# wusize/CLIPSelf

Hardware: AMD Instinct MI355X
Metric: images/sec (student+teacher distill step), ViT-B/16 32 crops/img (higher is better)
Workload: dtype bf16; 1 GPU; EVA02-CLIP-B-16 CLIPSelf image-patches step, 64 images x 32 crops per GPU, 224^2 (BASELINE configs[1]); global_batch=64, crops_per_image=32, image_size=224, parallelism=dp1, teacher_chunk=2048, teacher_last_block=cls_query_only, teacher_schedule=one_batch_ahead_on_side_stream

## Files before the change

clipself_amd/csrc/elementwise.hip:

```cpp
#include "cs_common.h"

namespace {

__device__ __forceinline__ float silu_f(float x) { return x / (1.f + __expf(-x)); }

__global__ __launch_bounds__(256) void swiglu_fwd_kernel(const __bf16* __restrict__ x12, long ldx, __bf16* __restrict__ h, long ldh,
                                                         int M, int Hd) {
    const int vec_per_row = Hd >> 3;
    const long total = (long)M * vec_per_row;
    for (long i = (long)blockIdx.x * blockDim.x + threadIdx.x; i < total; i += (long)gridDim.x * blockDim.x) {
        const int m = (int)(i / vec_per_row), j = (int)(i - (long)m * vec_per_row) * 8;
        U128 a, b, o;
        a.u = *(const uint4*)(x12 + (size_t)m * ldx + j);
        b.u = *(const uint4*)(x12 + (size_t)m * ldx + Hd + j);
#pragma unroll
        for (int e = 0; e < 8; ++e) o.e[e] = f2bf(silu_f(bf2f(a.e[e])) * bf2f(b.e[e]));
        *(uint4*)(h + (size_t)m * ldh + j) = o.u;
    }
}

__global__ __launch_bounds__(256) void swiglu_bwd_kernel(const __bf16* __restrict__ dh, long lddh, const __bf16* __restrict__ x12, long ldx,
                                                         __bf16* __restrict__ dx12, long lddx, int M, int Hd) {
    const int vec_per_row = Hd >> 3;
    const long total = (long)M * vec_per_row;
    for (long i = (long)blockIdx.x * blockDim.x + threadIdx.x; i < total; i += (long)gridDim.x * blockDim.x) {
        const int m = (int)(i / vec_per_row), j = (int)(i - (long)m * vec_per_row) * 8;
        U128 a, b, g, o1, o2;
        a.u = *(const uint4*)(x12 + (size_t)m * ldx + j);
        b.u = *(const uint4*)(x12 + (size_t)m * ldx + Hd + j);
        g.u = *(const uint4*)(dh + (size_t)m * lddh + j);
#pragma unroll
        for (int e = 0; e < 8; ++e) {
            const float x1 = bf2f(a.e[e]), x2 = bf2f(b.e[e]), d = bf2f(g.e[e]);
            const float sig = 1.f / (1.f + __expf(-x1));
            o1.e[e] = f2bf(d * x2 * (sig + x1 * sig * (1.f - sig)));
            o2.e[e] = f2bf(d * x1 * sig);
        }
        *(uint4*)(dx12 + (size_t)m * lddx + j) = o1.u;
        *(uint4*)(dx12 + (size_t)m * lddx + Hd + j) = o2.u;
    }
}

__global__ __launch_bounds__(256) void swiglu_bwd_colsum_kernel(const __bf16* __restrict__ dh, long lddh, const __bf16* __restrict__ x12, long ldx,
                                                                __bf16* __restrict__ dx12, long lddx, float* __restrict__ part, int M, int Hd,
                                                                int rows_per_block) {
    __shared__ float red[2][4][512];
    const int tx = threadIdx.x & 63, ty = threadIdx.x >> 6;
    const int j = (blockIdx.x * 64 + tx) * 8;
    const int m_begin = blockIdx.y * rows_per_block, m_end = min(M, m_begin + rows_per_block);
    float s1[8] = {0, 0, 0, 0, 0, 0, 0, 0}, s2[8] = {0, 0, 0, 0, 0, 0, 0, 0};
    if (j < Hd) {
        auto one = [&](const U128& a, const U128& b, const U128& g, int m) {
            U128 o1, o2;
#pragma unroll
            for (int e = 0; e < 8; ++e) {
                const float x1 = bf2f(a.e[e]), x2 = bf2f(b.e[e]), d = bf2f(g.e[e]);
                const float sig = 1.f / (1.f + __expf(-x1));
                o1.e[e] = f2bf(d * x2 * (sig + x1 * sig * (1.f - sig)));
                o2.e[e] = f2bf(d * x1 * sig);
                s1[e] += bf2f(o1.e[e]);
                s2[e] += bf2f(o2.e[e]);
            }
            *(uint4*)(dx12 + (size_t)m * lddx + j) = o1.u;
            *(uint4*)(dx12 + (size_t)m * lddx + Hd + j) = o2.u;
        };
        int m = m_begin + ty;
        for (; m + 4 < m_end; m += 8) {
            U128 a[2], b[2], g[2];
#pragma unroll
            for (int u = 0; u < 2; ++u) {
                a[u].u = *(const uint4*)(x12 + (size_t)(m + 4 * u) * ldx + j);
                b[u].u = *(const uint4*)(x12 + (size_t)(m + 4 * u) * ldx + Hd + j);
                g[u].u = *(const uint4*)(dh + (size_t)(m + 4 * u) * lddh + j);
            }
            one(a[0], b[0], g[0], m);
            one(a[1], b[1], g[1], m + 4);
        }
        for (; m < m_end; m += 4) {
            U128 a, b, g;
            a.u = *(const uint4*)(x12 + (size_t)m * ldx + j);
            b.u = *(const uint4*)(x12 + (size_t)m * ldx + Hd + j);
            g.u = *(const uint4*)(dh + (size_t)m * lddh + j);
            one(a, b, g, m);
        }
    }
#pragma unroll
    for (int e = 0; e < 8; ++e) { red[0][ty][tx * 8 + e] = s1[e]; red[1][ty][tx * 8 + e] = s2[e]; }
    __syncthreads();
    for (int c = threadIdx.x; c < 512; c += 256) {
        const int col = blockIdx.x * 512 + c;
        if (col < Hd) {
            part[(size_t)blockIdx.y * 2 * Hd + col] = (red[0][0][c] + red[0][1][c]) + (red[0][2][c] + red[0][3][c]);
            part[(size_t)blockIdx.y * 2 * Hd + Hd + col] = (red[1][0][c] + red[1][1][c]) + (red[1][2][c] + red[1][3][c]);
        }
    }
}

template <int IT>
__global__ __launch_bounds__(256) void swiglu_bwd_q8_kernel(const __bf16* __restrict__ dh, long lddh, const __bf16* __restrict__ x12, long ldx,
// ... 127 lines not shown
            U128 o;
#pragma unroll
            for (int e = 0; e < 8; ++e) ((uint16_t*)&o)[e] = tile[rv + e][c];
            *(uint4*)(dst + (size_t)(c0 + c) * ld_out + r0 + rv) = o.u;
        }
        return;
    }
    const int tx = threadIdx.x & 63, ty = threadIdx.x >> 6;
#pragma unroll
    for (int i = 0; i < 16; ++i) {
        const int r = r0 + ty * 16 + i, c = c0 + tx;
        tile[ty * 16 + i][tx] = (r < R && c < Cc) ? src[(size_t)r * ld_in + c] : (uint16_t)0;
    }
    __syncthreads();
#pragma unroll
    for (int i = 0; i < 16; ++i) {
        const int c = c0 + ty * 16 + i, r = r0 + tx;
        if (c < Cc && r < ld_out) dst[(size_t)c * ld_out + r] = tile[tx][ty * 16 + i];
    }
}

__global__ __launch_bounds__(256) void transpose_bf16_kernel(const __bf16* __restrict__ in, long ld_in, __bf16* __restrict__ out,
                                                             long ld_out, int R, int Cc) {
    __shared__ uint16_t tile[64][66];
    transpose_tile(in, ld_in, out, ld_out, R, Cc, blockIdx.y * 64, blockIdx.x * 64, tile);
}

struct TransposeDesc {
    const __bf16* in;
    __bf16* out;
    long ld_in, ld_out;
    int R, Cc, tile0, tiles_x;
};
__global__ __launch_bounds__(256) void transpose_bf16_batched_kernel(const TransposeDesc* __restrict__ desc, int count) {
    __shared__ uint16_t tile[64][66];
    const int t = blockIdx.x;
    int i = 0;
    while (i + 1 < count && desc[i + 1].tile0 <= t) ++i;
    const TransposeDesc d = desc[i];
    const int local = t - d.tile0;
    transpose_tile(d.in, d.ld_in, d.out, d.ld_out, d.R, d.Cc, (local / d.tiles_x) * 64, (local % d.tiles_x) * 64, tile);
}

__global__ __launch_bounds__(256) void colsum_bf16_kernel(const __bf16* __restrict__ x, long ldx, float* __restrict__ out, int M, int N,
                                                          int rows_per_block) {
    __shared__ float red[4][512];
    const int tx = threadIdx.x & 63, ty = threadIdx.x >> 6;
    const int n = (blockIdx.x * 64 + tx) * 8;
    const int m_begin = blockIdx.y * rows_per_block, m_end = min(M, m_begin + rows_per_block);
    float s[8] = {0, 0, 0, 0, 0, 0, 0, 0};
    const bool vec = (ldx & 7) == 0 && ((uintptr_t)x & 15) == 0;
    if (n + 8 <= N && vec) {
        int m = m_begin + ty;
        for (; m + 12 < m_end; m += 16) {
            U128 v[4];
#pragma unroll
            for (int u = 0; u < 4; ++u) v[u].u = *(const uint4*)(x + (size_t)(m + 4 * u) * ldx + n);
#pragma unroll
            for (int u = 0; u < 4; ++u)
#pragma unroll
                for (int e = 0; e < 8; ++e) s[e] += bf2f(v[u].e[e]);
        }
        for (; m < m_end; m += 4) {
            U128 v;
            v.u = *(const uint4*)(x + (size_t)m * ldx + n);
#pragma unroll
            for (int e = 0; e < 8; ++e) s[e] += bf2f(v.e[e]);
        }
    } else {
        for (int m = m_begin + ty; m < m_end; m += 4)
            for (int e = 0; e < 8; ++e)
                if (n + e < N) s[e] += bf2f(x[(size_t)m * ldx + n + e]);
    }
#pragma unroll
    for (int e = 0; e < 8; ++e) red[ty][tx * 8 + e] = s[e];
    __syncthreads();
    for (int c = threadIdx.x; c < 512; c += 256) {
        const int col = blockIdx.x * 512 + c;
        if (col < N) out[(size_t)blockIdx.y * N + col] = (red[0][c] + red[1][c]) + (red[2][c] + red[3][c]);
    }
}

__global__ __launch_bounds__(256) void colsum_reduce_kernel(const float* __restrict__ part, int nblocks, int N, float* __restrict__ out) {
    __shared__ float red[4][64];
    const int tx = threadIdx.x & 63, r = threadIdx.x >> 6;
    const int n = blockIdx.x * 64 + tx;
    float s = 0.f;
    if (n < N) {
        int b = r;
        for (; b + 28 < nblocks; b += 32) {
            float v[8];
#pragma unroll
            for (int u = 0; u < 8; ++u) v[u] = part[(size_t)(b + 4 * u) * N + n];
#pragma unroll
            for (int u = 0; u < 8; ++u) s += v[u];
        }
        for (; b < nblocks; b += 4) s += part[(size_t)b * N + n];
    }
    red[r][tx] = s;
    __syncthreads();
    if (r == 0 && n < N) out[n] += (red[0][tx] + red[1][tx]) + (red[2][tx] + red[3][tx]);
}

template <typename TI>
__global__ __launch_bounds__(256) void im2row_kernel(const TI* __restrict__ img, __bf16* __restrict__ out, int B, int S, int p, int g, int ldo) {
    const int segs = p / 8;
    const long total = (long)B * g * g * 3 * p * segs;
    for (long i = (long)blockIdx.x * blockDim.x + threadIdx.x; i < total; i += (long)gridDim.x * blockDim.x) {
        long t = i;
        const int sg = (int)(t % segs); t /= segs;
        const int iy = (int)(t % p); t /= p;
        const int c = (int)(t % 3); t /= 3;
        const int px = (int)(t % g); t /= g;
        const int py = (int)(t % g); t /= g;
        const int b = (int)t;
        const TI* s = img + (((size_t)b * 3 + c) * S + (py * p + iy)) * S + px * p + sg * 8;
        U128 o;
#pragma unroll
        for (int e = 0; e < 8; ++e) o.e[e] = f2bf((float)s[e]);
        const size_t row = ((size_t)b * g + py) * g + px;
        *(uint4*)(out + row * ldo + (c * p + iy) * p + sg * 8) = o.u;
    }
}

template <typename TI>
__global__ __launch_bounds__(256) void im2row_generic_kernel(const TI* __restrict__ img, __bf16* __restrict__ out, int B, int S, int p, int g, int ldo) {
    const long total = (long)B * g * g * ldo;
    const int kk = 3 * p * p;
    for (long i = (long)blockIdx.x * blockDim.x + threadIdx.x; i < total; i += (long)gridDim.x * blockDim.x) {
        const int col = (int)(i % ldo);
        const long row = i / ldo;
        float v = 0.f;
        if (col < kk) {
            const int ix = col % p, iy = (col / p) % p, c = col / (p * p);
            const int px = (int)(row % g), py = (int)((row / g) % g), b = (int)(row / ((long)g * g));
            v = (float)img[(((size_t)b * 3 + c) * S + (py * p + iy)) * S + px * p + ix];
        }
        out[i] = f2bf(v);
    }
}

__global__ void cls_row_kernel(float* __restrict__ x, const float* __restrict__ cls, const float* __restrict__ pos, int B, int Ntok, int C) {
    const long i = (long)blockIdx.x * blockDim.x + threadIdx.x;
    if (i >= (long)B * C) return;
    const int b = (int)(i / C), c = (int)(i - (long)b * C);
    x[(size_t)b * Ntok * C + c] = cls[c] + pos[c];
}

inline int grid_for(long total, int block = 256, int cap = 256 * 16) {
    long g = (total + block - 1) / block;
    return (int)(g < 1 ? 1 : (g > cap ? cap : g));
}

}

extern "C" int cs_swiglu_fwd(const void* x12, long ldx, void* h, long ldh, int M, int Hd, hipStream_t stream) {
    CS_CHECK_ARG(Hd % 8 == 0 && ldx % 8 == 0 && ldh % 8 == 0 && M > 0, "cs_swiglu_fwd: Hd/ld must be multiples of 8");
    hipLaunchKernelGGL(swiglu_fwd_kernel, dim3(grid_for((long)M * (Hd / 8))), dim3(256), 0, stream, (const __bf16*)x12, ldx, (__bf16*)h, ldh, M, Hd);
    CS_LAUNCH_CHECK();
    return 0;
}
extern "C" int cs_swiglu_bwd(const void* dh, long lddh, const void* x12, long ldx, void* dx12, long lddx, int M, int Hd, hipStream_t stream) {
    CS_CHECK_ARG(Hd % 8 == 0 && ldx % 8 == 0 && lddh % 8 == 0 && lddx % 8 == 0 && M > 0, "cs_swiglu_bwd: Hd/ld must be multiples of 8");
    hipLaunchKernelGGL(swiglu_bwd_kernel, dim3(grid_for((long)M * (Hd / 8))), dim3(256), 0, stream, (const __bf16*)dh, lddh, (const __bf16*)x12, ldx,
                       (__bf16*)dx12, lddx, M, Hd);
    CS_LAUNCH_CHECK();
    return 0;
}
constexpr int COLSUM_ROWS = 64;
extern "C" int cs_swiglu_bwd_colsum(const void* dh, long lddh, const void* x12, long ldx, void* dx12, long lddx, float* colsum, void* workspace,
                                    int M, int Hd, hipStream_t stream) {
    CS_CHECK_ARG(Hd % 8 == 0 && ldx % 8 == 0 && lddh % 8 == 0 && lddx % 8 == 0 && M > 0, "cs_swiglu_bwd_colsum: Hd/ld must be multiples of 8");
    CS_CHECK_ARG(colsum != nullptr && workspace != nullptr, "cs_swiglu_bwd_colsum: colsum and workspace (cs_colsum_workspace(M, 2*Hd) bytes) are required");
    const int nblocks = (M + COLSUM_ROWS - 1) / COLSUM_ROWS;
    hipLaunchKernelGGL(swiglu_bwd_colsum_kernel, dim3((Hd + 511) / 512, nblocks), dim3(256), 0, stream, (const __bf16*)dh, lddh, (const __bf16*)x12, ldx,
                       (__bf16*)dx12, lddx, (float*)workspace, M, Hd, COLSUM_ROWS);
    CS_LAUNCH_CHECK();
    hipLaunchKernelGGL(colsum_reduce_kernel, dim3((2 * Hd + 63) / 64), dim3(256), 0, stream, (const float*)workspace, nblocks, 2 * Hd, colsum);
    CS_LAUNCH_CHECK();
    return 0;
}
extern "C" int cs_swiglu_bwd_q8(const void* dh, long lddh, const void* x12, long ldx, void* dx12, long lddx, void* q8, long ldq, float* q_scale,
                                int M, int Hd, hipStream_t stream) {
    const int Kp = (2 * Hd + 127) / 128 * 128;
    CS_CHECK_ARG(Hd % 8 == 0 && Hd >= 8 && Hd <= 4096 && ldx % 8 == 0 && lddh % 8 == 0 && lddx % 8 == 0 && M > 0, "cs_swiglu_bwd_q8: Hd=%d (%% 8, <= 4096), ld %% 8", Hd);
    CS_CHECK_ARG(q8 && q_scale && ldq >= Kp && ldq % 8 == 0 && ((uintptr_t)q8 % 8) == 0, "cs_swiglu_bwd_q8: q8 rows of >= %d bytes, 8-byte aligned", Kp);
    const dim3 grid((M + 3) / 4), block(256);
#define SWQ(IT) hipLaunchKernelGGL(swiglu_bwd_q8_kernel<IT>, grid, block, 0, stream, (const __bf16*)dh, lddh, (const __bf16*)x12, ldx, (__bf16*)dx12, lddx, \
                                   (unsigned char*)q8, ldq, q_scale, M, Hd, Kp)
    if (Hd <= 2048) SWQ(4); else if (Hd <= 3072) SWQ(6); else SWQ(8);
#undef SWQ
    CS_LAUNCH_CHECK();
    return 0;
}
extern "C" int cs_gelu_fwd(const void* x, long ldx, void* y, long ldy, int M, int N, int quick, hipStream_t stream) {
    CS_CHECK_ARG(x && y && N % 8 == 0 && ldx % 8 == 0 && ldy % 8 == 0 && M > 0 && N > 0, "cs_gelu_fwd: N/ld must be multiples of 8");
    const dim3 grid(grid_for((long)M * (N / 8))), block(256);
    if (quick) hipLaunchKernelGGL(gelu_fwd_kernel<true>, grid, block, 0, stream, (const __bf16*)x, ldx, (__bf16*)y, ldy, M, N);
    else hipLaunchKernelGGL(gelu_fwd_kernel<false>, grid, block, 0, stream, (const __bf16*)x, ldx, (__bf16*)y, ldy, M, N);
    CS_LAUNCH_CHECK();
    return 0;
}
extern "C" int cs_gelu_bwd(const void* dy, long lddy, const void* x, long ldx, void* dx, long lddx, int M, int N, int quick, hipStream_t stream) {
    CS_CHECK_ARG(dy && x && dx && N % 8 == 0 && ldx % 8 == 0 && lddy % 8 == 0 && lddx % 8 == 0 && M > 0 && N > 0,
                 "cs_gelu_bwd: N/ld must be multiples of 8");
    const dim3 grid(grid_for((long)M * (N / 8))), block(256);
    if (quick) hipLaunchKernelGGL(gelu_bwd_kernel<true>, grid, block, 0, stream, (const __bf16*)dy, lddy, (const __bf16*)x, ldx, (__bf16*)dx, lddx, M, N);
    else hipLaunchKernelGGL(gelu_bwd_kernel<false>, grid, block, 0, stream, (const __bf16*)dy, lddy, (const __bf16*)x, ldx, (__bf16*)dx, lddx, M, N);
    CS_LAUNCH_CHECK();
    return 0;
}
extern "C" int cs_cast_f32_bf16(const float* x, void* y, long n, hipStream_t stream) {
    CS_CHECK_ARG(n > 0 && n % 8 == 0, "cs_cast_f32_bf16: n must be a positive multiple of 8");
    hipLaunchKernelGGL(cast_f32_bf16_kernel, dim3(grid_for(n / 8)), dim3(256), 0, stream, x, (__bf16*)y, n / 8);
    CS_LAUNCH_CHECK();
    return 0;
}
extern "C" int cs_transpose_bf16(const void* in, long ld_in, void* out, long ld_out, int R, int Cc, hipStream_t stream) {
    CS_CHECK_ARG(R > 0 && Cc > 0 && ld_out >= R, "cs_transpose_bf16: bad shape R=%d C=%d ld_out=%ld", R, Cc, ld_out);
    dim3 grid((Cc + 63) / 64, (int)((ld_out + 63) / 64));
    hipLaunchKernelGGL(transpose_bf16_kernel, grid, dim3(256), 0, stream, (const __bf16*)in, ld_in, (__bf16*)out, ld_out, R, Cc);
    CS_LAUNCH_CHECK();
    return 0;
}
extern "C" int cs_transpose_bf16_batched(const void* desc, int count, int total_tiles, hipStream_t stream) {
    CS_CHECK_ARG(desc != nullptr && count > 0 && total_tiles > 0, "cs_transpose_bf16_batched: empty batch");
    static_assert(sizeof(TransposeDesc) == 48, "descriptor layout is part of the C ABI");
    hipLaunchKernelGGL(transpose_bf16_batched_kernel, dim3(total_tiles), dim3(256), 0, stream, (const TransposeDesc*)desc, count);
    CS_LAUNCH_CHECK();
    return 0;
}
extern "C" size_t cs_colsum_workspace(int M, int N) {
    return (size_t)((M + COLSUM_ROWS - 1) / COLSUM_ROWS) * (size_t)(N > 0 ? N : 0) * sizeof(float);
}
extern "C" int cs_colsum_bf16(const void* x, long ldx, float* out, void* workspace, int M, int N, hipStream_t stream) {
    CS_CHECK_ARG(M > 0 && N > 0 && workspace != nullptr, "cs_colsum_bf16: empty input or no workspace (cs_colsum_workspace bytes)");
    const int nblocks = (M + COLSUM_ROWS - 1) / COLSUM_ROWS;
    dim3 grid((N + 511) / 512, nblocks);
    hipLaunchKernelGGL(colsum_bf16_kernel, grid, dim3(256), 0, stream, (const __bf16*)x, ldx, (float*)workspace, M, N, COLSUM_ROWS);
    CS_LAUNCH_CHECK();
    hipLaunchKernelGGL(colsum_reduce_kernel, dim3((N + 63) / 64), dim3(256), 0, stream, (const float*)workspace, nblocks, N, out);
    CS_LAUNCH_CHECK();
    return 0;
}
extern "C" int cs_im2row(const void* img, int img_dtype, void* out, int B, int S, int p, int ldo, hipStream_t stream) {
    CS_CHECK_ARG(S % p == 0 && B > 0 && ldo >= 3 * p * p, "cs_im2row: patch size must divide S and ldo >= 3*p*p (p=%d S=%d ldo=%d)", p, S, ldo);
    const int g = S / p;
    if (p % 8 == 0 && ldo == 3 * p * p) {
        const long total = (long)B * g * g * 3 * p * (p / 8);
        if (img_dtype == 0)
            hipLaunchKernelGGL((im2row_kernel<float>), dim3(grid_for(total)), dim3(256), 0, stream, (const float*)img, (__bf16*)out, B, S, p, g, ldo);
        else
            hipLaunchKernelGGL((im2row_kernel<__bf16>), dim3(grid_for(total)), dim3(256), 0, stream, (const __bf16*)img, (__bf16*)out, B, S, p, g, ldo);
    } else {
        const long total = (long)B * g * g * ldo;
        if (img_dtype == 0)
            hipLaunchKernelGGL((im2row_generic_kernel<float>), dim3(grid_for(total)), dim3(256), 0, stream, (const float*)img, (__bf16*)out, B, S, p, g, ldo);
        else
            hipLaunchKernelGGL((im2row_generic_kernel<__bf16>), dim3(grid_for(total)), dim3(256), 0, stream, (const __bf16*)img, (__bf16*)out, B, S, p, g, ldo);
    }
    CS_LAUNCH_CHECK();
    return 0;
}
extern "C" int cs_cls_row(float* x, const float* cls, const float* pos, int B, int Ntok, int C, hipStream_t stream) {
    CS_CHECK_ARG(B > 0, "cs_cls_row: empty batch");
    hipLaunchKernelGGL(cls_row_kernel, dim3((int)(((long)B * C + 255) / 256)), dim3(256), 0, stream, x, cls, pos, B, Ntok, C);
    CS_LAUNCH_CHECK();
    return 0;
}

namespace {

template <int IT>
__global__ __launch_bounds__(256) void quant_rows_fp8_kernel(const __bf16* __restrict__ x, long ldx, unsigned char* __restrict__ q, long ldq,
                                                             float* __restrict__ scale, int M, int K, int Kp) {
    const int lane = threadIdx.x & 63;
    const long row = (long)blockIdx.x * 4 + (threadIdx.x >> 6);
    if (row >= M) return;
    U128 v[IT];
    float amax = 0.f;
#pragma unroll
    for (int it = 0; it < IT; ++it) {
        const int k = (it * 64 + lane) * 8;
        if (k < K) {
            v[it].u = *(const uint4*)(x + row * ldx + k);
#pragma unroll
            for (int e = 0; e < 8; ++e) amax = fmaxf(amax, fabsf(bf2f(v[it].e[e])));
        } else {
            v[it].u = make_uint4(0, 0, 0, 0);
        }
    }
    amax = wave_max(amax);
    const float inv = amax > 0.f ? 448.f / amax : 0.f;
    if (lane == 0) scale[row] = amax > 0.f ? amax / 448.f : 1.f;
#pragma unroll
    for (int it = 0; it < IT; ++it) {
        const int k = (it * 64 + lane) * 8;
        if (k < Kp) {
            unsigned lo = 0, hi = 0;
            lo = __builtin_amdgcn_cvt_pk_fp8_f32(bf2f(v[it].e[0]) * inv, bf2f(v[it].e[1]) * inv, lo, false);
            lo = __builtin_amdgcn_cvt_pk_fp8_f32(bf2f(v[it].e[2]) * inv, bf2f(v[it].e[3]) * inv, lo, true);
            hi = __builtin_amdgcn_cvt_pk_fp8_f32(bf2f(v[it].e[4]) * inv, bf2f(v[it].e[5]) * inv, hi, false);
            hi = __builtin_amdgcn_cvt_pk_fp8_f32(bf2f(v[it].e[6]) * inv, bf2f(v[it].e[7]) * inv, hi, true);
            *(uint2*)(q + row * ldq + k) = make_uint2(lo, hi);
        }
    }
}

}

extern "C" int cs_quant_rows_fp8(const void* x, long ldx, void* q, long ldq, float* scale, int M, int K, hipStream_t stream) {
    const int Kp = (K + 127) / 128 * 128;
    CS_CHECK_ARG(M > 0 && K > 0 && K % 8 == 0 && K <= 8192, "cs_quant_rows_fp8: K=%d must be a multiple of 8, at most 8192", K);
    CS_CHECK_ARG(ldx % 8 == 0 && ldq >= Kp && ldq % 8 == 0 && ((uintptr_t)x % 16) == 0 && ((uintptr_t)q % 8) == 0,
                 "cs_quant_rows_fp8: rows must be 16-byte (input) / 8-byte (output) aligned and ldq >= %d", Kp);
    if (K <= 4096) hipLaunchKernelGGL(quant_rows_fp8_kernel<8>, dim3((M + 3) / 4), dim3(256), 0, stream, (const __bf16*)x, ldx, (unsigned char*)q, ldq, scale, M, K, Kp);
    else hipLaunchKernelGGL(quant_rows_fp8_kernel<16>, dim3((M + 3) / 4), dim3(256), 0, stream, (const __bf16*)x, ldx, (unsigned char*)q, ldq, scale, M, K, Kp);
    CS_LAUNCH_CHECK();
    return 0;
}
```

clipself_amd/csrc/gemm.hip:

```cpp
#include "gemm_common.h"
#include <hip/amd_detail/amd_hip_unsafe_atomics.h>

namespace {

constexpr int EP_LD = 68;
constexpr int EP_BYTES = 32 * EP_LD * 4;

template <int FM, int BN>
__device__ __forceinline__ void epilogue_swiglu(const GemmArgs& p, const f32x16 (&acc)[FM][2], char* slab_bytes, char* rowst_bytes, int lane,
                                                int row0, int tn, int wn) {
    const int l31 = lane & 31, hf = lane >> 5;
    uint32_t* slab = (uint32_t*)slab_bytes;
    const int hbase = tn * (BN / 2) + wn * 32;
    const int hl = hbase + l31;
    float b1 = 0.f, b2 = 0.f;
    if (p.bias && hl < p.group) { b1 = p.bias[hl]; b2 = p.bias[p.group + hl]; }
    const bool ln = p.ln_mean != nullptr;
    float c1 = 0.f, c2 = 0.f;
    float2* rowst = (float2*)rowst_bytes;
    if (ln) {
        if (hl < p.group) { c1 = p.ln_colsum[hl]; c2 = p.ln_colsum[p.group + hl]; }
        for (int r = lane; r < FM * 32; r += 64) {
            const int row = min(row0 + r, p.M - 1);
            const float rs = p.ln_rstd[row];
            rowst[r] = make_float2(-rs * p.ln_mean[row], rs);
        }
        asm volatile("s_waitcnt lgkmcnt(0)" ::: "memory");
    }
    const int c4 = lane & 7, hcol = hbase + c4 * 4;
    const bool colok = hcol < p.group;
#pragma unroll
    for (int i = 0; i < FM; ++i) {
#pragma unroll
        for (int e = 0; e < 16; e += 2) {
            float h[2];
            float4 st4 = make_float4(0.f, 1.f, 0.f, 1.f);
            if (ln) st4 = *(const float4*)(rowst + i * 32 + mfma32_row(e, lane));
#pragma unroll
            for (int t = 0; t < 2; ++t) {
                float u = acc[i][0][e + t], v = acc[i][1][e + t];
                if (ln) {
                    const float2 st = t ? make_float2(st4.z, st4.w) : make_float2(st4.x, st4.y);
                    u = fmaf(st.y, u, fmaf(st.x, c1, b1));
                    v = fmaf(st.y, v, fmaf(st.x, c2, b2));
                } else {
                    u += b1;
                    v += b2;
                }
                h[t] = u * __builtin_amdgcn_rcpf(1.f + __builtin_amdgcn_exp2f(-1.4426950408889634f * u)) * v;
            }
            union { bf16x2 v; uint32_t u; } pk;
            pk.v[0] = f2bf(h[0]);
            pk.v[1] = f2bf(h[1]);
            const int rp = ((e & 3) >> 1) + 4 * (e >> 2) + 2 * hf;
            slab[rp * 32 + l31] = pk.u;
        }
        asm volatile("s_waitcnt lgkmcnt(0)" ::: "memory");
        const int row_base = row0 + i * 32;
        float ps[4] = {0, 0, 0, 0}, pq[4] = {0, 0, 0, 0};
#pragma unroll
        for (int k = 0; k < 2; ++k) {
            const int rp = (lane >> 3) + 8 * k;
            const uint4 w = *(const uint4*)(slab + rp * 32 + c4 * 4);
            const uint2 lo = make_uint2((w.x & 0xffffu) | (w.y << 16), (w.z & 0xffffu) | (w.w << 16));
            const uint2 hi = make_uint2((w.x >> 16) | (w.y & 0xffff0000u), (w.z >> 16) | (w.w & 0xffff0000u));
            const int ra = row_base + 2 * rp;
            if (colok && ra < p.M) *(uint2*)((__bf16*)p.C + (size_t)ra * p.ldc + hcol) = lo;
            if (colok && ra + 1 < p.M) *(uint2*)((__bf16*)p.C + (size_t)(ra + 1) * p.ldc + hcol) = hi;
            if (p.stats_part && colok) {
                const uint32_t ws[4] = {w.x, w.y, w.z, w.w};
#pragma unroll
                for (int t = 0; t < 4; ++t) {
                    const float a = __uint_as_float(ws[t] << 16), b = __uint_as_float(ws[t] & 0xffff0000u);
                    ps[2 * k] += a; pq[2 * k] += a * a;
                    ps[2 * k + 1] += b; pq[2 * k + 1] += b * b;
                }
            }
        }
        if (p.stats_part) {
            const int sel = lane & 7;
            float sv = 0.f, qv = 0.f;
#pragma unroll
            for (int j = 0; j < 4; ++j) {
// ... 538 lines not shown
                 "cs_gemm_nt: N, ldc must be multiples of 4 and C 16-byte aligned (vector epilogue)");
    CS_CHECK_ARG(bias == nullptr || ((uintptr_t)bias % 16) == 0, "cs_gemm_nt: bias must be 16-byte aligned");
    GemmArgs a;
    a.A = (const __bf16*)A; a.B = (const __bf16*)B; a.C = C; a.bias = bias; a.extra = extra;
    a.M = M; a.N = N; a.K = K; a.lda = lda; a.ldb = ldb; a.ldc = ldc; a.group = group;
    a.split_stride = 0;
    a.ln_mean = ln_mean; a.ln_rstd = ln_rstd; a.ln_colsum = ln_colsum; a.stats_part = stats_part;
    a.xb_out = (__bf16*)xb_out; a.ldxb = ldxb;
    a.tiles_m = a.tiles_n = 0;
    a.gm = ((flags >> 8) & 15) ? ((flags >> 8) & 15) : 8;
    a.rm = (flags >> 16) & 3;
    a.nsplit = 1;
    if (a.rm == 1 || a.rm == 2) {
        const int f = (flags >> 8) & 15;
        CS_CHECK_ARG(f == 0 || f == 1 || f == 2 || f == 4 || f == 8, "cs_gemm_nt: B-stationary raster needs 1, 2, 4 or 8 N parts (got %d)", f);
        int parts = f;
        if (parts == 0) for (parts = 1; parts < 8 && (double)N * K * 2 / parts > 3.3e6; parts *= 2) {}
        a.nsplit = parts;
        a.gm = 8;
    }
    if (epi == EPI_SWIGLU_BF16) CS_CHECK_ARG(group > 0 && N == 2 * group, "cs_gemm_nt: swiglu epilogue needs N == 2*group");
    if (epi == EPI_RESID_LN_F32) CS_CHECK_ARG(ln_mean && ln_rstd && ln_colsum && ((uintptr_t)ln_colsum % 16) == 0, "cs_gemm_nt_ln: epilogue 6 needs mean, rstd and a 16-byte aligned column-sum vector");
    CS_CHECK_ARG(stats_part == nullptr || epi == EPI_SWIGLU_BF16 || epi == EPI_RESID_F32 || epi == EPI_RESID_LN_F32,
                 "cs_gemm_nt_ln: statistics output exists for the SwiGLU and residual epilogues");
    CS_CHECK_ARG(xb_out == nullptr || ((epi == EPI_RESID_F32 || epi == EPI_RESID_LN_F32) && ldxb % 4 == 0 && ((uintptr_t)xb_out % 8) == 0),
                 "cs_gemm_nt_ln: the bf16 copy exists for the residual epilogues (8-byte aligned, ldxb %% 4 == 0)");
    CS_CHECK_ARG((ln_mean == nullptr) == (ln_rstd == nullptr) && (ln_mean == nullptr || ln_colsum != nullptr),
                 "cs_gemm_nt_ln: mean, rstd and the column-sum vector come together");
    CS_CHECK_ARG(ln_mean == nullptr || epi_is_bf16(epi) || epi == EPI_SWIGLU_BF16 || epi == EPI_RESID_LN_F32,
                 "cs_gemm_nt_ln: a folded LayerNorm exists for epilogues 0, 3, 6, 7 and 8");
    if (epi == EPI_PATCH_F32 || epi == EPI_RESID_F32 || epi == EPI_RESID_LN_F32) CS_CHECK_ARG(extra != nullptr && ((uintptr_t)extra % 16) == 0, "cs_gemm_nt: epilogue %d needs 16-byte aligned extra", epi);
    if (epi == EPI_PATCH_F32) CS_CHECK_ARG(group > 0, "cs_gemm_nt: patch epilogue needs group");
    a.ktiles_per_split = K / BK;
    const int glds = (flags & 1) ? 0 : 1;
    const int force = (flags >> 4) & 15;
    a.dbg = (flags >> 12) & 15;
    a.reserve = (flags >> 20) & 255;
    switch (epi) {
        case EPI_BF16: return launch<EPI_BF16>(a, splits, glds, force, stream);
        case EPI_F32: return launch<EPI_F32>(a, splits, glds, force, stream);
        case EPI_RESID_F32: return launch<EPI_RESID_F32>(a, splits, glds, force, stream);
        case EPI_SWIGLU_BF16: return launch<EPI_SWIGLU_BF16>(a, splits, glds, force, stream);
        case EPI_ATOMIC_F32: return launch<EPI_ATOMIC_F32>(a, splits, glds, force, stream);
        case EPI_PATCH_F32: return launch<EPI_PATCH_F32>(a, splits, glds, force, stream);
        case EPI_RESID_LN_F32: return launch<EPI_RESID_LN_F32>(a, splits, glds, force, stream);
        case EPI_GELU_BF16: return launch<EPI_GELU_BF16>(a, splits, glds, force, stream);
        case EPI_QGELU_BF16: return launch<EPI_QGELU_BF16>(a, splits, glds, force, stream);
    }
    cs_set_error("cs_gemm_nt: unknown epilogue %d", epi);
    return -1;
}

static int gemm_nt_split_f32(const void* A, const void* B, float* C, int M, int N, int K, int lda, int ldb, int cfg, int splits, hipStream_t stream) {
    CS_CHECK_ARG(M > 0 && N > 0 && K > 0 && K % BK == 0 && N % 4 == 0, "cs_gemm_wgrad: bad problem M=%d N=%d K=%d", M, N, K);
    CS_CHECK_ARG((lda % 8) == 0 && (ldb % 8) == 0 && ((uintptr_t)A % 16) == 0 && ((uintptr_t)B % 16) == 0, "cs_gemm_wgrad: operands must be 16-byte aligned rows");
    GemmArgs a;
    a.A = (const __bf16*)A; a.B = (const __bf16*)B; a.C = C; a.bias = nullptr; a.extra = nullptr;
    a.M = M; a.N = N; a.K = K; a.lda = lda; a.ldb = ldb; a.ldc = N; a.group = 0;
    a.split_stride = (long)M * N;
    a.ln_mean = a.ln_rstd = a.ln_colsum = nullptr; a.stats_part = nullptr; a.xb_out = nullptr; a.ldxb = 0;
    a.tiles_m = a.tiles_n = 0; a.gm = 8; a.dbg = 0; a.rm = 0; a.nsplit = 1; a.reserve = 0;
    a.ktiles_per_split = K / BK;
    return launch<EPI_F32>(a, splits, 1, cfg, stream);
}

extern "C" int cs_gemm_nt(const void* A, const void* B, void* C, const float* bias, const float* extra, int M, int N, int K,
                          int lda, int ldb, int ldc, int epi, int splits, int group, int flags, hipStream_t stream) {
    CS_CHECK_ARG(epi != EPI_RESID_LN_F32, "cs_gemm_nt: epilogue 6 (folded LayerNorm) is reached through cs_gemm_nt_ln");
    return gemm_nt_impl(A, B, C, bias, extra, nullptr, nullptr, nullptr, nullptr, nullptr, 0, M, N, K, lda, ldb, ldc, epi, splits, group, flags, stream);
}

extern "C" int cs_gemm_nt_ln(const void* A, const void* B, void* C, const float* bias, const float* extra, const float* ln_mean,
                             const float* ln_rstd, const float* ln_colsum, float* stats_part, void* xb_out, int ldxb, int M, int N, int K,
                             int lda, int ldb, int ldc, int epi, int splits, int group, int flags, hipStream_t stream) {
    return gemm_nt_impl(A, B, C, bias, extra, ln_mean, ln_rstd, ln_colsum, stats_part, xb_out, ldxb, M, N, K, lda, ldb, ldc, epi, splits, group,
                        flags, stream);
}


namespace {

__global__ __launch_bounds__(256) void splitk_reduce_kernel(const float* __restrict__ ws, int splits, long stride, float* __restrict__ dst,
                                                            int M, int N, int ldc) {
    const long i = (long)blockIdx.x * 256 + threadIdx.x;
    const int n4 = N >> 2;
    if (i >= (long)M * n4) return;
    const int row = (int)(i / n4), c = (int)(i - (long)row * n4) * 4;
    float4 acc = *(const float4*)(ws + (size_t)row * N + c);
    for (int s = 1; s < splits; ++s) {
        const float4 t = *(const float4*)(ws + (size_t)s * stride + (size_t)row * N + c);
        acc.x += t.x; acc.y += t.y; acc.z += t.z; acc.w += t.w;
    }
    float4* d = (float4*)(dst + (size_t)row * ldc + c);
    const float4 o = *d;
    *d = make_float4(o.x + acc.x, o.y + acc.y, o.z + acc.z, o.w + acc.w);
}

typedef __attribute__((ext_vector_type(4))) short s16x4;

__device__ __forceinline__ int tn_swz(int tok) { return (tok & 3) << 1; }
typedef short s16x8 __attribute__((ext_vector_type(8)));
struct TrFrag { s16x4 lo, hi; };
__device__ __forceinline__ void tr_read(TrFrag& f, const char* tile, int tok, int colbyte) {
    const int a0 = tok * 512 + (colbyte ^ (tn_swz(tok) << 5)), a1 = (tok + 4) * 512 + (colbyte ^ (tn_swz(tok + 4) << 5));
    const unsigned base = (unsigned)(uintptr_t)(__attribute__((address_space(3))) const char*)tile;
    asm volatile("ds_read_b64_tr_b16 %0, %1" : "=v"(f.lo) : "v"(base + (unsigned)a0));
    asm volatile("ds_read_b64_tr_b16 %0, %1" : "=v"(f.hi) : "v"(base + (unsigned)a1));
}
__device__ __forceinline__ bf16x8 tr_join(const TrFrag& f) {
    const s16x8 v = __builtin_shufflevector(f.lo, f.hi, 0, 1, 2, 3, 4, 5, 6, 7);
    return __builtin_bit_cast(bf16x8, v);
}

template <bool RAGGED>
__global__ __launch_bounds__(512) void gemm_tn_kernel(GemmArgs p) {
    constexpr int BM = 256, BN = 256, WN = 4, TM = 128, TN = 64, FM = 4, FN = 2;
    constexpr int T_BYTES = 64 * 512;
    extern __shared__ __attribute__((aligned(16))) char smem[];
    const int tid = threadIdx.x, lane = tid & 63;
    const int wave = __builtin_amdgcn_readfirstlane(tid >> 6);
    const int wm = wave / WN, wn = wave - wm * WN;
    const int li = lane & 15, grp = lane >> 4, hf = grp >> 1, g1 = grp & 1;
    int tm, tn;
    tile_of_block(p, tm, tn);
    const int n0 = tm * BM, k0 = tn * BN;
    char* const b_ring = smem + 3 * T_BYTES;
    const int drow = lane >> 5, pc = lane & 31;
    const bool role_a = wave >= 4;
    const int piece0 = (wave & 3) * 8;
    unsigned ocol[8], ooff[8];
#pragma unroll
    for (int x = 0; x < 8; ++x) {
        const int row = 2 * (piece0 + x) + drow;
        const int lc = ((((pc >> 1) ^ tn_swz(row)) << 1) | (pc & 1));
        const unsigned ca = (unsigned)(RAGGED ? min(n0 + lc * 8, p.M - 8) : n0 + lc * 8) * 2u;
        const unsigned cb = (unsigned)(RAGGED ? min(k0 + lc * 8, p.N - 8) : k0 + lc * 8) * 2u;
        ocol[x] = role_a ? ca : cb;
        ooff[x] = (unsigned)row * (unsigned)(role_a ? p.lda : p.ldb) * 2u + ocol[x];
    }
    const int ktiles_all = (p.K + 63) >> 6;
    const int kt_begin = blockIdx.y * p.ktiles_per_split, kt_end = min(kt_begin + p.ktiles_per_split, ktiles_all);
    auto issue = [&](int kt, char* dst) {
        const int ld = role_a ? p.lda : p.ldb;
        const char* src = (const char*)(role_a ? p.A : p.B) + (size_t)kt * 64 * ld * 2;
        const int rmax = p.K - 1 - kt * 64;
        if (!RAGGED || rmax >= 63) {
#pragma unroll
            for (int x = 0; x < 8; ++x)
                __builtin_amdgcn_global_load_lds((const __attribute__((address_space(1))) void*)(src + ooff[x]),
                                                 (__attribute__((address_space(3))) void*)(dst + (piece0 + x) * 1024), 16, 0, 0);
        } else {
#pragma unroll
            for (int x = 0; x < 8; ++x) {
                const int row = min(2 * (piece0 + x) + drow, rmax);
                __builtin_amdgcn_global_load_lds((const __attribute__((address_space(1))) void*)(src + (size_t)row * ld * 2 + ocol[x]),
                                                 (__attribute__((address_space(3))) void*)(dst + (piece0 + x) * 1024), 16, 0, 0);
            }
        }
    };
    f32x16 acc[FM][FN];
#pragma unroll
    for (int i = 0; i < FM; ++i)
#pragma unroll
        for (int j = 0; j < FN; ++j)
#pragma unroll
            for (int e = 0; e < 16; ++e) acc[i][j][e] = 0.f;
    if (role_a) {
        if (kt_begin < kt_end) issue(kt_begin, smem);
        if (kt_begin + 1 < kt_end) issue(kt_begin + 1, smem + T_BYTES);
    } else if (kt_begin < kt_end) {
        issue(kt_begin, b_ring);
    }
    const int segbyte = (16 * g1 + 4 * (li & 3)) * 2, trow = 8 * hf + (li >> 2);
    int cur = 0;
    for (int kt = kt_begin; kt < kt_end; ++kt) {
        if (role_a && kt + 1 < kt_end) asm volatile("s_waitcnt vmcnt(8)" ::: "memory");
        else asm volatile("s_waitcnt vmcnt(0)" ::: "memory");
        asm volatile("s_waitcnt lgkmcnt(0)" ::: "memory");
        __builtin_amdgcn_s_barrier();
        const int i0 = kt - kt_begin;
        if (!role_a && kt + 1 < kt_end) issue(kt + 1, b_ring + ((i0 + 1) & 1) * T_BYTES);
        const char* ta = smem + cur * T_BYTES;
        const char* tb = b_ring + (i0 & 1) * T_BYTES;
        const int tvalid = p.K - kt * 64;
        if (RAGGED && tvalid < 64) {
            for (int idx = tid; idx < (64 - tvalid) * 32; idx += 512)
                *(uint4*)(smem + cur * T_BYTES + (tvalid + (idx >> 5)) * 512 + (idx & 31) * 16) = make_uint4(0, 0, 0, 0);
            __syncthreads();
        }
        TrFrag a[2][FM], b[2][FN];
        auto load_frags = [&](int set, int ts) {
#pragma unroll
            for (int i = 0; i < FM; ++i) tr_read(a[set][i], ta, 16 * ts + trow, (wm * TM + i * 32) * 2 + segbyte);
#pragma unroll
            for (int j = 0; j < FN; ++j) tr_read(b[set][j], tb, 16 * ts + trow, (wn * TN + j * 32) * 2 + segbyte);
        };
        static_assert(FM == 4 && FN == 2, "tr_wait names exactly FM = 4 and FN = 2 fragment pairs: extend its operand list with the tile");
        auto tr_wait = [&](int set) {
            asm volatile("s_waitcnt lgkmcnt(0)"
                         : "+v"(a[set][0].lo), "+v"(a[set][0].hi), "+v"(a[set][1].lo), "+v"(a[set][1].hi), "+v"(a[set][2].lo), "+v"(a[set][2].hi),
                           "+v"(a[set][3].lo), "+v"(a[set][3].hi), "+v"(b[set][0].lo), "+v"(b[set][0].hi), "+v"(b[set][1].lo), "+v"(b[set][1].hi));
        };
        load_frags(0, 0);
        tr_wait(0);
#pragma unroll
        for (int ts = 0; ts < 4; ++ts) {
            if (ts < 3) load_frags((ts + 1) & 1, ts + 1);
            if (ts == 3 && role_a && kt + 2 < kt_end) issue(kt + 2, smem + ((i0 + 2) % 3) * T_BYTES);
#pragma unroll
            for (int i = 0; i < FM; ++i)
#pragma unroll
                for (int j = 0; j < FN; ++j)
                    acc[i][j] = __builtin_amdgcn_mfma_f32_32x32x16_bf16(tr_join(a[ts & 1][i]), tr_join(b[ts & 1][j]), acc[i][j], 0, 0, 0);
            if (ts < 3) tr_wait((ts + 1) & 1);
        }
        cur = cur == 2 ? 0 : cur + 1;
    }
    __syncthreads();
    epilogue<EPI_F32, FM, FN, BN>(p, acc, smem, wave, lane, n0 + wm * TM, k0, tn, wn);
}

void choose_wgrad(int M, int N, int K, int& cfg, int& splits) {
    const int ktiles = K / BK;
    const double out_mb = 4.0 * M * N / 1e6;
    const struct { int cfg, bm, bn, per_cu; double us; } cand[3] = {{1, 128, 128, 2, 1.9}, {2, 256, 128, 1, 1.4}, {7, 256, 256, 1, 2.2}};
    double best = 1e30;
    cfg = 7; splits = 1;
    for (const auto& c : cand) {
        if (M < c.bm || N < c.bn) continue;
        const long tiles = (long)((M + c.bm - 1) / c.bm) * ((N + c.bn - 1) / c.bn);
        for (int s = 1; s <= 64 && s <= ktiles; ++s) {
            const long rounds = (tiles * s + (long)cs_num_cus() * c.per_cu - 1) / ((long)cs_num_cus() * c.per_cu);
            const int kper = (ktiles + s - 1) / s;
            const double t = rounds * (kper * c.us + 6.0) + (s + 2) * out_mb / 5.0 + 6.0;
            if (t < best) { best = t; cfg = c.cfg; splits = s; }
        }
    }
}

}

namespace {
int choose_tn_splits(int N, int K, int tokens) {
    const long tiles = (long)((N + 255) / 256) * ((K + 255) / 256);
    const int ktiles = (tokens + 63) / 64;
    double best = 1e30;
    int splits = 1;
    for (int sp = 1; sp <= 64 && sp <= ktiles; ++sp) {
        const long rounds = (tiles * sp + 255) / 256;
        const double t = rounds * (((ktiles + sp - 1) / sp) * 2.2 + 6.0) + (sp + 2) * (4.0 * N * K / 1e6) / 5.0;
        if (t < best) { best = t; splits = sp; }
    }
    return splits;
}
}

extern "C" size_t cs_gemm_wgrad_tn_workspace(int N, int K, int tokens) {
    if (tokens <= 0 || N < 8 || K < 8 || N % 8 != 0 || K % 8 != 0) return 0;
    return (size_t)choose_tn_splits(N, K, tokens) * N * K * sizeof(float);
}

extern "C" int cs_gemm_wgrad_tn(const void* dY, const void* X, float* dW, void* workspace, int N, int K, int tokens, int ldy, int ldx, int ldc,
                                hipStream_t stream) {
    if (tokens <= 0 || N < 8 || K < 8 || N % 8 != 0 || K % 8 != 0) return 1;
    CS_CHECK_ARG(workspace != nullptr && ((uintptr_t)workspace % 16) == 0 && dW != nullptr && ((uintptr_t)dW % 16) == 0 && ldc % 4 == 0,
                 "cs_gemm_wgrad_tn: workspace / dW must be 16-byte aligned buffers");
    CS_CHECK_ARG(ldy % 8 == 0 && ldx % 8 == 0 && ((uintptr_t)dY % 16) == 0 && ((uintptr_t)X % 16) == 0 && ldy >= N && ldx >= K,
                 "cs_gemm_wgrad_tn: operand rows must be 16-byte aligned");
    CS_CHECK_ARG((long)64 * ldy * 2 < 0x7fffffffL && (long)64 * ldx * 2 < 0x7fffffffL, "cs_gemm_wgrad_tn: row stride too large");
    int splits = choose_tn_splits(N, K, tokens);
    GemmArgs a;
    a.A = (const __bf16*)dY; a.B = (const __bf16*)X; a.C = workspace; a.bias = nullptr; a.extra = nullptr;
    a.M = N; a.N = K; a.K = tokens; a.lda = ldy; a.ldb = ldx; a.ldc = K; a.group = 0;
    a.split_stride = (long)N * K;
    a.ln_mean = a.ln_rstd = a.ln_colsum = nullptr; a.stats_part = nullptr; a.xb_out = nullptr; a.ldxb = 0;
    a.tiles_m = (N + 255) / 256; a.tiles_n = (K + 255) / 256; a.gm = 8; a.dbg = 0; a.rm = 0; a.nsplit = 1; a.reserve = 0;
    const int ktiles = (tokens + 63) / 64;
    a.ktiles_per_split = (ktiles + splits - 1) / splits;
    constexpr size_t lds = 160 * 1024;
    static bool once = ((void)hipFuncSetAttribute((const void*)gemm_tn_kernel<false>, hipFuncAttributeMaxDynamicSharedMemorySize, (int)lds),
                        (void)hipFuncSetAttribute((const void*)gemm_tn_kernel<true>, hipFuncAttributeMaxDynamicSharedMemorySize, (int)lds), true);
    (void)once;
    if (tokens % 64 == 0 && N % 256 == 0 && K % 256 == 0) hipLaunchKernelGGL(gemm_tn_kernel<false>, dim3(a.tiles_m * a.tiles_n, splits), dim3(512), lds, stream, a);
    else hipLaunchKernelGGL(gemm_tn_kernel<true>, dim3(a.tiles_m * a.tiles_n, splits), dim3(512), lds, stream, a);
    CS_LAUNCH_CHECK();
    const long n = (long)N * (K >> 2);
    hipLaunchKernelGGL(splitk_reduce_kernel, dim3((unsigned)((n + 255) / 256)), dim3(256), 0, stream, (const float*)workspace, splits,
                       (long)N * K, dW, N, K, ldc);
    CS_LAUNCH_CHECK();
    return 0;
}

extern "C" size_t cs_gemm_wgrad_workspace(int M, int N, int K) {
    int cfg, splits;
    choose_wgrad(M, N, K, cfg, splits);
    return (size_t)splits * M * N * sizeof(float);
}

extern "C" int cs_gemm_wgrad(const void* A, const void* B, float* dW, void* workspace, int M, int N, int K, int lda, int ldb, int ldc,
                             hipStream_t stream) {
    CS_CHECK_ARG(workspace != nullptr && ((uintptr_t)workspace % 16) == 0 && dW != nullptr && ((uintptr_t)dW % 16) == 0 && ldc % 4 == 0,
                 "cs_gemm_wgrad: workspace / dW must be 16-byte aligned buffers");
    int cfg, splits;
    choose_wgrad(M, N, K, cfg, splits);
    const int rc = gemm_nt_split_f32(A, B, (float*)workspace, M, N, K, lda, ldb, cfg, splits, stream);
    if (rc) return rc;
    const long n = (long)M * (N >> 2);
    hipLaunchKernelGGL(splitk_reduce_kernel, dim3((unsigned)((n + 255) / 256)), dim3(256), 0, stream, (const float*)workspace, splits,
                       (long)M * N, dW, M, N, ldc);
    CS_LAUNCH_CHECK();
    return 0;
}
```

clipself_amd/csrc/norm.hip:

```cpp
#include "cs_common.h"

namespace {

constexpr int MAXC = 3072;
constexpr int ROWS_PER_WG = 4;

template <typename T> struct Vec4;
template <> struct Vec4<float> {
    typedef float4 raw;
    static __device__ __forceinline__ raw load_raw(const float* p) { return *(const float4*)p; }
    static __device__ __forceinline__ void cvt(const raw& t, float (&v)[4]) { v[0] = t.x; v[1] = t.y; v[2] = t.z; v[3] = t.w; }
    static __device__ __forceinline__ void load(const float* p, float (&v)[4]) { cvt(load_raw(p), v); }
};
template <> struct Vec4<__bf16> {
    typedef uint2 raw;
    static __device__ __forceinline__ raw load_raw(const __bf16* p) { return *(const uint2*)p; }
    static __device__ __forceinline__ void cvt(const raw& r, float (&v)[4]) {
        U64 t; t.u = r;
#pragma unroll
        for (int i = 0; i < 4; ++i) v[i] = bf2f(t.e[i]);
    }
    static __device__ __forceinline__ void load(const __bf16* p, float (&v)[4]) { cvt(load_raw(p), v); }
};
__device__ __forceinline__ void store_bf16x4(__bf16* p, const float (&v)[4]) {
    U64 t;
#pragma unroll
    for (int i = 0; i < 4; ++i) t.e[i] = f2bf(v[i]);
    *(uint2*)p = t.u;
}
__device__ __forceinline__ void store_x4(__bf16* p, const float (&v)[4]) { store_bf16x4(p, v); }
__device__ __forceinline__ void store_x4(float* p, const float (&v)[4]) { *(float4*)p = make_float4(v[0], v[1], v[2], v[3]); }

template <typename TX, int MAXG, typename TY = __bf16, bool Q8 = false, bool RAG = false>
__global__ __launch_bounds__(256) void ln_fwd_kernel(const TX* __restrict__ x, long ldx, const float* __restrict__ gamma,
                                                     const float* __restrict__ beta, TY* __restrict__ y, long ldy,
                                                     float* __restrict__ mean_out, float* __restrict__ rstd_out,
                                                     int M, int C, float eps, unsigned char* __restrict__ q8 = nullptr, long ldq = 0,
                                                     float* __restrict__ q_scale = nullptr, int Kp = 0) {
    const int lane = threadIdx.x & 63;
    const int row = blockIdx.x * ROWS_PER_WG + (threadIdx.x >> 6);
    if (row >= M) return;
    const TX* xr = x + (size_t)row * ldx;
    const int ng = (C + 255) >> 8;
    const int clast = (C - 1) & ~3;
    float v[MAXG][4];
    typename Vec4<TX>::raw xr_raw[MAXG];
#pragma unroll
    for (int g = 0; g < MAXG; ++g) {
        const int c = (g * 64 + lane) * 4;
        xr_raw[g] = Vec4<TX>::load_raw(xr + (g < ng ? min(c, clast) : 0));
    }
    float s = 0.f;
#pragma unroll
    for (int g = 0; g < MAXG; ++g) {
        const int c = (g * 64 + lane) * 4;
        Vec4<TX>::cvt(xr_raw[g], v[g]);
#pragma unroll
        for (int i = 0; i < 4; ++i) v[g][i] = (g < ng && (RAG ? c + i < C : c < C)) ? v[g][i] : 0.f;
        s += (v[g][0] + v[g][1]) + (v[g][2] + v[g][3]);
    }
    const float mean = wave_sum(s) / (float)C;
    float q = 0.f;
#pragma unroll
    for (int g = 0; g < MAXG; ++g) {
        const int c = (g * 64 + lane) * 4;
#pragma unroll
        for (int i = 0; i < 4; ++i) { const float d = v[g][i] - mean; q += (g < ng && c + i < C) ? d * d : 0.f; }
    }
    const float rstd = rsqrtf(wave_sum(q) / (float)C + eps);
    if (y != nullptr) {
        TY* yr = y + (size_t)row * ldy;
        float4 ga[MAXG], be[MAXG];
#pragma unroll
        for (int g = 0; g < MAXG; ++g) {
            const int c = g < ng ? min((g * 64 + lane) * 4, clast) : 0;
            ga[g] = *(const float4*)(gamma + c);
            be[g] = *(const float4*)(beta + c);
        }
        float amax = 0.f;
#pragma unroll
        for (int g = 0; g < MAXG; ++g) {
            const int c = (g * 64 + lane) * 4;
            if (g < ng && c < C) {
                float o[4] = {(v[g][0] - mean) * rstd * ga[g].x + be[g].x, (v[g][1] - mean) * rstd * ga[g].y + be[g].y,
                              (v[g][2] - mean) * rstd * ga[g].z + be[g].z, (v[g][3] - mean) * rstd * ga[g].w + be[g].w};
                if (RAG) {
#pragma unroll
                    for (int i = 0; i < 4; ++i) o[i] = (c + i < C) ? o[i] : 0.f;
                }
                store_x4(yr + c, o);
                if (Q8) {
#pragma unroll
                    for (int i = 0; i < 4; ++i) {
                        v[g][i] = (c + i < C) ? bf2f(f2bf(o[i])) : 0.f;
                        amax = fmaxf(amax, fabsf(v[g][i]));
                    }
                }
            } else if (Q8) {
#pragma unroll
                for (int i = 0; i < 4; ++i) v[g][i] = 0.f;
            }
        }
        if (Q8) {
            amax = wave_max(amax);
            const float inv = amax > 0.f ? 448.f / amax : 0.f;
            if (lane == 0) q_scale[row] = amax > 0.f ? amax / 448.f : 1.f;
#pragma unroll
            for (int g = 0; g < MAXG; ++g) {
                const int c = (g * 64 + lane) * 4;
                if (c < Kp) {
                    unsigned w = 0;
                    w = __builtin_amdgcn_cvt_pk_fp8_f32(v[g][0] * inv, v[g][1] * inv, w, false);
                    w = __builtin_amdgcn_cvt_pk_fp8_f32(v[g][2] * inv, v[g][3] * inv, w, true);
                    *(unsigned*)(q8 + (size_t)row * ldq + c) = w;
                }
            }
        }
    }
    if (lane == 0 && mean_out) { mean_out[row] = mean; rstd_out[row] = rstd; }
}

__global__ __launch_bounds__(256) void ln_stats_finalize_kernel(const float* __restrict__ part, int P, int npp, int C, int M, float eps,
                                                                float* __restrict__ mean_out, float* __restrict__ rstd_out) {
    const int row = blockIdx.x * 256 + threadIdx.x;
    if (row >= M) return;
    const float2* src = (const float2*)part + row;
    float s = 0.f, q = 0.f, b = 0.f;
    int p = 0;
    for (; p + 8 <= P; p += 8) {
        float2 v[8];
#pragma unroll
        for (int j = 0; j < 8; ++j) v[j] = src[(size_t)(p + j) * M];
#pragma unroll
        for (int j = 0; j < 8; ++j) {
            const int n = min(npp, C - (p + j) * npp);
            if (n > 0) {
                const float t = v[j].x * v[j].x / (float)n;
                s += v[j].x;
                q += fmaxf(v[j].y - t, 0.f);
                b += t;
            }
        }
    }
    for (; p < P; ++p) {
        const int n = min(npp, C - p * npp);
        if (n <= 0) break;
        const float2 sq = src[(size_t)p * M];
        const float t = sq.x * sq.x / (float)n;
        s += sq.x;
        q += fmaxf(sq.y - t, 0.f);
        b += t;
    }
    const float mean = s / (float)C;
    const float m2 = q + fmaxf(b - s * mean, 0.f);
    mean_out[row] = mean;
    rstd_out[row] = rsqrtf(m2 / (float)C + eps);
}

__global__ __launch_bounds__(256) void ln_stats_finalize2_kernel(const float* __restrict__ part, int P, int npp, int C, int M, float eps,
                                                                 float* __restrict__ mean_out, float* __restrict__ rstd_out) {
    const int row = (blockIdx.x * 256 + threadIdx.x) * 2;
    if (row >= M) return;
    const float4* src = (const float4*)(part + (size_t)row * 2);
    const size_t stride = (size_t)M / 2;
    float s[2] = {0.f, 0.f}, q[2] = {0.f, 0.f}, b[2] = {0.f, 0.f};
    auto add = [&](const float4& v, int n) {
        const float t0 = v.x * v.x / (float)n, t1 = v.z * v.z / (float)n;
        s[0] += v.x; q[0] += fmaxf(v.y - t0, 0.f); b[0] += t0;
        s[1] += v.z; q[1] += fmaxf(v.w - t1, 0.f); b[1] += t1;
    };
    for (int p = 0; p < P; p += 16) {
        float4 v[16];
#pragma unroll
        for (int j = 0; j < 16; ++j) v[j] = src[(size_t)min(p + j, P - 1) * stride];
#pragma unroll
        for (int j = 0; j < 16; ++j) {
            const int n = min(npp, C - (p + j) * npp);
            if (p + j < P && n > 0) add(v[j], n);
        }
    }
#pragma unroll
    for (int r = 0; r < 2; ++r) {
        const float mean = s[r] / (float)C;
        const float m2 = q[r] + fmaxf(b[r] - s[r] * mean, 0.f);
        mean_out[row + r] = mean;
        rstd_out[row + r] = rsqrtf(m2 / (float)C + eps);
    }
}

enum { DX_BF16 = 0, DX_F32_ASSIGN = 1, DX_F32_ACCUM = 2 };

template <typename TX, int DXMODE, int MAXG, bool COPY, bool RAG = false>
__global__ __launch_bounds__(256) void ln_bwd_kernel(const __bf16* __restrict__ dy, long lddy, const TX* __restrict__ x, long ldx,
                                                     const float* __restrict__ gamma, const float* __restrict__ mean_in,
                                                     const float* __restrict__ rstd_in, void* __restrict__ dx, long lddx,
                                                     __bf16* __restrict__ dxb, long lddxb, float* __restrict__ part, int M, int C,
                                                     unsigned char* __restrict__ q8 = nullptr, long ldq = 0, float* __restrict__ q_scale = nullptr,
                                                     int Kp = 0) {
    static_assert(!COPY || DXMODE != DX_BF16, "the bf16 copy exists for the fp32 stream modes");
// ... 66 lines not shown
                } else {
                    float* p = (float*)dx + (size_t)row * lddx + c;
                    if (DXMODE == DX_F32_ACCUM) {
                        const float4 t = *(const float4*)p;
                        const float tv[4] = {t.x, t.y, t.z, t.w};
#pragma unroll
                        for (int i = 0; i < 4; ++i) o[i] += (!RAG || c + i < C) ? tv[i] : 0.f;
                    }
                    *(float4*)p = make_float4(o[0], o[1], o[2], o[3]);
                    if (COPY) {
                        U64 t;
#pragma unroll
                        for (int i = 0; i < 4; ++i) {
                            t.e[i] = f2bf(o[i]);
                            rq[g][i] = (c + i < C) ? bf2f(t.e[i]) : 0.f;
                            dc[g][i] += rq[g][i];
                            amax = fmaxf(amax, fabsf(rq[g][i]));
                        }
                        *(uint2*)(dxb + (size_t)row * lddxb + c) = t.u;
                    }
                }
            }
        }
        if (COPY && q8 != nullptr) {
            amax = wave_max(amax);
            const float inv = amax > 0.f ? 448.f / amax : 0.f;
            if (lane == 0) q_scale[row] = amax > 0.f ? amax / 448.f : 1.f;
#pragma unroll
            for (int g = 0; g < MAXG; ++g) {
                const int c = (g * 64 + lane) * 4;
                if (c < Kp) {
                    unsigned w = 0;
                    w = __builtin_amdgcn_cvt_pk_fp8_f32(rq[g][0] * inv, rq[g][1] * inv, w, false);
                    w = __builtin_amdgcn_cvt_pk_fp8_f32(rq[g][2] * inv, rq[g][3] * inv, w, true);
                    *(unsigned*)(q8 + (size_t)row * ldq + c) = w;
                }
            }
        }
    }
    if (part == nullptr) return;
    if (wave > 0) {
        float* mine = red + (size_t)(wave - 1) * NR * Cp;
#pragma unroll
        for (int g = 0; g < MAXG; ++g) {
            const int c = (g * 64 + lane) * 4;
            if (g < ng && c < C) {
                *(float4*)(mine + c) = make_float4(dg[g][0], dg[g][1], dg[g][2], dg[g][3]);
                *(float4*)(mine + Cp + c) = make_float4(db[g][0], db[g][1], db[g][2], db[g][3]);
                if (COPY) *(float4*)(mine + 2 * Cp + c) = make_float4(dc[g][0], dc[g][1], dc[g][2], dc[g][3]);
            }
        }
    }
    __syncthreads();
    if (wave == 0) {
        float* outp = part + (size_t)blockIdx.x * NR * Cp;
#pragma unroll
        for (int g = 0; g < MAXG; ++g) {
            const int c = (g * 64 + lane) * 4;
            if (g < ng && c < C) {
                float a[4] = {dg[g][0], dg[g][1], dg[g][2], dg[g][3]};
                float b[4] = {db[g][0], db[g][1], db[g][2], db[g][3]};
                float cc[4] = {0.f, 0.f, 0.f, 0.f};
                if (COPY) { cc[0] = dc[g][0]; cc[1] = dc[g][1]; cc[2] = dc[g][2]; cc[3] = dc[g][3]; }
                for (int w = 0; w < 3; ++w) {
                    const float4 t = *(const float4*)(red + (size_t)w * NR * Cp + c);
                    const float4 u = *(const float4*)(red + (size_t)w * NR * Cp + Cp + c);
                    a[0] += t.x; a[1] += t.y; a[2] += t.z; a[3] += t.w;
                    b[0] += u.x; b[1] += u.y; b[2] += u.z; b[3] += u.w;
                    if (COPY) {
                        const float4 v = *(const float4*)(red + (size_t)w * NR * Cp + 2 * Cp + c);
                        cc[0] += v.x; cc[1] += v.y; cc[2] += v.z; cc[3] += v.w;
                    }
                }
                *(float4*)(outp + c) = make_float4(a[0], a[1], a[2], a[3]);
                *(float4*)(outp + Cp + c) = make_float4(b[0], b[1], b[2], b[3]);
                if (COPY) *(float4*)(outp + 2 * Cp + c) = make_float4(cc[0], cc[1], cc[2], cc[3]);
            }
        }
    }
}

__global__ __launch_bounds__(256) void ln_param_reduce_kernel(const float* __restrict__ part, int nparts, int C, int NR, float* __restrict__ out0,
                                                              float* __restrict__ out1, float* __restrict__ out2, int accumulate) {
    __shared__ float red[16][16];
    const int cl = threadIdx.x & 15, grp = threadIdx.x >> 4;
    const int Cp = (C + 3) & ~3;
    const int c = blockIdx.x * 16 + cl;
    const int r = c / Cp, cc = c - r * Cp;
    float* const outs[3] = {out0, out1, out2};
    const bool live = r < NR && cc < C && outs[r < 3 ? r : 0] != nullptr;
    float s0 = 0.f, s1 = 0.f, s2 = 0.f, s3 = 0.f;
    const size_t stride = (size_t)NR * Cp;
    if (live) {
        int p = grp;
        for (; p + 48 < nparts; p += 64) {
            s0 += part[(size_t)p * stride + c];
            s1 += part[(size_t)(p + 16) * stride + c];
            s2 += part[(size_t)(p + 32) * stride + c];
            s3 += part[(size_t)(p + 48) * stride + c];
        }
        for (; p < nparts; p += 16) s0 += part[(size_t)p * stride + c];
    }
    red[grp][cl] = (s0 + s1) + (s2 + s3);
    __syncthreads();
    if (grp == 0 && live) {
        float s = 0.f;
#pragma unroll
        for (int g = 0; g < 16; ++g) s += red[g][cl];
        float* dst = outs[r] + cc;
        *dst = accumulate ? *dst + s : s;
    }
}

__global__ __launch_bounds__(256) void l2norm_fwd_kernel(const float* __restrict__ x, float* __restrict__ y,
                                                         float* __restrict__ inv_out, int M, int C, float eps) {
    const int lane = threadIdx.x & 63;
    const int row = blockIdx.x * ROWS_PER_WG + (threadIdx.x >> 6);
    if (row >= M) return;
    const float* xr = x + (size_t)row * C;
    float s = 0.f;
    for (int c = lane * 4; c < C; c += 256) { const float4 t = *(const float4*)(xr + c); s += t.x * t.x + t.y * t.y + t.z * t.z + t.w * t.w; }
    const float inv = 1.f / fmaxf(sqrtf(wave_sum(s)), eps);
    for (int c = lane * 4; c < C; c += 256) {
        const float4 t = *(const float4*)(xr + c);
        *(float4*)(y + (size_t)row * C + c) = make_float4(t.x * inv, t.y * inv, t.z * inv, t.w * inv);
    }
    if (lane == 0 && inv_out) inv_out[row] = inv;
}

__global__ __launch_bounds__(256) void l2norm_bwd_kernel(const float* __restrict__ dy, const float* __restrict__ y,
                                                         const float* __restrict__ inv, __bf16* __restrict__ dx, int M, int C) {
    const int lane = threadIdx.x & 63;
    const int row = blockIdx.x * ROWS_PER_WG + (threadIdx.x >> 6);
    if (row >= M) return;
    const float* yr = y + (size_t)row * C;
    const float* gr = dy + (size_t)row * C;
    float s = 0.f;
    for (int c = lane * 4; c < C; c += 256) {
        const float4 a = *(const float4*)(yr + c), b = *(const float4*)(gr + c);
        s += a.x * b.x + a.y * b.y + a.z * b.z + a.w * b.w;
    }
    const float dot = wave_sum(s), iv = inv[row];
    for (int c = lane * 4; c < C; c += 256) {
        const float4 a = *(const float4*)(yr + c), b = *(const float4*)(gr + c);
        float o[4] = {(b.x - a.x * dot) * iv, (b.y - a.y * dot) * iv, (b.z - a.z * dot) * iv, (b.w - a.w * dot) * iv};
        store_bf16x4(dx + (size_t)row * C + c, o);
    }
}

}

static int layernorm_fwd_impl(const void* x, int x_dtype, long ldx, const float* gamma, const float* beta, void* y, long ldy, float* mean,
                              float* rstd, int M, int C, float eps, void* q8, long ldq, float* q_scale, hipStream_t stream) {
    CS_CHECK_ARG(C <= MAXC && (C % 4 == 0 || (ldx >= ((C + 3) & ~3) && (y == nullptr || ldy >= ((C + 3) & ~3)))), "cs_layernorm_fwd: C=%d unsupported (ld too small for a padded row, or > %d)", C, MAXC);
    CS_CHECK_ARG(M > 0, "cs_layernorm_fwd: empty input");
    dim3 grid((M + ROWS_PER_WG - 1) / ROWS_PER_WG), block(256);
    if (q8 != nullptr) {
        const int Kp = (C + 127) / 128 * 128;
        CS_CHECK_ARG(y != nullptr && q_scale != nullptr && ldq >= Kp && ldq % 4 == 0 && ((uintptr_t)q8 % 4) == 0 && Kp <= 256 * 12,
                     "cs_layernorm_fwd_q8: needs y, the scale vector and 4-byte aligned e4m3 rows of >= %d bytes", Kp);
#define LNQ2(TX, NG, RG) hipLaunchKernelGGL((ln_fwd_kernel<TX, NG, __bf16, true, RG>), grid, block, 0, stream, (const TX*)x, ldx, gamma, beta, (__bf16*)y, ldy, mean, rstd, M, C, eps, (unsigned char*)q8, ldq, q_scale, Kp)
#define LNQ(TX, NG) do { if (C % 4 == 0) LNQ2(TX, NG, false); else LNQ2(TX, NG, true); } while (0)
        if (x_dtype == 0) { if (Kp <= 1024) LNQ(float, 4); else if (Kp <= 2048) LNQ(float, 8); else LNQ(float, 12); }
        else { if (Kp <= 1024) LNQ(__bf16, 4); else if (Kp <= 2048) LNQ(__bf16, 8); else LNQ(__bf16, 12); }
#undef LNQ
#undef LNQ2
        CS_LAUNCH_CHECK();
        return 0;
    }
#define LNF2(TX, NG, RG) hipLaunchKernelGGL((ln_fwd_kernel<TX, NG, __bf16, false, RG>), grid, block, 0, stream, (const TX*)x, ldx, gamma, beta, (__bf16*)y, ldy, mean, rstd, M, C, eps)
#define LNF(TX, NG) do { if (C % 4 == 0) LNF2(TX, NG, false); else LNF2(TX, NG, true); } while (0)
    if (x_dtype == 0) { if (C <= 1024) LNF(float, 4); else if (C <= 2048) LNF(float, 8); else LNF(float, 12); }
    else { if (C <= 1024) LNF(__bf16, 4); else if (C <= 2048) LNF(__bf16, 8); else LNF(__bf16, 12); }
#undef LNF
#undef LNF2
    CS_LAUNCH_CHECK();
    return 0;
}
extern "C" int cs_layernorm_fwd(const void* x, int x_dtype, long ldx, const float* gamma, const float* beta, void* y, long ldy,
                                float* mean, float* rstd, int M, int C, float eps, hipStream_t stream) {
    return layernorm_fwd_impl(x, x_dtype, ldx, gamma, beta, y, ldy, mean, rstd, M, C, eps, nullptr, 0, nullptr, stream);
}
extern "C" int cs_layernorm_fwd_q8(const void* x, int x_dtype, long ldx, const float* gamma, const float* beta, void* y, long ldy,
                                   float* mean, float* rstd, void* q8, long ldq, float* q_scale, int M, int C, float eps, hipStream_t stream) {
    CS_CHECK_ARG(q8 != nullptr, "cs_layernorm_fwd_q8: q8 is required (use cs_layernorm_fwd otherwise)");
    return layernorm_fwd_impl(x, x_dtype, ldx, gamma, beta, y, ldy, mean, rstd, M, C, eps, q8, ldq, q_scale, stream);
}

extern "C" int cs_layernorm_fwd_f32(const float* x, long ldx, const float* gamma, const float* beta, float* y, long ldy, float* mean,
                                    float* rstd, int M, int C, float eps, hipStream_t stream) {
    CS_CHECK_ARG(x && y && gamma && beta && C <= MAXC && C % 4 == 0 && ldx % 4 == 0 && ldy % 4 == 0 && M > 0,
                 "cs_layernorm_fwd_f32: C=%d unsupported (multiple of 4, <= %d)", C, MAXC);
    CS_CHECK_ARG((mean == nullptr) == (rstd == nullptr), "cs_layernorm_fwd_f32: mean/rstd must both be given or both null");
    dim3 grid((M + ROWS_PER_WG - 1) / ROWS_PER_WG), block(256);
#define LNF32(NG) hipLaunchKernelGGL((ln_fwd_kernel<float, NG, float>), grid, block, 0, stream, x, ldx, gamma, beta, y, ldy, mean, rstd, M, C, eps)
    if (C <= 1024) LNF32(4); else if (C <= 2048) LNF32(8); else LNF32(12);
#undef LNF32
    CS_LAUNCH_CHECK();
    return 0;
}

extern "C" int cs_ln_stats_finalize(const float* part, int P, int npp, int C, int M, float eps, float* mean, float* rstd, hipStream_t stream) {
    CS_CHECK_ARG(part && mean && rstd && P > 0 && npp > 0 && C > 0 && M > 0 && (long)P * npp >= C,
                 "cs_ln_stats_finalize: bad arguments P=%d npp=%d C=%d M=%d", P, npp, C, M);
    if (M % 2 == 0 && ((uintptr_t)part % 16) == 0)
        hipLaunchKernelGGL(ln_stats_finalize2_kernel, dim3((M / 2 + 255) / 256), dim3(256), 0, stream, part, P, npp, C, M, eps, mean, rstd);
    else
        hipLaunchKernelGGL(ln_stats_finalize_kernel, dim3((M + 255) / 256), dim3(256), 0, stream, part, P, npp, C, M, eps, mean, rstd);
    CS_LAUNCH_CHECK();
    return 0;
}

extern "C" size_t cs_layernorm_bwd_workspace(int M, int C) {
    const int nwg = min(512, (M + 3) / 4);
    return (size_t)nwg * 3 * ((C + 3) & ~3) * sizeof(float);
}
static int layernorm_bwd_impl(const void* dy, long lddy, const void* x, int x_dtype, long ldx, const float* gamma, const float* mean,
                              const float* rstd, void* dx, int dx_mode, long lddx, float* dgamma, float* dbeta,
                              int accumulate_params, void* workspace, void* dx_copy, long ldcopy, float* copy_colsum, void* q8, long ldq,
                              float* q_scale, int M, int C, hipStream_t stream) {
    const int Kp = (C + 127) / 128 * 128;
    CS_CHECK_ARG(q8 == nullptr || (dx_copy != nullptr && q_scale != nullptr && ldq >= Kp && ldq % 4 == 0 && ((uintptr_t)q8 % 4) == 0 && Kp <= 256 * 12),
                 "cs_layernorm_bwd_q8: needs dx_copy, the scale vector and 4-byte aligned e4m3 rows of >= %d bytes", Kp);
    CS_CHECK_ARG(C <= MAXC && (C % 4 == 0 || (ldx >= ((C + 3) & ~3) && lddy >= ((C + 3) & ~3) && lddx >= ((C + 3) & ~3))), "cs_layernorm_bwd: C=%d unsupported", C);
    CS_CHECK_ARG(M > 0, "cs_layernorm_bwd: empty input");
    CS_CHECK_ARG(dx_mode >= 0 && dx_mode <= 2, "cs_layernorm_bwd: bad dx_mode");
    CS_CHECK_ARG((dgamma == nullptr) == (dbeta == nullptr), "cs_layernorm_bwd: dgamma/dbeta must both be given or both null");
    CS_CHECK_ARG(dx_copy == nullptr || (dx_mode != 0 && ldcopy >= ((C + 3) & ~3) && ldcopy % 4 == 0 && ((uintptr_t)dx_copy % 8) == 0),
                 "cs_layernorm_bwd: the bf16 copy exists for the fp32 dx modes (8-byte aligned rows, ldcopy >= C rounded up to 4)");
    CS_CHECK_ARG(copy_colsum == nullptr || dx_copy != nullptr, "cs_layernorm_bwd: copy_colsum are the column sums of dx_copy");
    const bool need_part = dgamma != nullptr || copy_colsum != nullptr;
    CS_CHECK_ARG(!need_part || workspace != nullptr, "cs_layernorm_bwd: workspace required for dgamma/dbeta / copy_colsum");
    const int nwg = min(512, (M + 3) / 4);
    float* part = need_part ? (float*)workspace : nullptr;
    const bool copy = dx_copy != nullptr;
    const int NR = copy ? 3 : 2;
    const size_t lds = (size_t)3 * NR * ((C + 3) & ~3) * sizeof(float);
    dim3 grid(nwg), block(256);
#define LNB5(TX, MODE, NG, CP, RG)                                                                                          \
    do {                                                                                                                    \
        static bool once = (hipFuncSetAttribute((const void*)ln_bwd_kernel<TX, MODE, NG, CP, RG>, hipFuncAttributeMaxDynamicSharedMemorySize, 3 * 3 * MAXC * 4), true); \
        (void)once;                                                                                                         \
        hipLaunchKernelGGL((ln_bwd_kernel<TX, MODE, NG, CP, RG>), grid, block, lds, stream, (const __bf16*)dy, lddy, (const TX*)x, ldx, gamma, mean, rstd, dx, lddx, \
                           (__bf16*)dx_copy, ldcopy, part, M, C, (unsigned char*)q8, ldq, q_scale, Kp);                     \
    } while (0)
#define LNB4(TX, MODE, NG, CP) do { if (C % 4 == 0) LNB5(TX, MODE, NG, CP, false); else LNB5(TX, MODE, NG, CP, true); } while (0)
#define LNB3(TX, MODE, NG) do { if (copy) { if constexpr (MODE != DX_BF16) LNB4(TX, MODE, NG, true); } else LNB4(TX, MODE, NG, false); } while (0)
#define LNB(TX, MODE) do { if (C <= 1024) LNB3(TX, MODE, 4); else if (C <= 2048) LNB3(TX, MODE, 8); else LNB3(TX, MODE, 12); } while (0)
    if (x_dtype == 0) {
        if (dx_mode == 0) LNB(float, DX_BF16); else if (dx_mode == 1) LNB(float, DX_F32_ASSIGN); else LNB(float, DX_F32_ACCUM);
    } else {
        if (dx_mode == 0) LNB(__bf16, DX_BF16); else if (dx_mode == 1) LNB(__bf16, DX_F32_ASSIGN); else LNB(__bf16, DX_F32_ACCUM);
    }
#undef LNB
#undef LNB3
#undef LNB4
#undef LNB5
    CS_LAUNCH_CHECK();
    if (need_part) {
        hipLaunchKernelGGL(ln_param_reduce_kernel, dim3((NR * ((C + 3) & ~3) + 15) / 16), dim3(256), 0, stream, part, nwg, C, NR, dgamma, dbeta,
                           copy_colsum, accumulate_params);
        CS_LAUNCH_CHECK();
    }
    return 0;
}
extern "C" int cs_layernorm_bwd(const void* dy, long lddy, const void* x, int x_dtype, long ldx, const float* gamma, const float* mean,
                                const float* rstd, void* dx, int dx_mode, long lddx, float* dgamma, float* dbeta,
                                int accumulate_params, void* workspace, void* dx_copy, long ldcopy, float* copy_colsum, int M, int C,
                                hipStream_t stream) {
    return layernorm_bwd_impl(dy, lddy, x, x_dtype, ldx, gamma, mean, rstd, dx, dx_mode, lddx, dgamma, dbeta, accumulate_params, workspace,
                              dx_copy, ldcopy, copy_colsum, nullptr, 0, nullptr, M, C, stream);
}
extern "C" int cs_layernorm_bwd_q8(const void* dy, long lddy, const void* x, int x_dtype, long ldx, const float* gamma, const float* mean,
                                   const float* rstd, void* dx, int dx_mode, long lddx, float* dgamma, float* dbeta,
                                   int accumulate_params, void* workspace, void* dx_copy, long ldcopy, float* copy_colsum, void* q8, long ldq,
                                   float* q_scale, int M, int C, hipStream_t stream) {
    CS_CHECK_ARG(q8 != nullptr, "cs_layernorm_bwd_q8: q8 is required (cs_layernorm_bwd is the form without it)");
    return layernorm_bwd_impl(dy, lddy, x, x_dtype, ldx, gamma, mean, rstd, dx, dx_mode, lddx, dgamma, dbeta, accumulate_params, workspace,
                              dx_copy, ldcopy, copy_colsum, q8, ldq, q_scale, M, C, stream);
}

extern "C" int cs_l2norm_fwd(const float* x, float* y, float* inv_norm, int M, int C, float eps, hipStream_t stream) {
    CS_CHECK_ARG(C % 4 == 0 && M > 0, "cs_l2norm_fwd: C must be a multiple of 4");
    hipLaunchKernelGGL(l2norm_fwd_kernel, dim3((M + ROWS_PER_WG - 1) / ROWS_PER_WG), dim3(256), 0, stream, x, y, inv_norm, M, C, eps);
    CS_LAUNCH_CHECK();
    return 0;
}
extern "C" int cs_l2norm_bwd(const float* dy, const float* y, const float* inv_norm, void* dx_bf16, int M, int C, hipStream_t stream) {
    CS_CHECK_ARG(C % 4 == 0 && M > 0, "cs_l2norm_bwd: C must be a multiple of 4");
    hipLaunchKernelGGL(l2norm_bwd_kernel, dim3((M + ROWS_PER_WG - 1) / ROWS_PER_WG), dim3(256), 0, stream, dy, y, inv_norm, (__bf16*)dx_bf16, M, C);
    CS_LAUNCH_CHECK();
    return 0;
}
```

clipself_amd/engine.py:

```python
from __future__ import annotations

import os

import torch

from .config import TowerCfg
from .engine_base import (ALIGN, BF16, DX_BF16, DX_F32_ACCUM, DX_F32_ASSIGN, EPI_ATOMIC_F32, EPI_BF16, EPI_F32, EPI_GELU_BF16,
                          EPI_PATCH_F32, EPI_QGELU_BF16, EPI_RESID_F32, EPI_RESID_LN_F32, EPI_SWIGLU_BF16, F32, TowerEngine, _round_up,
                          is_no_decay, padded_hidden)


def param_groups_layout(cfg: TowerCfg, prefix: str = "visual."):
    C, Hd, E, p = cfg.width, cfg.hidden, cfg.embed_dim, cfg.patch_size
    Hp, Kpe, Kp = padded_hidden(cfg), 3 * p * p, _round_up(3 * p * p, 64)
    t = lambda name, shape, storage=None: (name, shape, storage if storage is not None else shape)
    groups = [[t(prefix + "cls_token", (1, 1, C))], [t(prefix + "pos_embed", (1, cfg.tokens, C))],
              [t(prefix + "patch_embed.proj.weight", (C, 3, p, p), (C, Kp))], [t(prefix + "patch_embed.proj.bias", (C,))]]
    for i in range(cfg.layers):
        b = f"{prefix}blocks.{i}."
        groups += [
            [t(b + "norm1.weight", (C,))], [t(b + "norm1.bias", (C,))],
            [t(b + "attn.q_proj.weight", (C, C)), t(b + "attn.k_proj.weight", (C, C)), t(b + "attn.v_proj.weight", (C, C))],
            [t(b + "attn.q_bias", (C,)), t(b + "attn._k_bias_zero", (C,)), t(b + "attn.v_bias", (C,))],
            [t(b + "attn.inner_attn_ln.weight", (C,))], [t(b + "attn.inner_attn_ln.bias", (C,))],
            [t(b + "attn.proj.weight", (C, C))], [t(b + "attn.proj.bias", (C,))],
            [t(b + "norm2.weight", (C,))], [t(b + "norm2.bias", (C,))],
            [t(b + "mlp.w1.weight", (Hd, C), (Hp, C)), t(b + "mlp.w2.weight", (Hd, C), (Hp, C))],
            [t(b + "mlp.w1.bias", (Hd,), (Hp,)), t(b + "mlp.w2.bias", (Hd,), (Hp,))],
            [t(b + "mlp.ffn_ln.weight", (Hd,), (Hp,))], [t(b + "mlp.ffn_ln.bias", (Hd,), (Hp,))],
            [t(b + "mlp.w3.weight", (C, Hd), (C, Hp))], [t(b + "mlp.w3.bias", (C,))],
        ]
    groups += [[t(prefix + "norm.weight", (C,))], [t(prefix + "norm.bias", (C,))],
               [t(prefix + "head.weight", (E, C))], [t(prefix + "head.bias", (E,))]]
    return groups


class EvaEngine(TowerEngine):
    BLOCK_TAG, FINAL_NORM, RESID_BIAS = "blocks.", "norm", "mlp.w3.bias"
    FP8_MAX_ROW = 8192

    def _layout(self):
        return param_groups_layout(self.cfg, self.prefix)

    def _pos_table(self, views):
        return views[self.prefix + "pos_embed"][0]

    def _never_reached(self, i: int, name: str) -> bool:
        return i == self.cfg.layers - 1 and (name.rsplit(".", 2)[-2:] in (["q_proj", "weight"], ["k_proj", "weight"])
                                             or name.endswith("attn.q_bias"))

    def __init__(self, cfg: TowerCfg, ops, trainable: bool = False, prefix: str = "visual."):
        super().__init__(cfg, ops, trainable=trainable, prefix=prefix)
        self.fold_sub_ln = not trainable
        self.fp8_forward = False
        self.w8 = {}
        self.fp8_dgrad = False
        self.wt8 = {}
        self.fused_swiglu_colsum = os.environ.get("CLIPSELF_NO_FUSED_SWIGLU_COLSUM") != "1"

    def _wants_folds(self):
        return self.fold_sub_ln

    def _fold_pass(self, images):
        return self.fold_sub_ln and self.block_folds_active(images)

    def _lo_plane(self, last, cls_folded):
        return last > 0

    def _bwd_widths(self):
        return max(self.cfg.width, self.Hp), max(2 * self.Hp, 3 * self.cfg.width)

    def _bwd_gq(self, M):
        C = self.cfg.width
        return (self.ops.empty((M, _round_up(C, 128)), torch.uint8), self.ops.empty((M,), F32)) if self.fp8_dgrad and C <= 3072 else None

    def _head(self, rows, out):
        self.ops.gemm_nt(rows, self.w[self.prefix + "head.weight"], out, bias=self.p[self.prefix + "head.bias"], epi=EPI_F32)

    def _head_dgrad(self, d_feats, d_lnf):
        self.ops.gemm_nt(d_feats, self.wt["head"][:, :self.cfg.embed_dim], d_lnf, epi=EPI_BF16)

    def _head_wgrad(self, d_feats, lnf, ws):
        self.ops.colsum_bf16(d_feats, self.g[self.prefix + "head.bias"], ws[1])
        self._wgrad(d_feats, lnf, self.g[self.prefix + "head.weight"])

    def sync_shadow(self):
        super().sync_shadow()
        if self.fp8_forward:
            self.sync_fp8()

    def _build_folds(self):
        cfg, C, Hl = self.cfg, self.cfg.width, self.cfg.hidden
        self.fold = {}
        with torch.no_grad():
            for i in range(cfg.layers):
                b = f"{self.prefix}blocks.{i}."
                out = {}
                for key, wname, ln, bname, K in (("proj", "attn.proj.weight", "attn.inner_attn_ln", "attn.proj.bias", C),
                                                 ("w3", "mlp.w3.weight", "mlp.ffn_ln", "mlp.w3.bias", Hl)):
                    W = self.storage_of(self.master, b + wname)
                    g, beta = self.p[b + ln + ".weight"][:K], self.p[b + ln + ".bias"][:K]
                    Wf = torch.zeros_like(W, dtype=BF16)
                    Wf[:, :K] = (W[:, :K] * g[None, :]).to(BF16)
                    out[key] = (Wf, Wf.float().sum(dim=1).contiguous(), (W[:, :K] @ beta + self.p[b + bname]).contiguous())
                if self.fold_block_ln:
                    Hd = self.Hp
                    for key, wname, bias_name, ln, rows in (("qkv", "attn.q_proj.weight", "attn.q_bias", "norm1", 3 * C),
                                                           ("w12", "mlp.w1.weight", "mlp.w1.bias", "norm2", 2 * Hd)):
                        o, ob = self.offsets[b + wname][0], self.offsets[b + bias_name][0]
                        W, bias = self.master[o:o + rows * C].view(rows, C), self.master[ob:ob + rows]
                        g, beta = self.p[b + ln + ".weight"], self.p[b + ln + ".bias"]
                        Wf = (W * g[None, :]).to(BF16).contiguous()
                        out[key] = (Wf, Wf.float().sum(dim=1).contiguous(), (W @ beta + bias).contiguous())
                self.fold[i] = out

    def sync_transposed(self, blocks=None):
        cfg, C, Hd = self.cfg, self.cfg.width, self.Hp
        pairs = []
        for i in (range(self.first_trainable, cfg.layers) if blocks is None else blocks):
            b = f"{self.prefix}blocks.{i}."
            o = self.offsets[b + "attn.q_proj.weight"][0]
            pairs.append((self.shadow[o:o + 3 * C * C].view(3 * C, C), self._wt_alloc((i, "qkv"), 3 * C, C)))
            pairs.append((self.w[b + "attn.proj.weight"], self._wt_alloc((i, "proj"), C, C)))
            o = self.offsets[b + "mlp.w1.weight"][0]
            pairs.append((self.shadow[o:o + 2 * Hd * C].view(2 * Hd, C), self._wt_alloc((i, "w12"), 2 * Hd, C)))
            pairs.append((self.storage_of(self.shadow, b + "mlp.w3.weight"), self._wt_alloc((i, "w3"), C, Hd)))
        pairs.append((self.w[self.prefix + "head.weight"], self._wt_alloc("head", self.cfg.embed_dim, C)))
        self.ops.transpose_bf16_batched(pairs)

    def _fp8_rows(self, X):
        M, K = X.shape
        q = self.ops.empty((M, _round_up(K, 128)), torch.uint8)
        sc = self.ops.empty((M,), F32)
        self.ops.quant_rows_fp8(X, q, sc)
        return q, sc

    def sync_fp8(self, blocks=None):
        cfg, C, Hd = self.cfg, self.cfg.width, self.Hp
        for i in (range(cfg.layers) if blocks is None else blocks):
            b = f"{self.prefix}blocks.{i}."
            o = self.offsets[b + "attn.q_proj.weight"][0]
# ... 79 lines not shown
        ops, cfg, P = self.ops, self.cfg, self.prefix
        B, _, S, _ = images.shape
        p, C = cfg.patch_size, cfg.width
        g = S // p
        N, Kpe = g * g + 1, self.Kpe
        A = ops.empty((B * g * g, Kpe), BF16)
        ops.im2row(images.contiguous(), A, p)
        x = ops.empty((B, N, C), F32)
        pos = self.pos_for(g)
        ops.gemm_nt(A, self.storage_of(self.shadow, P + "patch_embed.proj.weight"), x.view(B * N, C),
                    bias=self.p[P + "patch_embed.proj.bias"], extra=pos, epi=EPI_PATCH_F32, group=g * g)
        ops.cls_row(x, self.p[P + "cls_token"].view(C), pos)
        if keep is not None:
            keep["patches"] = A
        return x, g

    def _qkv_w(self, b):
        C = self.cfg.width
        o = self.offsets[b + "attn.q_proj.weight"][0]
        ob = self.offsets[b + "attn.q_bias"][0]
        return self.shadow[o:o + 3 * C * C].view(3 * C, C), self.master[ob:ob + 3 * C]

    def _w12(self, b):
        C, Hd = self.cfg.width, self.Hp
        o = self.offsets[b + "mlp.w1.weight"][0]
        ob = self.offsets[b + "mlp.w1.bias"][0]
        return self.shadow[o:o + 2 * Hd * C].view(2 * Hd, C), self.master[ob:ob + 2 * Hd]

    def _block_fwd(self, i, x, B, N, cos, sin, with_attn=True, save=None, inplace=True):
        ops, cfg = self.ops, self.cfg
        C, Hd, Hl, H, eps = cfg.width, self.Hp, cfg.hidden, cfg.heads, cfg.ln_eps
        padded = Hd != Hl
        b = f"{self.prefix}blocks.{i}."
        M = B * N
        keep = save is not None
        st = (lambda: (ops.empty((M,), F32), ops.empty((M,), F32))) if keep else (lambda: (None, None))

        ln1 = ops.empty((M, C), BF16)
        m1, r1 = st()
        q1 = self._ln(x, self.p[b + "norm1.weight"], self.p[b + "norm1.bias"], ln1, m1, r1, eps)
        wqkv, bqkv = self._qkv_w(b)
        qkv = lse = None
        if with_attn and not keep and inplace and self.fold_sub_ln:
            qkv = ops.empty((M, 3 * C), BF16)
            ops.gemm_nt(ln1, wqkv, qkv, bias=bqkv, epi=EPI_BF16)
            att = ops.empty((M, C), BF16)
            part = ops.empty((H, M, 2), F32)
            ops.attn_fwd_stats(qkv, cos, sin, att, None, part, B, N, H, cfg.head_width ** -0.5)
            return self._block_post_folded(i, b, x, att, part, M)
        if with_attn:
            qkv = ops.empty((M, 3 * C), BF16)
            self._linear(i, "qkv", ln1, wqkv, qkv, bqkv, xq=q1)
            att = ops.empty((M, C), BF16)
            lse = ops.empty((B * H, N), F32) if keep else None
            ops.attn_fwd(qkv, cos, sin, att, lse, B, N, H, cfg.head_width ** -0.5)
        else:
            att = ops.empty((M, C), BF16)
            self._linear(i, "qkv", ln1, wqkv[2 * C:], att, bqkv[2 * C:], rows=(2 * C, 3 * C), xq=q1)
        x2 = self._block_post(i, b, x, att, M, st, save, inplace)
        if keep:
            save.update(x0=x, ln1=ln1, st1=(m1, r1), qkv=qkv, lse=lse, att=att, with_attn=with_attn)
        return x2

    def _block_post(self, i, b, x, att, M, st, save, inplace):
        ops, cfg = self.ops, self.cfg
        C, Hd, Hl, eps = cfg.width, self.Hp, cfg.hidden, cfg.ln_eps
        padded = Hd != Hl
        keep = save is not None
        iln = ops.empty((M, C), BF16)
        m2, r2 = st()
        q2 = self._ln(att, self.p[b + "attn.inner_attn_ln.weight"], self.p[b + "attn.inner_attn_ln.bias"], iln, m2, r2, eps)
        x1 = x if inplace else ops.empty((M, C), F32)
        self._linear(i, "proj", iln, self.w[b + "attn.proj.weight"], x1, self.p[b + "attn.proj.bias"], extra=x, epi=EPI_RESID_F32, xq=q2)

        ln2 = ops.empty((M, C), BF16)
        m3, r3 = st()
        q3 = self._ln(x1, self.p[b + "norm2.weight"], self.p[b + "norm2.bias"], ln2, m3, r3, eps)
        w12, b12 = self._w12(b)
        hid = ops.empty((M, Hd), BF16)
        x12 = None
        if keep or self.fp8_forward:
            x12 = ops.empty((M, 2 * Hd), BF16)
            self._linear(i, "w12", ln2, w12, x12, b12, xq=q3)
            ops.swiglu_fwd(x12, hid)
        else:
            ops.gemm_nt(ln2, w12, hid, bias=b12, epi=EPI_SWIGLU_BF16, group=Hd)
        fln = (ops.zeros if padded else ops.empty)((M, Hd), BF16)
        m4, r4 = st()
        q4 = self._ln(hid[:, :Hl], self.p[b + "mlp.ffn_ln.weight"], self.p[b + "mlp.ffn_ln.bias"], fln[:, :Hl], m4, r4, eps)
        x2 = x1 if inplace else ops.empty((M, C), F32)
        self._linear(i, "w3", fln, self.storage_of(self.shadow, b + "mlp.w3.weight"), x2, self.p[b + "mlp.w3.bias"], extra=x1,
                     epi=EPI_RESID_F32, xq=q4)
        if keep:
            save.update(iln=iln, st2=(m2, r2), x1=x1, ln2=ln2, st3=(m3, r3), x12=x12, hid=hid, fln=fln, st4=(m4, r4))
        return x2

    def _block_post_folded(self, i, b, x, att, att_part, M):
        ops, cfg = self.ops, self.cfg
        C, Hd, Hl, eps = cfg.width, self.Hp, cfg.hidden, cfg.ln_eps
        f = self.fold[i]
        mean, rstd = ops.empty((M,), F32), ops.empty((M,), F32)
        ops.ln_stats_finalize(att_part, 64, C, mean, rstd, eps)
        Wp, cp, dp = f["proj"]
        ops.gemm_nt_ln(att, Wp, x, bias=dp, extra=x, ln_mean=mean, ln_rstd=rstd, ln_colsum=cp, epi=EPI_RESID_LN_F32)

        ln2 = ops.empty((M, C), BF16)
        ops.layernorm_fwd(x, self.p[b + "norm2.weight"], self.p[b + "norm2.bias"], ln2, None, None, eps)
        w12, b12 = self._w12(b)
        hid = ops.empty((M, Hd), BF16)
        part = ops.empty((4 * ((Hd + 127) // 128), M, 2), F32)
        ops.gemm_nt_ln(ln2, w12, hid, bias=b12, stats_part=part, epi=EPI_SWIGLU_BF16, group=Hd)
        ops.ln_stats_finalize(part, 32, Hl, mean, rstd, eps)
        W3, c3, d3 = f["w3"]
        ops.gemm_nt_ln(hid, W3, x, bias=d3, extra=x, ln_mean=mean, ln_rstd=rstd, ln_colsum=c3, epi=EPI_RESID_LN_F32)
        return x

    def _teacher_block_folded(self, i, x, xb, st, B, N, cos, sin, emit_next, lo=None):
        ops, cfg = self.ops, self.cfg
        C, Hd, Hl, H, eps = cfg.width, self.Hp, cfg.hidden, cfg.heads, cfg.ln_eps
        b = f"{self.prefix}blocks.{i}."
        M = B * N
        f = self.fold[i]
        qkv = ops.empty((M, 3 * C), BF16)
        first = xb is None
        if first:
            ln1 = ops.empty((M, C), BF16)
            ops.layernorm_fwd(x, self.p[b + "norm1.weight"], self.p[b + "norm1.bias"], ln1, None, None, eps)
            wqkv, bqkv = self._qkv_w(b)
            ops.gemm_nt(ln1, wqkv, qkv, bias=bqkv, epi=EPI_BF16)
        else:
            Wq, cq, dq = f["qkv"]
            ops.gemm_nt_ln(xb, Wq, qkv, bias=dq, ln_mean=st[0], ln_rstd=st[1], ln_colsum=cq, epi=EPI_BF16)
        att = ops.empty((M, C), BF16)
        part_a = ops.empty((H, M, 2), F32)
        ops.attn_fwd_stats(qkv, cos, sin, att, None, part_a, B, N, H, cfg.head_width ** -0.5)
        mean, rstd = ops.empty((M,), F32), ops.empty((M,), F32)
        ops.ln_stats_finalize(part_a, 64, C, mean, rstd, eps)
        Wp, cp, dp = f["proj"]
        part_x = ops.empty(((C + 63) // 64, M, 2), F32)
        xb2 = xb if (lo is not None and not first) else ops.empty((M, C), BF16)
        if lo is not None:
            ops.gemm_nt_ln_split(att, Wp, xb2, lo, dp, mean, rstd, cp, x_in=x if first else None, stats_part=part_x)
        else:
            ops.gemm_nt_ln(att, Wp, x, bias=dp, extra=x, ln_mean=mean, ln_rstd=rstd, ln_colsum=cp, stats_part=part_x, xb_out=xb2,
                           epi=EPI_RESID_LN_F32)
        mean2, rstd2 = ops.empty((M,), F32), ops.empty((M,), F32)
        ops.ln_stats_finalize(part_x, 64, C, mean2, rstd2, eps)
        W12, c12, d12 = f["w12"]
        hid = ops.empty((M, Hd), BF16)
        part_h = ops.empty((4 * ((Hd + 127) // 128), M, 2), F32)
        ops.gemm_nt_ln(xb2, W12, hid, bias=d12, ln_mean=mean2, ln_rstd=rstd2, ln_colsum=c12, stats_part=part_h, epi=EPI_SWIGLU_BF16,
                       group=Hd)
        ops.ln_stats_finalize(part_h, 32, Hl, mean, rstd, eps)
        W3, c3, d3 = f["w3"]
        if lo is not None:
            if not emit_next:
                ops.gemm_nt_ln_split(hid, W3, xb2, lo, d3, mean, rstd, c3, x_out=x)
                return None, None
            ops.gemm_nt_ln_split(hid, W3, xb2, lo, d3, mean, rstd, c3, stats_part=part_x)
        else:
            if not emit_next:
                ops.gemm_nt_ln(hid, W3, x, bias=d3, extra=x, ln_mean=mean, ln_rstd=rstd, ln_colsum=c3, epi=EPI_RESID_LN_F32)
                return None, None
            ops.gemm_nt_ln(hid, W3, x, bias=d3, extra=x, ln_mean=mean, ln_rstd=rstd, ln_colsum=c3, stats_part=part_x, xb_out=xb2,
                           epi=EPI_RESID_LN_F32)
        ops.ln_stats_finalize(part_x, 64, C, mean2, rstd2, eps)
        return xb2, (mean2, rstd2)

    def _block_fwd_cls(self, i, x, B, N, cos, sin, xb=None, st=None, lo=None):
        ops, cfg = self.ops, self.cfg
        C, H, eps = cfg.width, cfg.heads, cfg.ln_eps
        b = f"{self.prefix}blocks.{i}."
        M = B * N
        wqkv, bqkv = self._qkv_w(b)
        kv = ops.empty((M, 2 * C), BF16)
        q = ops.empty((B, C), BF16)
        if xb is not None:
            Wq, cq, dq = self.fold[i]["qkv"]
            ops.gemm_nt_ln(xb, Wq[C:], kv, bias=dq[C:], ln_mean=st[0], ln_rstd=st[1], ln_colsum=cq[C:], epi=EPI_BF16)
            xc = (self._join_planes(xb.view(B, N, C)[:, 0, :], lo.view(B, N, C)[:, 0, :]) if lo is not None
                  else x.view(B, N, C)[:, 0, :].contiguous())
            ln1c = ops.empty((B, C), BF16)
            ops.layernorm_fwd(xc, self.p[b + "norm1.weight"], self.p[b + "norm1.bias"], ln1c, None, None, eps)
            ops.gemm_nt(ln1c, wqkv[:C], q, bias=bqkv[:C], epi=EPI_BF16)
        else:
            ln1 = ops.empty((M, C), BF16)
            ops.layernorm_fwd(x, self.p[b + "norm1.weight"], self.p[b + "norm1.bias"], ln1, None, None, eps)
            ops.gemm_nt(ln1, wqkv[C:], kv, bias=bqkv[C:], epi=EPI_BF16)
            ops.gemm_nt(ln1.view(B, N, C)[:, 0, :], wqkv[:C], q, bias=bqkv[:C], epi=EPI_BF16)
            xc = x.view(B, N, C)[:, 0, :].contiguous()
        att = ops.empty((B, C), BF16)
        ops.attn_cls_fwd(q, kv, cos, sin, att, B, N, H, cfg.head_width ** -0.5)
        return self._block_post(i, b, xc, att, B, lambda: (None, None), None, True)

    def _block_bwd(self, i, s, g, gb, B, N, cos, sin, ws, next_bias=None, gq=None):
        q8a = dict(q8=gq[0], q_scale=gq[1]) if gq is not None else {}
        ops, cfg = self.ops, self.cfg
        C, Hd, Hl, H = cfg.width, self.Hp, cfg.hidden, cfg.heads
        padded = Hd != Hl
        b = f"{self.prefix}blocks.{i}."
        M = B * N
        G = self.g
        self._wgrad(gb, s["fln"], self.storage_of(self.grad, b + "mlp.w3.weight"))
        d_fln = ops.empty((M, Hd), BF16)
        self._dgrad(i, "w3", gb, d_fln, q=gq)
        d_hid = (ops.zeros if padded else ops.empty)((M, Hd), BF16)
        ops.layernorm_bwd(d_fln[:, :Hl], s["hid"][:, :Hl], self.p[b + "mlp.ffn_ln.weight"], *s["st4"], d_hid[:, :Hl], DX_BF16,
                          G[b + "mlp.ffn_ln.weight"], G[b + "mlp.ffn_ln.bias"], True, ws[0])
        d_x12 = ops.empty((M, 2 * Hd), BF16)
        ob = self.offsets[b + "mlp.w1.bias"][0]
        q12 = None
        if self.fp8_dgrad and Hd <= 4096:
            q12 = (ops.empty((M, _round_up(2 * Hd, 128)), torch.uint8), ops.empty((M,), F32))
            ops.swiglu_bwd(d_hid, s["x12"], d_x12, q8=q12[0], q_scale=q12[1])
            ops.colsum_bf16(d_x12, self.grad[ob:ob + 2 * Hd], ws[1])
        elif self.fused_swiglu_colsum:
            ops.swiglu_bwd_colsum(d_hid, s["x12"], d_x12, self.grad[ob:ob + 2 * Hd], ws[1])
        else:
            ops.swiglu_bwd(d_hid, s["x12"], d_x12)
            ops.colsum_bf16(d_x12, self.grad[ob:ob + 2 * Hd], ws[1])
        ow = self.offsets[b + "mlp.w1.weight"][0]
        self._wgrad(d_x12, s["ln2"], self.grad[ow:ow + 2 * Hd * C].view(2 * Hd, C))
        d_ln2 = ops.empty((M, C), BF16)
        self._dgrad(i, "w12", d_x12, d_ln2, q=q12)
        ops.layernorm_bwd(d_ln2, s["x1"], self.p[b + "norm2.weight"], *s["st3"], g, DX_F32_ACCUM,
                          G[b + "norm2.weight"], G[b + "norm2.bias"], True, ws[0], dx_copy=gb, copy_colsum=G[b + "attn.proj.bias"], **q8a)
        self._wgrad(gb, s["iln"], G[b + "attn.proj.weight"])
        d_iln = ops.empty((M, C), BF16)
        self._dgrad(i, "proj", gb, d_iln, q=gq)
        d_att = ops.empty((M, C), BF16)
        ops.layernorm_bwd(d_iln, s["att"], self.p[b + "attn.inner_attn_ln.weight"], *s["st2"], d_att, DX_BF16,
                          G[b + "attn.inner_attn_ln.weight"], G[b + "attn.inner_attn_ln.bias"], True, ws[0])
        oq = self.offsets[b + "attn.q_proj.weight"][0]
        d_ln1 = ops.empty((M, C), BF16)
        if s["with_attn"]:
            d_qkv = ops.empty((M, 3 * C), BF16)
            ops.attn_bwd(s["qkv"], s["att"], d_att, s["lse"], cos, sin, d_qkv, ws[0], B, N, H, cfg.head_width ** -0.5)
            obq = self.offsets[b + "attn.q_bias"][0]
            ops.colsum_bf16(d_qkv, self.grad[obq:obq + 3 * C], ws[1])
            self.grad[obq + C:obq + 2 * C].zero_()
            self._wgrad(d_qkv, s["ln1"], self.grad[oq:oq + 3 * C * C].view(3 * C, C))
            self._dgrad(i, "qkv", d_qkv, d_ln1)
        else:
            ops.colsum_bf16(d_att, G[b + "attn.v_bias"], ws[1])
            self._wgrad(d_att, s["ln1"], G[b + "attn.v_proj.weight"])
            self._dgrad(i, "qkv", d_att, d_ln1, cols=(2 * C, 3 * C))
        ops.layernorm_bwd(d_ln1, s["x0"], self.p[b + "norm1.weight"], *s["st1"], g, DX_F32_ACCUM,
                          G[b + "norm1.weight"], G[b + "norm1.bias"], True, ws[0], dx_copy=gb if next_bias is not None else None,
                          copy_colsum=next_bias, **(q8a if next_bias is not None else {}))

    def _stem_bwd(self, g, keep, B, N, grid, ws):
        ops, cfg, P = self.ops, self.cfg, self.prefix
        C = cfg.width
        g3 = g.view(B, N, C)
        d_pos = g3.sum(dim=0)
        self.g[P + "cls_token"].view(C).add_(d_pos[0])
        self._pos_grad(d_pos, grid)
        gp = g3[:, 1:, :].to(BF16).reshape(B * (N - 1), C)
        ops.colsum_bf16(gp, self.g[P + "patch_embed.proj.bias"])
        self._wgrad(gp, keep["patches"], self.storage_of(self.grad, P + "patch_embed.proj.weight"))
```

clipself_amd/engine_base.py:

```python
from __future__ import annotations

import math
import os
from collections import OrderedDict

import torch
import torch.nn.functional as F

from .config import TowerCfg

BF16, F32 = torch.bfloat16, torch.float32
EPI_BF16, EPI_F32, EPI_RESID_F32, EPI_SWIGLU_BF16, EPI_ATOMIC_F32, EPI_PATCH_F32, EPI_RESID_LN_F32, EPI_GELU_BF16, EPI_QGELU_BF16 = range(9)
DX_BF16, DX_F32_ASSIGN, DX_F32_ACCUM = range(3)
ALIGN = 64


def _round_up(x: int, m: int) -> int:
    return (x + m - 1) // m * m


def padded_hidden(cfg: TowerCfg) -> int:
    return _round_up(cfg.hidden, 64)


def is_no_decay(name: str, ndim: int) -> bool:
    return ndim < 2 or "bn" in name or "ln" in name or "bias" in name or "logit_scale" in name


class TowerEngine:
    BLOCK_TAG = None
    FINAL_NORM = None
    RESID_BIAS = None
    HEAD_FWD_TRANSPOSED = False

    def block_index(self, name: str):
        tag = self.prefix + self.BLOCK_TAG
        return int(name[len(tag):].split(".")[0]) if name.startswith(tag) else None

    def _never_reached(self, i: int, name: str) -> bool:
        return False

    def __init__(self, cfg: TowerCfg, ops, trainable: bool = False, prefix: str = "visual."):
        self.cfg, self.ops, self.prefix, self.trainable = cfg, ops, prefix, trainable
        self.offsets = OrderedDict()
        self.logical = {}
        off = 0
        self.block_ranges = []
        cur_block, blk_begin = None, 0
        for grp in self._layout():
            off = _round_up(off, ALIGN)
            blk = self.block_index(grp[0][0])
            if blk != cur_block:
                if cur_block is not None:
                    self.block_ranges.append((blk_begin, off))
                cur_block, blk_begin = blk, off
            for name, shape, storage in grp:
                self.offsets[name] = (off, storage)
                self.logical[name] = shape
                off += math.prod(storage)
        self.numel = _round_up(off, 256)
        self.stem_range = (0, self.block_ranges[0][0]) if self.block_ranges else (0, 0)
        self.head_range = (self.block_ranges[-1][1], self.numel) if self.block_ranges else (0, self.numel)
        self.master = ops.zeros((self.numel,), F32)
        self.shadow = ops.zeros((self.numel,), BF16)
        self.device = self.master.device
        self.Hp = padded_hidden(cfg)
        self.Kpe = _round_up(3 * cfg.patch_size * cfg.patch_size, 64)
        self.p = {n: self.view_of(self.master, n) for n in self.offsets}
        self.w = {n: self.view_of(self.shadow, n) for n in self.offsets}
        self._tables = {}
        self._pos_cache = {}
        self.grad = self.exp_avg = self.exp_avg_sq = self.flags = None
        self.g = {}
        self.wt = {}
        self.first_trainable = cfg.layers
        self.train_all = False
        self.flags_version = 0
        self.grad_ready_hook = None
        self._ctx = None
        self._wgrad_ws = None
        self.cls_only_last_block = True
        self.fold_block_ln = not trainable
        self.block_fold_guard = not trainable
        self.block_fold_limit = 2.0
        self.block_fold_ratio = None
        self.split_stream = not trainable
        self.fold = {}
        self.rccl_window = (0, 0)
        self.wgrad_tn = True
        if trainable:
            self.grad = ops.zeros((self.numel,), F32)
            self.exp_avg = ops.zeros((self.numel,), F32)
            self.exp_avg_sq = ops.zeros((self.numel,), F32)
            self.g = {n: self.view_of(self.grad, n) for n in self.offsets}
            self.flags = torch.zeros(self.numel // 64, dtype=torch.uint8, device=self.device)

    def storage_of(self, buf, name):
        o, st = self.offsets[name]
        return buf[o:o + math.prod(st)].view(st)

    def view_of(self, buf, name):
        o, st = self.offsets[name]
        shape = self.logical[name]
        flat = buf[o:o + math.prod(st)]
        if tuple(st) == tuple(shape) or math.prod(st) == math.prod(shape):
            return flat.view(shape)
        if len(st) == 1:
            return flat[:shape[0]]
        if len(shape) == 2:
            return flat.view(st)[:shape[0], :shape[1]]
        inner = [1]
        for d in reversed(shape[2:]):
            inner.insert(0, inner[0] * d)
        return torch.as_strided(flat, shape, (st[1], *inner))

    def public_names(self):
        return [n for n in self.offsets if "._" not in n]

    def load_state(self, sd: dict, strict: bool = True):
        missing = []
        with torch.no_grad():
            for n in self.public_names():
                if n in sd:
                    self.p[n].copy_(sd[n].to(self.device, F32).reshape(self.p[n].shape))
                else:
                    missing.append(n)
        if strict and missing:
            raise KeyError(f"missing keys: {missing[:5]}... ({len(missing)})")
        self.sync_shadow()
        return missing

    def sync_shadow(self):
        self.ops.cast_f32_bf16(self.master, self.shadow)
        self._pos_cache.clear()
        self.block_fold_ratio = None
        if self.trainable or self.HEAD_FWD_TRANSPOSED:
            self.sync_transposed()
        if self._wants_folds():
            self._build_folds()

    def _wants_folds(self) -> bool:
        return self.fold_block_ln

    def _wt_alloc(self, key, rows, cols):
        t = self.wt.get(key)
        if t is None:
            t = self.ops.zeros((cols, _round_up(rows, 64)), BF16)
            self.wt[key] = t
        return t

    def set_trainable_blocks(self, unlocked_groups: int):
        L = self.cfg.layers
        self.first_trainable = L - unlocked_groups if 0 < unlocked_groups <= L else 0
        self.train_all = False
        self._set_flags()

    def set_trainable_all(self):
        self.first_trainable = 0
        self.train_all = True
        self._set_flags()

    def _set_flags(self):
        if not self.trainable:
            return
        self.flags.zero_()
        names = list(self.offsets)
        for k, name in enumerate(names):
            o, s = self.offsets[name]
            i = self.block_index(name)
            if "._" in name or (i is None and not self._nonblock_trains(name)) or (i is not None and (i < self.first_trainable or self._never_reached(i, name))):
                continue
            n = math.prod(s)
# ... 150 lines not shown
            N = g * g + 1
            cos, sin = self.rope_tables(g)
            xf = x.view(B * N, cfg.width)
            last = cfg.layers - 1 if self.cls_only_last_block else cfg.layers
            xb = st = None
            cls_folded = folded and self._cls_block_folds() and last < cfg.layers and last > 0
            lo = ops.empty((B * N, cfg.width), torch.int16) if folded and self.split_stream and self._lo_plane(last, cls_folded) else None
            try:
                for i in range(last):
                    self._rccl_window_step(i, k0)
                    if folded:
                        xb, st = self._teacher_block_folded(i, xf, xb, st, B, N, cos, sin, emit_next=i + 1 < last or cls_folded, lo=lo)
                    else:
                        self._block_fwd(i, xf, B, N, cos, sin, True, None, True)
            finally:
                self._rccl_window_close(k0)
            if last < cfg.layers:
                xc = self._block_fwd_cls(last, xf, B, N, cos, sin, xb if cls_folded else None, st, lo)
            else:
                xc = x[:, 0, :]
            cls = ops.empty((B, cfg.width), BF16)
            ops.layernorm_fwd(xc, self.p[fn + ".weight"], self.p[fn + ".bias"], cls, None, None, cfg.ln_eps)
            self._head(cls, out[k0:k0 + B])
        return out

    def encode_dense(self, images, need_grad: bool = False):
        ops, cfg, fn = self.ops, self.cfg, self.prefix + self.FINAL_NORM
        B = images.shape[0]
        stem_keep = {} if (need_grad and self._pos_trains()) else None
        x, g = self._stem(images, stem_keep)
        N, C, E = g * g + 1, cfg.width, cfg.embed_dim
        cos, sin = self.rope_tables(g)
        xf = x.view(B * N, C)
        saves = {}
        for i in range(cfg.layers):
            keep = need_grad and i >= self.first_trainable
            save = {} if keep else None
            xf = self._block_fwd(i, xf, B, N, cos, sin, with_attn=(i < cfg.layers - 1), save=save, inplace=not keep)
            if keep:
                saves[i] = save
        M = B * N
        lnf = ops.empty((M, C), BF16)
        mean = ops.empty((M,), F32) if need_grad else None
        rstd = ops.empty((M,), F32) if need_grad else None
        ops.layernorm_fwd(xf, self.p[fn + ".weight"], self.p[fn + ".bias"], lnf, mean, rstd, cfg.ln_eps)
        feats = ops.empty((M, E), F32)
        self._head(lnf, feats)
        dense = ops.empty((M, E), F32)
        inv = ops.empty((M,), F32)
        ops.l2norm_fwd(feats, dense, inv)
        if need_grad:
            self._ctx = dict(B=B, N=N, g=g, saves=saves, xL=xf, stf=(mean, rstd), dense=dense, inv=inv, cos=cos, sin=sin, stem=stem_keep,
                             lnf=lnf if self.train_all else None)
        return dense.view(B, N, E), g

    def roi_pool(self, dense, rois, g):
        pooled = self.ops.empty((rois.shape[0], dense.shape[2]), F32)
        if rois.shape[0]:
            self.ops.roialign_fwd(dense, rois, pooled, g, g, 1)
        return pooled

    def zero_grad(self):
        self.grad.zero_()

    def _wgrad(self, dY, X, dW):
        ops = self.ops
        M, N = dY.shape
        K = X.shape[1]
        need = ops.gemm_wgrad_tn_workspace(N, K, M) if self.wgrad_tn else 0
        if need:
            if self._wgrad_ws is None or self._wgrad_ws.numel() < need:
                self._wgrad_ws = ops.empty((need,), torch.uint8)
            ops.gemm_wgrad_tn(dY, X, dW, self._wgrad_ws)
            return
        Xt = self._transposed(X)
        Mp = Xt.shape[1]
        dYt = ops.empty((N, Mp), BF16)
        ops.transpose_bf16(dY, dYt)
        need = ops.gemm_wgrad_workspace(N, Xt.shape[0], Mp)
        if self._wgrad_ws is None or self._wgrad_ws.numel() < need:
            self._wgrad_ws = ops.empty((need,), torch.uint8)
        ops.gemm_wgrad(dYt, Xt, dW, self._wgrad_ws)

    def _transposed(self, X):
        M, K = X.shape
        Xt = self.ops.empty((K, _round_up(M, 64)), BF16)
        self.ops.transpose_bf16(X, Xt)
        return Xt

    def _bwd_gq(self, M):
        return None

    def backward_dense(self, d_dense):
        ops, cfg, P = self.ops, self.cfg, self.prefix
        c = self._ctx
        if c is None:
            raise RuntimeError("backward_dense() without a preceding encode_dense(need_grad=True)")
        self._ctx = None
        B, N, C, E = c["B"], c["N"], cfg.width, cfg.embed_dim
        M = B * N
        d_feats = ops.empty((M, E), BF16)
        ops.l2norm_bwd(d_dense.reshape(M, E), c["dense"], c["inv"], d_feats)
        d_lnf = ops.empty((M, C), BF16)
        self._head_dgrad(d_feats, d_lnf)
        g = ops.empty((M, C), F32)
        gb = ops.empty((M, C), BF16)
        gq = self._bwd_gq(M)
        q8a = dict(q8=gq[0], q_scale=gq[1]) if gq is not None else {}
        ln_width, colsum_width = self._bwd_widths()
        ws_bytes = max(ops.layernorm_bwd_workspace(M, ln_width), ops.attn_bwd_workspace(B, N, cfg.heads))
        ws = (ops.empty((ws_bytes,), torch.uint8), ops.empty((max(ops.colsum_workspace(M, colsum_width), 4),), torch.uint8))
        L, first, fn = cfg.layers, self.first_trainable, P + self.FINAL_NORM
        resid_bias = lambda i: self.g[f"{P}{self.BLOCK_TAG}{i}.{self.RESID_BIAS}"] if i >= first else None
        if self.train_all:
            self._head_wgrad(d_feats, c["lnf"], ws)
            ops.layernorm_bwd(d_lnf, c["xL"], self.p[fn + ".weight"], *c["stf"], g, DX_F32_ASSIGN,
                              self.g[fn + ".weight"], self.g[fn + ".bias"], True, ws[0], dx_copy=gb, copy_colsum=resid_bias(L - 1), **q8a)
            if self.grad_ready_hook is not None:
                self.grad_ready_hook("head")
        else:
            ops.layernorm_bwd(d_lnf, c["xL"], self.p[fn + ".weight"], *c["stf"], g, DX_F32_ASSIGN, None, None, True, ws[0],
                              dx_copy=gb if first < L else None, copy_colsum=resid_bias(L - 1), **(q8a if first < L else {}))
        for i in range(L - 1, first - 1, -1):
            self._block_bwd(i, c["saves"].pop(i), g, gb, B, N, c["cos"], c["sin"], ws, next_bias=resid_bias(i - 1) if i > 0 else None, gq=gq)
            if self.grad_ready_hook is not None:
                self.grad_ready_hook(i)
        if c["stem"] is not None:
            self._stem_bwd(g, c["stem"], B, N, c["g"], ws[0])
            if self.grad_ready_hook is not None:
                self.grad_ready_hook("stem")

    def roi_pool_backward(self, d_pooled, rois, B, N, g):
        d_dense = self.ops.zeros((B, N, self.cfg.embed_dim), F32)
        if rois.shape[0]:
            self.ops.roialign_bwd(d_pooled.contiguous(), rois, d_dense, g, g, 1)
        return d_dense

    def adamw_step(self, step: int, lr: float, wd: float, beta1=0.9, beta2=0.999, eps=1e-8, grad_scale: float = 1.0):
        self.ops.adamw_step(self.master, self.grad, self.exp_avg, self.exp_avg_sq, self.shadow, self.flags,
                            lr, beta1, beta2, eps, wd, step, grad_scale)
        self.sync_transposed()
        if self._pos_trains():
            self._pos_cache.clear()
```

clipself_amd/hip.py:

```python
from __future__ import annotations

import ctypes
import os
import subprocess
from pathlib import Path

import torch

_CSRC = Path(__file__).resolve().parent / "csrc"
_LIB_PATH = Path(os.environ["CLIPSELF_HIP_LIB"]) if os.environ.get("CLIPSELF_HIP_LIB") else _CSRC / "libclipself_hip.so"

EPI_BF16, EPI_F32, EPI_RESID_F32, EPI_SWIGLU_BF16, EPI_ATOMIC_F32, EPI_PATCH_F32, EPI_RESID_LN_F32, EPI_GELU_BF16, EPI_QGELU_BF16 = range(9)
DX_BF16, DX_F32_ASSIGN, DX_F32_ACCUM = range(3)

_vp, _i, _l, _f, _sz = ctypes.c_void_p, ctypes.c_int, ctypes.c_long, ctypes.c_float, ctypes.c_size_t

SIGNATURES = {
    "cs_last_error": (ctypes.c_char_p, []),
    "cs_gemm_nt": (_i, [_vp, _vp, _vp, _vp, _vp, _i, _i, _i, _i, _i, _i, _i, _i, _i, _i, _vp]),
    "cs_crop_resize_workspace": (_sz, [_i, _i, _i]),
    "cs_crop_resize_u8": (_i, [_vp, _i, _i, _vp, _i, _i, _i, _vp, _vp, _vp, _vp, _vp]),
    "cs_quant_rows_fp8": (_i, [_vp, _l, _vp, _l, _vp, _i, _i, _vp]),
    "cs_gemm_nt_f8": (_i, [_vp, _vp, _vp, _vp, _vp, _vp, _vp, _i, _i, _i, _i, _i, _i, _i, _i, _vp]),
    "cs_resize_bilinear_f32": (_i, [_vp, _vp, _i, _i, _i, _i, _i, _vp]),
    "cs_gemm_wgrad_workspace": (_sz, [_i, _i, _i]),
    "cs_gemm_wgrad": (_i, [_vp, _vp, _vp, _vp, _i, _i, _i, _i, _i, _i, _vp]),
    "cs_gemm_wgrad_tn_workspace": (_sz, [_i, _i, _i]),
    "cs_gemm_wgrad_tn": (_i, [_vp, _vp, _vp, _vp, _i, _i, _i, _i, _i, _i, _vp]),
    "cs_gemm_nt_ln": (_i, [_vp, _vp, _vp, _vp, _vp, _vp, _vp, _vp, _vp, _vp, _i, _i, _i, _i, _i, _i, _i, _i, _i, _i, _i, _vp]),
    "cs_gemm_nt_ln_split": (_i, [_vp, _vp, _vp, _vp, _vp, _vp, _vp, _vp, _vp, _vp, _i, _vp, _i, _i, _i, _i, _i, _i, _i, _vp]),
    "cs_ln_stats_finalize": (_i, [_vp, _i, _i, _i, _i, _f, _vp, _vp, _vp]),
    "cs_attn_fwd_stats": (_i, [_vp, _vp, _vp, _vp, _vp, _vp, _i, _i, _i, _i, _i, _f, _vp]),
    "cs_layernorm_fwd": (_i, [_vp, _i, _l, _vp, _vp, _vp, _l, _vp, _vp, _i, _i, _f, _vp]),
    "cs_layernorm_fwd_q8": (_i, [_vp, _i, _l, _vp, _vp, _vp, _l, _vp, _vp, _vp, _l, _vp, _i, _i, _f, _vp]),
    "cs_layernorm_fwd_f32": (_i, [_vp, _l, _vp, _vp, _vp, _l, _vp, _vp, _i, _i, _f, _vp]),
    "cs_layernorm_bwd_workspace": (_sz, [_i, _i]),
    "cs_layernorm_bwd": (_i, [_vp, _l, _vp, _i, _l, _vp, _vp, _vp, _vp, _i, _l, _vp, _vp, _i, _vp, _vp, _l, _vp, _i, _i, _vp]),
    "cs_layernorm_bwd_q8": (_i, [_vp, _l, _vp, _i, _l, _vp, _vp, _vp, _vp, _i, _l, _vp, _vp, _i, _vp, _vp, _l, _vp, _vp, _l, _vp, _i, _i, _vp]),
    "cs_l2norm_fwd": (_i, [_vp, _vp, _vp, _i, _i, _f, _vp]),
    "cs_l2norm_bwd": (_i, [_vp, _vp, _vp, _vp, _i, _i, _vp]),
    "cs_attn_fwd": (_i, [_vp, _vp, _vp, _vp, _vp, _i, _i, _i, _i, _i, _f, _vp]),
    "cs_attn_cls_fwd": (_i, [_vp, _vp, _vp, _vp, _vp, _i, _i, _i, _i, _i, _i, _f, _vp]),
    "cs_attn_query_fwd": (_i, [_vp, _vp, _vp, _vp, _vp, _i, _i, _i, _i, _i, _i, _i, _f, _vp]),
    "cs_attn_bwd_workspace": (_sz, [_i, _i, _i, _i]),
    "cs_attn_bwd": (_i, [_vp, _vp, _vp, _vp, _vp, _vp, _vp, _vp, _i, _i, _i, _i, _i, _f, _vp, _vp]),
    "cs_swiglu_fwd": (_i, [_vp, _l, _vp, _l, _i, _i, _vp]),
    "cs_swiglu_bwd": (_i, [_vp, _l, _vp, _l, _vp, _l, _i, _i, _vp]),
    "cs_swiglu_bwd_colsum": (_i, [_vp, _l, _vp, _l, _vp, _l, _vp, _vp, _i, _i, _vp]),
    "cs_swiglu_bwd_q8": (_i, [_vp, _l, _vp, _l, _vp, _l, _vp, _l, _vp, _i, _i, _vp]),
    "cs_gelu_fwd": (_i, [_vp, _l, _vp, _l, _i, _i, _i, _vp]),
    "cs_gelu_bwd": (_i, [_vp, _l, _vp, _l, _vp, _l, _i, _i, _i, _vp]),
    "cs_cast_f32_bf16": (_i, [_vp, _vp, _l, _vp]),
    "cs_transpose_bf16": (_i, [_vp, _l, _vp, _l, _i, _i, _vp]),
    "cs_transpose_bf16_batched": (_i, [_vp, _i, _i, _vp]),
    "cs_colsum_workspace": (_sz, [_i, _i]),
    "cs_colsum_bf16": (_i, [_vp, _l, _vp, _vp, _i, _i, _vp]),
    "cs_im2row": (_i, [_vp, _i, _vp, _i, _i, _i, _i, _vp]),
    "cs_cls_row": (_i, [_vp, _vp, _vp, _i, _i, _i, _vp]),
    "cs_roialign_fwd": (_i, [_vp, _vp, _vp, _i, _i, _i, _i, _i, _i, _vp]),
    "cs_roialign_bwd": (_i, [_vp, _vp, _vp, _i, _i, _i, _i, _i, _i, _i, _vp]),
    "cs_cosine_loss_fwd": (_i, [_vp, _vp, _vp, _vp, _i, _i, _f, _vp]),
    "cs_cosine_loss_bwd": (_i, [_vp, _vp, _vp, _vp, _i, _i, _f, _f, _vp, _vp]),
    "cs_fed_bce_fwd": (_i, [_vp, _l, _vp, _vp, _vp, _i, _i, _f, _f, _vp]),
    "cs_fed_bce_bwd": (_i, [_vp, _l, _vp, _vp, _l, _i, _i, _f, _f, _vp, _vp]),
    "cs_num_compute_units": (_i, []),
    "cs_stream_create_cu_mask": (_i, [_i, _i, ctypes.POINTER(_vp)]),
    "cs_stream_destroy": (_i, [_vp]),
    "cs_adamw_step": (_i, [_vp, _vp, _vp, _vp, _vp, _vp, _l, _f, _f, _f, _f, _f, _i, _f, _vp]),
}


class AttnExtra(ctypes.Structure):
    _fields_ = [("q", _vp), ("o", _vp), ("dout", _vp), ("lse", _vp), ("allow", _vp), ("dq", _vp), ("Q", _i), ("ldq", _i), ("ldo", _i), ("lddq", _i)]


def library_path() -> Path:
    return _LIB_PATH


def build_library(force: bool = False) -> Path:
    if force:
        for o in _CSRC.glob("_obj_*.o"):
            o.unlink()
    subprocess.run(["bash", str(_CSRC / "build.sh")], check=True)
    return _LIB_PATH


_lib = None


def load_library():
    global _lib
    if _lib is None:
        if not _LIB_PATH.exists():
            raise RuntimeError(
                f"{_LIB_PATH} is missing: build it with clipself_amd/csrc/build.sh (or __graft_entry__.build()). "
                "There is no CPU fallback for the CLIPSelf hot path.")
        lib = ctypes.CDLL(str(_LIB_PATH))
        for name, (res, args) in SIGNATURES.items():
            fn = getattr(lib, name)
            fn.restype, fn.argtypes = res, args
        _lib = lib
    return _lib


def _p(t):
    return None if t is None else t.data_ptr()


def _dt(t) -> int:
    if t.dtype == torch.float32:
        return 0
    if t.dtype == torch.bfloat16:
        return 1
    raise TypeError(f"unsupported dtype {t.dtype}")


def _readable(t, n) -> bool:
    return t is None or t.untyped_storage().nbytes() - t.storage_offset() * t.element_size() >= n * t.element_size()


class HipOps:

    name = "hip"
    ATTN_EXTRA_QUERIES = True
    ATTN_CAUSAL = True

    def __init__(self):
        self.lib = load_library()
        if not torch.cuda.is_available():
            raise RuntimeError("HipOps needs a ROCm device (torch.cuda.is_available() is False); no CPU fallback exists")
        self.gemm_flags = 0
        self._rccl_reserve = 0
        self._share = 0
        self._cap = 0
        self.num_cus = int(self.lib.cs_num_compute_units())

    def _update_flags(self):
        n = self._rccl_reserve + self._share
        if self._cap:
            n = max(n, self.num_cus - self._cap)
        if not (0 <= n <= self.num_cus - 8 and n < 256):
            raise ValueError(f"persistent GEMM grids keep at least 8 workgroups and can leave at most 255 compute units free "
                             f"(asked to leave {n} of {self.num_cus} CUs: RCCL reserve {self._rccl_reserve}, tower share {self._share}, cap {self._cap})")
        self.gemm_flags = (self.gemm_flags & ~(255 << 20)) | (int(n) << 20)

    def reserve_compute_units(self, n: int):
        self._rccl_reserve = int(n)
        self._update_flags()

    def share_compute_units(self, n: int):
        self._share = int(n)
        self._update_flags()

    def cap_compute_units(self, n: int):
        self._cap = int(n)
        self._update_flags()

    def persistent_grid(self) -> int:
        return self.num_cus - ((self.gemm_flags >> 20) & 255)

    def num_compute_units(self) -> int:
        return self.num_cus

    def stream_create_cu_mask(self, first_cu: int, n_cus: int):
        h = ctypes.c_void_p()
        self._ok(self.lib.cs_stream_create_cu_mask(int(first_cu), int(n_cus), ctypes.byref(h)), "cs_stream_create_cu_mask")
        s = torch.cuda.ExternalStream(h.value)
        s._cs_handle = h.value
        return s

    def stream_destroy(self, stream):
        torch.cuda.synchronize()
        self._ok(self.lib.cs_stream_destroy(ctypes.c_void_p(stream._cs_handle)), "cs_stream_destroy")

    def _stream(self):
        return torch.cuda.current_stream().cuda_stream

    def _ok(self, rc, who):
        if rc != 0:
            raise RuntimeError(f"{who} failed ({rc}): {self.lib.cs_last_error().decode()}")

    @staticmethod
    def _chk(*ts):
        for t in ts:
            if t is not None and not t.is_cuda:
                raise RuntimeError("HipOps received a non-GPU tensor; the hot path has no CPU fallback")

    def empty(self, shape, dtype):
        return torch.empty(shape, dtype=dtype, device="cuda")

    def zeros(self, shape, dtype):
        return torch.zeros(shape, dtype=dtype, device="cuda")

    def gemm_nt(self, A, B, C, bias=None, extra=None, epi=EPI_BF16, splits=1, group=0, flags=0):
        self._chk(A, B, C, bias, extra)
        M, K = A.shape
        N = B.shape[0]
        assert B.shape[1] == K and A.stride(1) == 1 and B.stride(1) == 1 and C.stride(-1) == 1
        if extra is not None and epi in (EPI_RESID_F32, EPI_PATCH_F32):
            assert extra.stride(0) == C.stride(0), "extra must share C's row stride"
        self._ok(self.lib.cs_gemm_nt(_p(A), _p(B), _p(C), _p(bias), _p(extra), M, N, K, A.stride(0), B.stride(0),
                                     C.stride(0), epi, splits, group, flags | self.gemm_flags, self._stream()), "cs_gemm_nt")

    def gemm_nt_ln(self, A, B, C, bias=None, extra=None, ln_mean=None, ln_rstd=None, ln_colsum=None, stats_part=None, xb_out=None,
                   epi=EPI_RESID_LN_F32, group=0, flags=0):
        self._chk(A, B, C, bias, extra, ln_mean, ln_rstd, ln_colsum, stats_part, xb_out)
        M, K = A.shape
        N = B.shape[0]
# ... 9 lines not shown
                                        _p(xb_out), xb_out.stride(0) if xb_out is not None else 0, M, N, K, A.stride(0), B.stride(0),
                                        C.stride(0), epi, 1, group, flags | self.gemm_flags, self._stream()), "cs_gemm_nt_ln")

    def gemm_nt_ln_split(self, A, B, hi, lo, bias, ln_mean, ln_rstd, ln_colsum, x_in=None, x_out=None, stats_part=None, flags=0):
        self._chk(A, B, hi, lo, bias, ln_mean, ln_rstd, ln_colsum, x_in, x_out, stats_part)
        M, K = A.shape
        N = B.shape[0]
        assert hi.dtype == torch.bfloat16 and lo.dtype == torch.int16 and hi.shape == (M, N) and lo.shape == (M, N)
        assert hi.stride(1) == 1 and lo.stride(1) == 1 and hi.stride(0) == lo.stride(0) and hi.stride(0) % 8 == 0
        assert x_out is None or stats_part is None, "fp32 out: hi / lo are only read, no statistics epilogue"
        x = x_in if x_in is not None else x_out
        assert x is None or (x.dtype == torch.float32 and x.shape == (M, N) and x.stride(1) == 1)
        self._ok(self.lib.cs_gemm_nt_ln_split(_p(A), _p(B), _p(bias), _p(ln_mean), _p(ln_rstd), _p(ln_colsum), _p(x_in), _p(x_out), _p(hi), _p(lo),
                                              hi.stride(0), _p(stats_part), M, N, K, A.stride(0), B.stride(0), x.stride(0) if x is not None else N,
                                              flags | self.gemm_flags, self._stream()), "cs_gemm_nt_ln_split")

    def quant_rows_fp8(self, x, q, scale):
        self._chk(x, q, scale)
        M, K = x.shape
        assert x.dtype == torch.bfloat16 and x.stride(1) == 1 and q.element_size() == 1 and q.stride(1) == 1 and q.shape[1] == (K + 127) // 128 * 128
        self._ok(self.lib.cs_quant_rows_fp8(_p(x), x.stride(0), _p(q), q.stride(0), _p(scale), M, K, self._stream()), "cs_quant_rows_fp8")

    def gemm_nt_f8(self, A8, B8, C, row_scale, col_scale, bias=None, extra=None, epi=EPI_BF16, flags=0):
        self._chk(A8, B8, C, row_scale, col_scale, bias, extra)
        M, K8 = A8.shape
        N = B8.shape[0]
        assert B8.shape[1] == K8 and A8.element_size() == 1 and B8.element_size() == 1 and C.stride(-1) == 1
        if extra is not None:
            assert extra.stride(0) == C.stride(0), "extra must share C's row stride"
        self._ok(self.lib.cs_gemm_nt_f8(_p(A8), _p(B8), _p(C), _p(bias), _p(extra), _p(row_scale), _p(col_scale), M, N, K8, A8.stride(0), B8.stride(0),
                                        C.stride(0), epi, flags | self.gemm_flags, self._stream()), "cs_gemm_nt_f8")

    def crop_resize(self, image_u8, boxes, size, pad_center=True, mean=(0.48145466, 0.4578275, 0.40821073),
                    std=(0.26862954, 0.26130258, 0.27577711), out=None):
        self._chk(image_u8, boxes, out)
        assert image_u8.dtype == torch.uint8 and image_u8.dim() == 3 and image_u8.shape[2] == 3 and image_u8.is_contiguous()
        boxes = boxes.to(torch.float32).contiguous()
        H, W, K = image_u8.shape[0], image_u8.shape[1], boxes.shape[0]
        if out is None:
            out = torch.empty((K, 3, size, size), dtype=torch.float32, device=image_u8.device)
        need = int(self.lib.cs_crop_resize_workspace(H, K, size))
        ws = getattr(self, "_crop_ws", None)
        if ws is None or ws.numel() < need:
            ws = self._crop_ws = torch.empty(need, dtype=torch.uint8, device=image_u8.device)
        m3, s3 = (ctypes.c_float * 3)(*mean), (ctypes.c_float * 3)(*std)
        self._ok(self.lib.cs_crop_resize_u8(_p(image_u8), H, W, _p(boxes), K, size, int(bool(pad_center)), m3, s3, _p(out), _p(ws),
                                            self._stream()), "cs_crop_resize_u8")
        return out

    def resize_bilinear(self, x, size):
        self._chk(x)
        assert x.dtype == torch.float32 and x.dim() == 4
        x = x.contiguous()
        B, C, H, W = x.shape
        out = torch.empty((B, C, size, size), dtype=torch.float32, device=x.device)
        self._ok(self.lib.cs_resize_bilinear_f32(_p(x), _p(out), B * C, H, W, size, size, self._stream()), "cs_resize_bilinear_f32")
        return out

    def gemm_wgrad_workspace(self, M, N, K) -> int:
        return int(self.lib.cs_gemm_wgrad_workspace(M, N, K))

    def gemm_wgrad(self, A, B, dW, workspace):
        self._chk(A, B, dW, workspace)
        M, K = A.shape
        N = B.shape[0]
        assert B.shape[1] == K and A.stride(1) == 1 and B.stride(1) == 1 and dW.stride(1) == 1 and dW.dtype == torch.float32
        assert workspace.numel() * workspace.element_size() >= self.gemm_wgrad_workspace(M, N, K)
        self._ok(self.lib.cs_gemm_wgrad(_p(A), _p(B), _p(dW), _p(workspace), M, N, K, A.stride(0), B.stride(0), dW.stride(0),
                                        self._stream()), "cs_gemm_wgrad")

    def gemm_wgrad_tn_workspace(self, N, K, tokens) -> int:
        return int(self.lib.cs_gemm_wgrad_tn_workspace(N, K, tokens))

    def gemm_wgrad_tn(self, dY, X, dW, workspace):
        self._chk(dY, X, dW, workspace)
        T, N = dY.shape
        K = X.shape[1]
        assert X.shape[0] == T and dY.stride(1) == 1 and X.stride(1) == 1 and dW.stride(1) == 1 and dW.dtype == torch.float32
        assert workspace.numel() * workspace.element_size() >= self.gemm_wgrad_tn_workspace(N, K, T) > 0
        rc = self.lib.cs_gemm_wgrad_tn(_p(dY), _p(X), _p(dW), _p(workspace), N, K, T, dY.stride(0), X.stride(0), dW.stride(0), self._stream())
        if rc == 1:
            raise RuntimeError("cs_gemm_wgrad_tn: shape outside the kernel's coverage (check gemm_wgrad_tn_workspace first)")
        self._ok(rc, "cs_gemm_wgrad_tn")

    def ln_stats_finalize(self, part, npp, C, mean, rstd, eps=1e-6):
        self._chk(part, mean, rstd)
        P, M = part.shape[0], part.shape[1]
        assert part.is_contiguous() and part.shape[2] == 2
        self._ok(self.lib.cs_ln_stats_finalize(_p(part), P, npp, C, M, eps, _p(mean), _p(rstd), self._stream()), "cs_ln_stats_finalize")

    def _check_rope_tables(self, cos, sin, Ntok):
        def ver(t):
            try:
                return t._version
            except RuntimeError:
                return -1
        key = (cos.data_ptr(), sin.data_ptr(), ver(cos), ver(sin), Ntok)
        seen = self.__dict__.setdefault("_rope_ok", set())
        if key in seen:
            return
        g = int(round((Ntok - 1) ** 0.5))
        if g * g != Ntok - 1 or tuple(cos.shape) != (Ntok - 1, 64) or tuple(sin.shape) != (Ntok - 1, 64):
            raise ValueError(f"rotary tables must be [g*g, 64] for a square token grid, got {tuple(cos.shape)} for {Ntok} tokens")
        for t in (cos, sin):
            v = t.view(g, g, 64)
            ok = (torch.equal(v[:, :, :32], v[:, :1, :32].expand(g, g, 32)) and torch.equal(v[:, :, 32:], v[:1, :, 32:].expand(g, g, 32))
                  and torch.equal(v[:, 0, :32], v[0, :, 32:]) and torch.equal(v[..., 0::2], v[..., 1::2]))
            if not ok:
                raise ValueError("rotary tables are not in the layout of rope.py:118-142 (separable, row part == column part, one entry per "
                                 "rotation pair): the attention kernels cannot read them")
        if len(seen) > 64:
            seen.clear()
        seen.add(key)

    def attn_fwd_stats(self, qkv, cos, sin, out, lse, stats_part, B, Ntok, H, scale):
        self._chk(qkv, cos, sin, out, lse, stats_part)
        self._check_rope_tables(cos, sin, Ntok)
        assert stats_part.is_contiguous() and tuple(stats_part.shape) == (H, B * Ntok, 2)
        self._ok(self.lib.cs_attn_fwd_stats(_p(qkv), _p(cos), _p(sin), _p(out), _p(lse), _p(stats_part), B, Ntok, H, qkv.stride(0),
                                            out.stride(0), scale, self._stream()), "cs_attn_fwd_stats")

    @staticmethod
    def _ln_pad(C, *params):
        if C % 4:
            assert all(_readable(t, (C + 3) // 4 * 4) for t in params), "LayerNorm with C % 4 != 0: gamma / beta must be readable up to roundup4(C)"

    def layernorm_fwd(self, x, gamma, beta, y, mean=None, rstd=None, eps=1e-6, q8=None, q_scale=None):
        if q8 is not None:
            return self.layernorm_fwd_q8(x, gamma, beta, y, q8, q_scale, mean, rstd, eps)
        self._chk(x, gamma, beta, y, mean, rstd)
        M, C = x.shape
        self._ln_pad(C, gamma, beta)
        self._ok(self.lib.cs_layernorm_fwd(_p(x), _dt(x), x.stride(0), _p(gamma), _p(beta), _p(y), y.stride(0) if y is not None else 0,
                                           _p(mean), _p(rstd), M, C, eps, self._stream()), "cs_layernorm_fwd")

    def layernorm_fwd_q8(self, x, gamma, beta, y, q8, q_scale, mean=None, rstd=None, eps=1e-6):
        self._chk(x, gamma, beta, y, mean, rstd, q8, q_scale)
        M, C = x.shape
        assert q8.element_size() == 1 and q8.stride(1) == 1 and q8.shape[1] >= (C + 127) // 128 * 128 and q_scale is not None and y is not None
        self._ln_pad(C, gamma, beta)
        self._ok(self.lib.cs_layernorm_fwd_q8(_p(x), _dt(x), x.stride(0), _p(gamma), _p(beta), _p(y), y.stride(0), _p(mean), _p(rstd),
                                              _p(q8), q8.stride(0), _p(q_scale), M, C, eps, self._stream()), "cs_layernorm_fwd_q8")

    def layernorm_fwd_f32(self, x, gamma, beta, y, mean=None, rstd=None, eps=1e-5):
        self._chk(x, gamma, beta, y, mean, rstd)
        M, C = x.shape
        assert x.dtype == torch.float32 and y.dtype == torch.float32 and x.stride(1) == 1 and y.stride(1) == 1
        assert x.data_ptr() != y.data_ptr(), "layernorm_fwd_f32 is out of place"
        self._ok(self.lib.cs_layernorm_fwd_f32(_p(x), x.stride(0), _p(gamma), _p(beta), _p(y), y.stride(0), _p(mean), _p(rstd), M, C, eps,
                                               self._stream()), "cs_layernorm_fwd_f32")

    def layernorm_bwd_workspace(self, M, C) -> int:
        return int(self.lib.cs_layernorm_bwd_workspace(M, C))

    def layernorm_bwd_q8(self, dy, x, gamma, mean, rstd, dx, dx_mode, dgamma, dbeta, accumulate, workspace, dx_copy, copy_colsum, q8, q_scale):
        self._chk(dy, x, gamma, mean, rstd, dx, dgamma, dbeta, workspace, dx_copy, copy_colsum, q8, q_scale)
        M, C = x.shape
        assert dx_copy is not None and dx_copy.dtype == torch.bfloat16 and dx_copy.shape == (M, C) and dx_copy.stride(1) == 1
        self._ln_pad(C, gamma)
        assert q8.element_size() == 1 and q8.stride(1) == 1 and q8.shape[1] >= (C + 127) // 128 * 128 and q_scale is not None
        self._ok(self.lib.cs_layernorm_bwd_q8(_p(dy), dy.stride(0), _p(x), _dt(x), x.stride(0), _p(gamma), _p(mean), _p(rstd),
                                              _p(dx), dx_mode, dx.stride(0), _p(dgamma), _p(dbeta), int(accumulate),
                                              _p(workspace), _p(dx_copy), dx_copy.stride(0), _p(copy_colsum), _p(q8), q8.stride(0), _p(q_scale),
                                              M, C, self._stream()), "cs_layernorm_bwd_q8")

    def layernorm_bwd(self, dy, x, gamma, mean, rstd, dx, dx_mode, dgamma=None, dbeta=None, accumulate=False, workspace=None,
                      dx_copy=None, copy_colsum=None, q8=None, q_scale=None):
        if q8 is not None:
            return self.layernorm_bwd_q8(dy, x, gamma, mean, rstd, dx, dx_mode, dgamma, dbeta, accumulate, workspace, dx_copy, copy_colsum,
                                         q8, q_scale)
        self._chk(dy, x, gamma, mean, rstd, dx, dgamma, dbeta, workspace, dx_copy, copy_colsum)
        M, C = x.shape
        self._ln_pad(C, gamma)
        if dx_copy is not None:
            assert dx_copy.dtype == torch.bfloat16 and dx_copy.shape == (M, C) and dx_copy.stride(1) == 1
        self._ok(self.lib.cs_layernorm_bwd(_p(dy), dy.stride(0), _p(x), _dt(x), x.stride(0), _p(gamma), _p(mean), _p(rstd),
                                           _p(dx), dx_mode, dx.stride(0), _p(dgamma), _p(dbeta), int(accumulate),
                                           _p(workspace), _p(dx_copy), dx_copy.stride(0) if dx_copy is not None else 0, _p(copy_colsum),
                                           M, C, self._stream()), "cs_layernorm_bwd")

    def l2norm_fwd(self, x, y, inv_norm, eps=1e-12):
        self._chk(x, y, inv_norm)
        M, C = x.shape
        assert x.is_contiguous() and y.is_contiguous()
        self._ok(self.lib.cs_l2norm_fwd(_p(x), _p(y), _p(inv_norm), M, C, eps, self._stream()), "cs_l2norm_fwd")

    def l2norm_bwd(self, dy, y, inv_norm, dx):
        self._chk(dy, y, inv_norm, dx)
        M, C = y.shape
        assert dy.is_contiguous() and y.is_contiguous() and dx.is_contiguous()
        self._ok(self.lib.cs_l2norm_bwd(_p(dy), _p(y), _p(inv_norm), _p(dx), M, C, self._stream()), "cs_l2norm_bwd")

    def attn_fwd(self, qkv, cos, sin, out, lse, B, Ntok, H, scale):
        self._chk(qkv, cos, sin, out, lse)
        self._check_rope_tables(cos, sin, Ntok)
        self._ok(self.lib.cs_attn_fwd(_p(qkv), _p(cos), _p(sin), _p(out), _p(lse), B, Ntok, H, qkv.stride(0), out.stride(0),
                                      scale, self._stream()), "cs_attn_fwd")

    def attn_cls_fwd(self, q, kv, cos, sin, out, B, Ntok, H, scale):
        self._chk(q, kv, cos, sin, out)
        self._ok(self.lib.cs_attn_cls_fwd(_p(q), _p(kv), _p(cos), _p(sin), _p(out), B, Ntok, H, q.stride(0), kv.stride(0),
                                          out.stride(0), scale, self._stream()), "cs_attn_cls_fwd")

    def attn_query_fwd(self, q, kv, allow, out, B, Q, Ntok, H, scale, lse=None):
        self._chk(q, kv, allow, out, lse)
        if allow is None:
            assert Q == Ntok and lse is None and Ntok <= 128, "attn_query_fwd(allow=None) is causal self-attention: Q == Ntok <= 128, no lse"
            assert q.stride(1) == 1 and kv.stride(1) == 1 and out.stride(1) == 1 and q.shape[0] == B * Ntok == kv.shape[0] == out.shape[0]
            self._ok(self.lib.cs_attn_query_fwd(_p(q), _p(kv), None, _p(out), None, B, Q, Ntok, H, q.stride(0), kv.stride(0), out.stride(0),
                                                scale, self._stream()), "cs_attn_query_fwd")
            return
        assert allow.dtype == torch.uint8 and allow.is_contiguous() and tuple(allow.shape) == (B * Q, Ntok)
        assert lse is None or (lse.dtype == torch.float32 and lse.is_contiguous() and lse.numel() == B * H * Q)
        self._ok(self.lib.cs_attn_query_fwd(_p(q), _p(kv), _p(allow), _p(out), _p(lse), B, Q, Ntok, H, q.stride(0), kv.stride(0), out.stride(0),
                                            scale, self._stream()), "cs_attn_query_fwd")

    def attn_bwd_workspace(self, B, Ntok, H, Q=0) -> int:
        return int(self.lib.cs_attn_bwd_workspace(B, Ntok, H, Q))

    def _check_identity_tables(self, cos, sin):
        key = ("ident", cos.data_ptr(), sin.data_ptr(), tuple(cos.shape))
        seen = self.__dict__.setdefault("_rope_ok", set())
        if key in seen:
            return
        if not (bool((cos == 1).all()) and bool((sin == 0).all())):
            raise ValueError("attn_bwd(extra=...): extra query rows are not rotated, so the rotary tables must be the identity (cos 1, sin 0)")
        seen.add(key)

    def attn_bwd(self, qkv, o, dout, lse, cos, sin, dqkv, workspace, B, Ntok, H, scale, extra=None):
        self._chk(qkv, o, dout, lse, cos, sin, dqkv, workspace)
        assert qkv.stride(0) == dqkv.stride(0)
        if extra is None:
            assert o.stride(0) == dout.stride(0)
            self._ok(self.lib.cs_attn_bwd(_p(qkv), _p(o), _p(dout), _p(lse), _p(cos), _p(sin), _p(dqkv), _p(workspace), B, Ntok, H,
                                          qkv.stride(0), o.stride(0), scale, None, self._stream()), "cs_attn_bwd")
            return
        q, eo, edo, elz, allow, dq, Q = (extra[k] for k in ("q", "o", "dout", "lse", "allow", "dq", "Q"))
        self._chk(q, eo, edo, elz, allow, dq)
        self._check_identity_tables(cos, sin)
        assert (o is None) == (dout is None) == (lse is None), "image rows: o, dout and lse together or not at all"
        assert o is None or o.stride(0) == dout.stride(0)
        assert eo.stride(0) == edo.stride(0) and all(t.stride(1) == 1 for t in (q, eo, edo, dq))
        assert q.shape[0] == B * Q and eo.shape[0] == B * Q and dq.shape[0] == B * Q
        assert allow.dtype == torch.uint8 and allow.is_contiguous() and tuple(allow.shape) == (B * Q, Ntok)
        assert elz.dtype == torch.float32 and elz.is_contiguous() and elz.numel() == B * H * Q
        assert workspace.numel() * workspace.element_size() >= self.attn_bwd_workspace(B, Ntok, H, Q)
        ex = AttnExtra(_p(q), _p(eo), _p(edo), _p(elz), _p(allow), _p(dq), Q, q.stride(0), eo.stride(0), dq.stride(0))
        self._ok(self.lib.cs_attn_bwd(_p(qkv), _p(o), _p(dout), _p(lse), _p(cos), _p(sin), _p(dqkv), _p(workspace), B, Ntok, H,
                                      qkv.stride(0), o.stride(0) if o is not None else H * 64, scale, ctypes.byref(ex), self._stream()), "cs_attn_bwd")

    def swiglu_fwd(self, x12, h):
        self._chk(x12, h)
        M, Hd = h.shape
        self._ok(self.lib.cs_swiglu_fwd(_p(x12), x12.stride(0), _p(h), h.stride(0), M, Hd, self._stream()), "cs_swiglu_fwd")

    def swiglu_bwd_q8(self, dh, x12, dx12, q8, q_scale):
        self._chk(dh, x12, dx12, q8, q_scale)
        M, Hd = dh.shape
        assert q_scale is not None and q8.element_size() == 1 and q8.stride(1) == 1 and q8.shape[1] >= (2 * Hd + 127) // 128 * 128
        self._ok(self.lib.cs_swiglu_bwd_q8(_p(dh), dh.stride(0), _p(x12), x12.stride(0), _p(dx12), dx12.stride(0), _p(q8), q8.stride(0),
                                           _p(q_scale), M, Hd, self._stream()), "cs_swiglu_bwd_q8")

    def swiglu_bwd_colsum(self, dh, x12, dx12, colsum, workspace):
        self._chk(dh, x12, dx12, colsum, workspace)
        M, Hd = dh.shape
        assert colsum.dtype == torch.float32 and colsum.numel() >= 2 * Hd and colsum.is_contiguous()
        assert workspace.numel() * workspace.element_size() >= self.colsum_workspace(M, 2 * Hd)
        self._ok(self.lib.cs_swiglu_bwd_colsum(_p(dh), dh.stride(0), _p(x12), x12.stride(0), _p(dx12), dx12.stride(0), _p(colsum), _p(workspace),
                                               M, Hd, self._stream()), "cs_swiglu_bwd_colsum")

    def swiglu_bwd(self, dh, x12, dx12, q8=None, q_scale=None):
        if q8 is not None:
            return self.swiglu_bwd_q8(dh, x12, dx12, q8, q_scale)
        self._chk(dh, x12, dx12)
        M, Hd = dh.shape
        self._ok(self.lib.cs_swiglu_bwd(_p(dh), dh.stride(0), _p(x12), x12.stride(0), _p(dx12), dx12.stride(0), M, Hd,
                                        self._stream()), "cs_swiglu_bwd")

    def gelu_fwd(self, x, y, quick=False):
        self._chk(x, y)
        M, N = x.shape
        self._ok(self.lib.cs_gelu_fwd(_p(x), x.stride(0), _p(y), y.stride(0), M, N, int(bool(quick)), self._stream()), "cs_gelu_fwd")

    def gelu_bwd(self, dy, x, dx, quick=False):
        self._chk(dy, x, dx)
        M, N = x.shape
        self._ok(self.lib.cs_gelu_bwd(_p(dy), dy.stride(0), _p(x), x.stride(0), _p(dx), dx.stride(0), M, N, int(bool(quick)),
                                      self._stream()), "cs_gelu_bwd")

    def cast_f32_bf16(self, x, y):
        self._chk(x, y)
        assert x.is_contiguous() and y.is_contiguous() and x.numel() == y.numel()
        self._ok(self.lib.cs_cast_f32_bf16(_p(x), _p(y), x.numel(), self._stream()), "cs_cast_f32_bf16")

    def transpose_bf16(self, inp, out):
        self._chk(inp, out)
        R, Cc = inp.shape
        assert out.shape[0] == Cc and out.is_contiguous()
        self._ok(self.lib.cs_transpose_bf16(_p(inp), inp.stride(0), _p(out), out.shape[1], R, Cc, self._stream()), "cs_transpose_bf16")

    def transpose_bf16_batched(self, pairs):
        import numpy as np
        key = tuple((a.data_ptr(), b.data_ptr(), a.shape, b.shape, a.stride(0)) for a, b in pairs)
        tables = self.__dict__.setdefault("_tr_desc_tables", {})
        cache = tables.get(key)
        if cache is None:
            if len(tables) >= 8:
                tables.clear()
            rec = np.zeros((len(pairs), 6), dtype=np.int64)
            tile0 = 0
            for i, (a, b) in enumerate(pairs):
                self._chk(a, b)
                R, Cc = a.shape
                assert b.shape[0] == Cc and b.is_contiguous() and b.shape[1] >= R and a.stride(1) == 1
                tiles_x, tiles_y = (Cc + 63) // 64, (b.shape[1] + 63) // 64
                rec[i] = (a.data_ptr(), b.data_ptr(), a.stride(0), b.shape[1], R | (Cc << 32), tile0 | (tiles_x << 32))
                tile0 += tiles_x * tiles_y
            cache = tables[key] = (key, torch.from_numpy(rec).cuda(), tile0)
        _, desc, total = cache
        self._ok(self.lib.cs_transpose_bf16_batched(_p(desc), len(pairs), total, self._stream()), "cs_transpose_bf16_batched")

    def colsum_workspace(self, M, N) -> int:
        return int(self.lib.cs_colsum_workspace(M, N))

    def colsum_bf16(self, x, out, workspace=None):
        self._chk(x, out, workspace)
        M, N = x.shape
        need = self.colsum_workspace(M, N)
        if workspace is None or workspace.numel() * workspace.element_size() < need:
            workspace = torch.empty(need, dtype=torch.uint8, device=x.device)
        self._ok(self.lib.cs_colsum_bf16(_p(x), x.stride(0), _p(out), _p(workspace), M, N, self._stream()), "cs_colsum_bf16")

    def im2row(self, img, out, p):
        self._chk(img, out)
        B, _, S, _ = img.shape
        assert img.is_contiguous()
        assert out.stride(1) == 1 and out.stride(0) == out.shape[1], "im2row writes whole rows (zeros in [3*p*p, ldo)): out must be contiguous"
        self._ok(self.lib.cs_im2row(_p(img), _dt(img), _p(out), B, S, p, out.stride(0), self._stream()), "cs_im2row")

    def cls_row(self, x, cls, pos):
        self._chk(x, cls, pos)
        B, Ntok, C = x.shape
        self._ok(self.lib.cs_cls_row(_p(x), _p(cls), _p(pos), B, Ntok, C, self._stream()), "cs_cls_row")

    def roialign_fwd(self, feat, rois, pooled, grid_h, grid_w, tok_off):
        self._chk(feat, rois, pooled)
        B, Ntok, E = feat.shape
        self._ok(self.lib.cs_roialign_fwd(_p(feat), _p(rois), _p(pooled), rois.shape[0], Ntok, grid_h, grid_w, E, tok_off,
                                          self._stream()), "cs_roialign_fwd")

    def roialign_bwd(self, dpooled, rois, dfeat, grid_h, grid_w, tok_off):
        self._chk(dpooled, rois, dfeat)
        B, Ntok, E = dfeat.shape
        self._ok(self.lib.cs_roialign_bwd(_p(dpooled), _p(rois), _p(dfeat), rois.shape[0], B, Ntok, grid_h, grid_w, E, tok_off,
                                          self._stream()), "cs_roialign_bwd")

    def cosine_loss_fwd(self, student, teacher, stats, loss, weight):
        self._chk(student, teacher, stats, loss)
        K, E = student.shape
        self._ok(self.lib.cs_cosine_loss_fwd(_p(student), _p(teacher), _p(stats), _p(loss), K, E, weight, self._stream()),
                 "cs_cosine_loss_fwd")

    def cosine_loss_bwd(self, student, teacher, stats, dstudent, weight, grad_scale=1.0, upstream=None):
        self._chk(student, teacher, stats, dstudent, upstream)
        K, E = student.shape
        self._ok(self.lib.cs_cosine_loss_bwd(_p(student), _p(teacher), _p(stats), _p(dstudent), K, E, weight, grad_scale,
                                             _p(upstream), self._stream()), "cs_cosine_loss_bwd")

    def fed_bce_fwd(self, logits, tgt, rowloss, loss, ns, temp, weight):
        self._chk(logits, tgt, rowloss, loss)
        assert tgt.dtype == torch.int32
        self._ok(self.lib.cs_fed_bce_fwd(_p(logits), logits.stride(0), _p(tgt), _p(rowloss), _p(loss), logits.shape[0], ns, temp, weight,
                                         self._stream()), "cs_fed_bce_fwd")

    def fed_bce_bwd(self, logits, tgt, dz, ns, temp, weight, upstream=None):
        self._chk(logits, tgt, dz, upstream)
        assert dz.stride(1) == 1 and dz.stride(0) == dz.shape[1], "fed_bce_bwd writes whole rows (zeros in [ns, ldd)): dz must be contiguous"
        self._ok(self.lib.cs_fed_bce_bwd(_p(logits), logits.stride(0), _p(tgt), _p(dz), dz.stride(0), logits.shape[0], ns, temp, weight,
                                         _p(upstream), self._stream()), "cs_fed_bce_bwd")

    def adamw_step(self, p, g, m, v, shadow, flags, lr, beta1, beta2, eps, wd, step, grad_scale=1.0):
        self._chk(p, g, m, v, shadow, flags)
        self._ok(self.lib.cs_adamw_step(_p(p), _p(g), _p(m), _p(v), _p(shadow), _p(flags), p.numel(), lr, beta1, beta2, eps, wd,
                                        step, grad_scale, self._stream()), "cs_adamw_step")
```

Measured before the change: 731.0 images/sec.

## Defer backward partial reductions into grouped launches and fuse SwiGLU with LayerNorm forward

Adds '_partials' variants of the colsum, LayerNorm-backward and split-K wgrad entry points. Instead of launching their own reduce kernel, these return a descriptor, and one cs_reduce_group call can then finish many pending reductions in a single launch. It also adds a fused swiglu_ln_fwd kernel that computes the SwiGLU hidden, writes it, and applies LayerNorm in the same pass. The goal is fewer small kernel launches and one less read of the hidden activation. In exchange, workspace buffers must stay live until the grouped reduce runs, and a shared reduce kernel has to cover several reduction kinds.

```diff
diff --git a/clipself_amd/csrc/elementwise.hip b/clipself_amd/csrc/elementwise.hip
--- a/clipself_amd/csrc/elementwise.hip
+++ b/clipself_amd/csrc/elementwise.hip
@@ -1,8 +1,8 @@
 #include "cs_common.h"
+#include "reduce_common.h"
+#include "swiglu_common.h"
 
 namespace {
-
-__device__ __forceinline__ float silu_f(float x) { return x / (1.f + __expf(-x)); }
 
 __global__ __launch_bounds__(256) void swiglu_fwd_kernel(const __bf16* __restrict__ x12, long ldx, __bf16* __restrict__ h, long ldh,
                                                          int M, int Hd) {
@@ -14,7 +14,7 @@
         a.u = *(const uint4*)(x12 + (size_t)m * ldx + j);
         b.u = *(const uint4*)(x12 + (size_t)m * ldx + Hd + j);
 #pragma unroll
-        for (int e = 0; e < 8; ++e) o.e[e] = f2bf(silu_f(bf2f(a.e[e])) * bf2f(b.e[e]));
+        for (int e = 0; e < 8; ++e) o.e[e] = swiglu_hidden(a.e[e], b.e[e]);
         *(uint4*)(h + (size_t)m * ldh + j) = o.u;
     }
 }
@@ -308,24 +308,8 @@
 }
 
 __global__ __launch_bounds__(256) void colsum_reduce_kernel(const float* __restrict__ part, int nblocks, int N, float* __restrict__ out) {
-    __shared__ float red[4][64];
-    const int tx = threadIdx.x & 63, r = threadIdx.x >> 6;
-    const int n = blockIdx.x * 64 + tx;
-    float s = 0.f;
-    if (n < N) {
-        int b = r;
-        for (; b + 28 < nblocks; b += 32) {
-            float v[8];
-#pragma unroll
-            for (int u = 0; u < 8; ++u) v[u] = part[(size_t)(b + 4 * u) * N + n];
-#pragma unroll
-            for (int u = 0; u < 8; ++u) s += v[u];
-        }
-        for (; b < nblocks; b += 4) s += part[(size_t)b * N + n];
-    }
-    red[r][tx] = s;
-    __syncthreads();
-    if (r == 0 && n < N) out[n] += (red[0][tx] + red[1][tx]) + (red[2][tx] + red[3][tx]);
+    __shared__ float red[256];
+    colsum_reduce_block(blockIdx.x, red, part, nblocks, N, out, 0, 0);
 }
 
 template <typename TI>
@@ -394,17 +378,32 @@
     return 0;
 }
 constexpr int COLSUM_ROWS = 64;
-extern "C" int cs_swiglu_bwd_colsum(const void* dh, long lddh, const void* x12, long ldx, void* dx12, long lddx, float* colsum, void* workspace,
-                                    int M, int Hd, hipStream_t stream) {
+static void colsum_defer(CsReduceDesc* d, const void* workspace, int nblocks, int N, float* out, int zero_begin, int zero_end) {
+    *d = CsReduceDesc{};
+    d->kind = CS_REDUCE_COLSUM; d->part = (const float*)workspace; d->out0 = out; d->nparts = nblocks; d->cols = N;
+    d->zero_begin = zero_begin; d->zero_end = zero_end;
+}
+static int swiglu_bwd_colsum_impl(const void* dh, long lddh, const void* x12, long ldx, void* dx12, long lddx, float* colsum, void* workspace,
+                                  int M, int Hd, CsReduceDesc* defer, hipStream_t stream) {
     CS_CHECK_ARG(Hd % 8 == 0 && ldx % 8 == 0 && lddh % 8 == 0 && lddx % 8 == 0 && M > 0, "cs_swiglu_bwd_colsum: Hd/ld must be multiples of 8");
     CS_CHECK_ARG(colsum != nullptr && workspace != nullptr, "cs_swiglu_bwd_colsum: colsum and workspace (cs_colsum_workspace(M, 2*Hd) bytes) are required");
     const int nblocks = (M + COLSUM_ROWS - 1) / COLSUM_ROWS;
     hipLaunchKernelGGL(swiglu_bwd_colsum_kernel, dim3((Hd + 511) / 512, nblocks), dim3(256), 0, stream, (const __bf16*)dh, lddh, (const __bf16*)x12, ldx,
                        (__bf16*)dx12, lddx, (float*)workspace, M, Hd, COLSUM_ROWS);
     CS_LAUNCH_CHECK();
+    if (defer != nullptr) { colsum_defer(defer, workspace, nblocks, 2 * Hd, colsum, 0, 0); return 0; }
     hipLaunchKernelGGL(colsum_reduce_kernel, dim3((2 * Hd + 63) / 64), dim3(256), 0, stream, (const float*)workspace, nblocks, 2 * Hd, colsum);
     CS_LAUNCH_CHECK();
     return 0;
+}
+extern "C" int cs_swiglu_bwd_colsum(const void* dh, long lddh, const void* x12, long ldx, void* dx12, long lddx, float* colsum, void* workspace,
+                                    int M, int Hd, hipStream_t stream) {
+    return swiglu_bwd_colsum_impl(dh, lddh, x12, ldx, dx12, lddx, colsum, workspace, M, Hd, nullptr, stream);
+}
+extern "C" int cs_swiglu_bwd_colsum_partials(const void* dh, long lddh, const void* x12, long ldx, void* dx12, long lddx, float* colsum,
+                                             void* workspace, int M, int Hd, CsReduceDesc* desc, hipStream_t stream) {
+    CS_CHECK_ARG(desc != nullptr, "cs_swiglu_bwd_colsum_partials: desc is required");
+    return swiglu_bwd_colsum_impl(dh, lddh, x12, ldx, dx12, lddx, colsum, workspace, M, Hd, desc, stream);
 }
 extern "C" int cs_swiglu_bwd_q8(const void* dh, long lddh, const void* x12, long ldx, void* dx12, long lddx, void* q8, long ldq, float* q_scale,
                                 int M, int Hd, hipStream_t stream) {
@@ -459,15 +458,26 @@
 extern "C" size_t cs_colsum_workspace(int M, int N) {
     return (size_t)((M + COLSUM_ROWS - 1) / COLSUM_ROWS) * (size_t)(N > 0 ? N : 0) * sizeof(float);
 }
-extern "C" int cs_colsum_bf16(const void* x, long ldx, float* out, void* workspace, int M, int N, hipStream_t stream) {
+static int colsum_bf16_impl(const void* x, long ldx, float* out, void* workspace, int M, int N, int zero_begin, int zero_end, CsReduceDesc* defer,
+                            hipStream_t stream) {
     CS_CHECK_ARG(M > 0 && N > 0 && workspace != nullptr, "cs_colsum_bf16: empty input or no workspace (cs_colsum_workspace bytes)");
     const int nblocks = (M + COLSUM_ROWS - 1) / COLSUM_ROWS;
     dim3 grid((N + 511) / 512, nblocks);
     hipLaunchKernelGGL(colsum_bf16_kernel, grid, dim3(256), 0, stream, (const __bf16*)x, ldx, (float*)workspace, M, N, COLSUM_ROWS);
     CS_LAUNCH_CHECK();
+    if (defer != nullptr) { colsum_defer(defer, workspace, nblocks, N, out, zero_begin, zero_end); return 0; }
     hipLaunchKernelGGL(colsum_reduce_kernel, dim3((N + 63) / 64), dim3(256), 0, stream, (const float*)workspace, nblocks, N, out);
     CS_LAUNCH_CHECK();
     return 0;
+}
+extern "C" int cs_colsum_bf16(const void* x, long ldx, float* out, void* workspace, int M, int N, hipStream_t stream) {
+    return colsum_bf16_impl(x, ldx, out, workspace, M, N, 0, 0, nullptr, stream);
+}
+extern "C" int cs_colsum_bf16_partials(const void* x, long ldx, float* out, void* workspace, int M, int N, int zero_begin, int zero_end,
+                                       CsReduceDesc* desc, hipStream_t stream) {
+    CS_CHECK_ARG(desc != nullptr && out != nullptr, "cs_colsum_bf16_partials: desc and out are required");
+    CS_CHECK_ARG(zero_begin >= zero_end || (zero_begin >= 0 && zero_end <= N), "cs_colsum_bf16_partials: zero range [%d, %d) outside [0, %d)", zero_begin, zero_end, N);
+    return colsum_bf16_impl(x, ldx, out, workspace, M, N, zero_begin, zero_end, desc, stream);
 }
 extern "C" int cs_im2row(const void* img, int img_dtype, void* out, int B, int S, int p, int ldo, hipStream_t stream) {
     CS_CHECK_ARG(S % p == 0 && B > 0 && ldo >= 3 * p * p, "cs_im2row: patch size must divide S and ldo >= 3*p*p (p=%d S=%d ldo=%d)", p, S, ldo);
diff --git a/clipself_amd/csrc/gemm.hip b/clipself_amd/csrc/gemm.hip
--- a/clipself_amd/csrc/gemm.hip
+++ b/clipself_amd/csrc/gemm.hip
@@ -1,4 +1,5 @@
 #include "gemm_common.h"
+#include "reduce_common.h"
 #include <hip/amd_detail/amd_hip_unsafe_atomics.h>
 
 namespace {
@@ -703,18 +704,7 @@
 
 __global__ __launch_bounds__(256) void splitk_reduce_kernel(const float* __restrict__ ws, int splits, long stride, float* __restrict__ dst,
                                                             int M, int N, int ldc) {
-    const long i = (long)blockIdx.x * 256 + threadIdx.x;
-    const int n4 = N >> 2;
-    if (i >= (long)M * n4) return;
-    const int row = (int)(i / n4), c = (int)(i - (long)row * n4) * 4;
-    float4 acc = *(const float4*)(ws + (size_t)row * N + c);
-    for (int s = 1; s < splits; ++s) {
-        const float4 t = *(const float4*)(ws + (size_t)s * stride + (size_t)row * N + c);
-        acc.x += t.x; acc.y += t.y; acc.z += t.z; acc.w += t.w;
-    }
-    float4* d = (float4*)(dst + (size_t)row * ldc + c);
-    const float4 o = *d;
-    *d = make_float4(o.x + acc.x, o.y + acc.y, o.z + acc.z, o.w + acc.w);
+    splitk_reduce_block(blockIdx.x, ws, splits, stride, dst, M, N, ldc);
 }
 
 typedef __attribute__((ext_vector_type(4))) short s16x4;
@@ -881,8 +871,8 @@
     return (size_t)choose_tn_splits(N, K, tokens) * N * K * sizeof(float);
 }
 
-extern "C" int cs_gemm_wgrad_tn(const void* dY, const void* X, float* dW, void* workspace, int N, int K, int tokens, int ldy, int ldx, int ldc,
-                                hipStream_t stream) {
+static int gemm_wgrad_tn_impl(const void* dY, const void* X, float* dW, void* workspace, int N, int K, int tokens, int ldy, int ldx, int ldc,
+                              CsReduceDesc* defer, hipStream_t stream) {
     if (tokens <= 0 || N < 8 || K < 8 || N % 8 != 0 || K % 8 != 0) return 1;
     CS_CHECK_ARG(workspace != nullptr && ((uintptr_t)workspace % 16) == 0 && dW != nullptr && ((uintptr_t)dW % 16) == 0 && ldc % 4 == 0,
                  "cs_gemm_wgrad_tn: workspace / dW must be 16-byte aligned buffers");
@@ -905,11 +895,26 @@
     if (tokens % 64 == 0 && N % 256 == 0 && K % 256 == 0) hipLaunchKernelGGL(gemm_tn_kernel<false>, dim3(a.tiles_m * a.tiles_n, splits), dim3(512), lds, stream, a);
     else hipLaunchKernelGGL(gemm_tn_kernel<true>, dim3(a.tiles_m * a.tiles_n, splits), dim3(512), lds, stream, a);
     CS_LAUNCH_CHECK();
+    if (defer != nullptr) {
+        *defer = CsReduceDesc{};
+        defer->kind = CS_REDUCE_SPLITK; defer->part = (const float*)workspace; defer->out0 = dW; defer->nparts = splits;
+        defer->stride = (long)N * K; defer->rows = N; defer->cols = K; defer->ldc = ldc;
+        return 0;
+    }
     const long n = (long)N * (K >> 2);
     hipLaunchKernelGGL(splitk_reduce_kernel, dim3((unsigned)((n + 255) / 256)), dim3(256), 0, stream, (const float*)workspace, splits,
                        (long)N * K, dW, N, K, ldc);
     CS_LAUNCH_CHECK();
     return 0;
+}
+extern "C" int cs_gemm_wgrad_tn(const void* dY, const void* X, float* dW, void* workspace, int N, int K, int tokens, int ldy, int ldx, int ldc,
+                                hipStream_t stream) {
+    return gemm_wgrad_tn_impl(dY, X, dW, workspace, N, K, tokens, ldy, ldx, ldc, nullptr, stream);
+}
+extern "C" int cs_gemm_wgrad_tn_partials(const void* dY, const void* X, float* dW, void* workspace, int N, int K, int tokens, int ldy, int ldx,
+                                         int ldc, CsReduceDesc* desc, hipStream_t stream) {
+    CS_CHECK_ARG(desc != nullptr, "cs_gemm_wgrad_tn_partials: desc is required");
+    return gemm_wgrad_tn_impl(dY, X, dW, workspace, N, K, tokens, ldy, ldx, ldc, desc, stream);
 }
 
 extern "C" size_t cs_gemm_wgrad_workspace(int M, int N, int K) {
diff --git a/clipself_amd/csrc/norm.hip b/clipself_amd/csrc/norm.hip
--- a/clipself_amd/csrc/norm.hip
+++ b/clipself_amd/csrc/norm.hip
@@ -1,4 +1,6 @@
 #include "cs_common.h"
+#include "reduce_common.h"
+#include "swiglu_common.h"
 
 namespace {
 
@@ -30,6 +32,26 @@
 }
 __device__ __forceinline__ void store_x4(__bf16* p, const float (&v)[4]) { store_bf16x4(p, v); }
 __device__ __forceinline__ void store_x4(float* p, const float (&v)[4]) { *(float4*)p = make_float4(v[0], v[1], v[2], v[3]); }
+
+template <int MAXG>
+__device__ __forceinline__ void ln_row_stats(const float (&v)[MAXG][4], int ng, int C, int lane, float eps, float& mean, float& rstd) {
+#pragma clang fp contract(off)
+    float s = 0.f;
+#pragma unroll
+    for (int g = 0; g < MAXG; ++g) s += (v[g][0] + v[g][1]) + (v[g][2] + v[g][3]);
+    mean = wave_sum(s) / (float)C;
+    float q = 0.f;
+#pragma unroll
+    for (int g = 0; g < MAXG; ++g) {
+        const int c = (g * 64 + lane) * 4;
+#pragma unroll
+        for (int i = 0; i < 4; ++i) { const float d = v[g][i] - mean; q += (g < ng && c + i < C) ? d * d : 0.f; }
+    }
+    rstd = rsqrtf(wave_sum(q) / (float)C + eps);
+}
+__device__ __forceinline__ float ln_affine(float v, float mean, float rstd, float ga, float be) {
+    return __builtin_fmaf((v - mean) * rstd, ga, be);
+}
 
 template <typename TX, int MAXG, typename TY = __bf16, bool Q8 = false, bool RAG = false>
 __global__ __launch_bounds__(256) void ln_fwd_kernel(const TX* __restrict__ x, long ldx, const float* __restrict__ gamma,
@@ -50,24 +72,15 @@
         const int c = (g * 64 + lane) * 4;
         xr_raw[g] = Vec4<TX>::load_raw(xr + (g < ng ? min(c, clast) : 0));
     }
-    float s = 0.f;
 #pragma unroll
     for (int g = 0; g < MAXG; ++g) {
         const int c = (g * 64 + lane) * 4;
         Vec4<TX>::cvt(xr_raw[g], v[g]);
 #pragma unroll
         for (int i = 0; i < 4; ++i) v[g][i] = (g < ng && (RAG ? c + i < C : c < C)) ? v[g][i] : 0.f;
-        s += (v[g][0] + v[g][1]) + (v[g][2] + v[g][3]);
-    }
-    const float mean = wave_sum(s) / (float)C;
-    float q = 0.f;
-#pragma unroll
-    for (int g = 0; g < MAXG; ++g) {
-        const int c = (g * 64 + lane) * 4;
-#pragma unroll
-        for (int i = 0; i < 4; ++i) { const float d = v[g][i] - mean; q += (g < ng && c + i < C) ? d * d : 0.f; }
-    }
-    const float rstd = rsqrtf(wave_sum(q) / (float)C + eps);
+    }
+    float mean, rstd;
+    ln_row_stats<MAXG>(v, ng, C, lane, eps, mean, rstd);
     if (y != nullptr) {
         TY* yr = y + (size_t)row * ldy;
         float4 ga[MAXG], be[MAXG];
@@ -82,8 +95,8 @@
         for (int g = 0; g < MAXG; ++g) {
             const int c = (g * 64 + lane) * 4;
             if (g < ng && c < C) {
-                float o[4] = {(v[g][0] - mean) * rstd * ga[g].x + be[g].x, (v[g][1] - mean) * rstd * ga[g].y + be[g].y,
-                              (v[g][2] - mean) * rstd * ga[g].z + be[g].z, (v[g][3] - mean) * rstd * ga[g].w + be[g].w};
+                float o[4] = {ln_affine(v[g][0], mean, rstd, ga[g].x, be[g].x), ln_affine(v[g][1], mean, rstd, ga[g].y, be[g].y),
+                              ln_affine(v[g][2], mean, rstd, ga[g].z, be[g].z), ln_affine(v[g][3], mean, rstd, ga[g].w, be[g].w)};
                 if (RAG) {
 #pragma unroll
                     for (int i = 0; i < 4; ++i) o[i] = (c + i < C) ? o[i] : 0.f;
@@ -115,6 +128,59 @@
                     *(unsigned*)(q8 + (size_t)row * ldq + c) = w;
                 }
             }
+        }
+    }
+    if (lane == 0 && mean_out) { mean_out[row] = mean; rstd_out[row] = rstd; }
+}
+
+template <int MAXG>
+__global__ __launch_bounds__(256) void swiglu_ln_fwd_kernel(const __bf16* __restrict__ x12, long ldx, __bf16* __restrict__ hid, long ldh,
+                                                            const float* __restrict__ gamma, const float* __restrict__ beta,
+                                                            __bf16* __restrict__ y, long ldy, float* __restrict__ mean_out,
+                                                            float* __restrict__ rstd_out, int M, int Hd, float eps) {
+    const int lane = threadIdx.x & 63;
+    const int row = blockIdx.x * ROWS_PER_WG + (threadIdx.x >> 6);
+    if (row >= M) return;
+    const __bf16* xr = x12 + (size_t)row * ldx;
+    const int ng = (Hd + 255) >> 8;
+    const int clast = Hd - 4;
+    uint2 a_raw[MAXG], b_raw[MAXG];
+#pragma unroll
+    for (int g = 0; g < MAXG; ++g) {
+        const int c = g < ng ? min((g * 64 + lane) * 4, clast) : 0;
+        a_raw[g] = *(const uint2*)(xr + c);
+        b_raw[g] = *(const uint2*)(xr + Hd + c);
+    }
+    float v[MAXG][4];
+#pragma unroll
+    for (int g = 0; g < MAXG; ++g) {
+        const int c = (g * 64 + lane) * 4;
+        const bool in = g < ng && c < Hd;
+        U64 a, b, h;
+        a.u = a_raw[g]; b.u = b_raw[g];
+#pragma unroll
+        for (int i = 0; i < 4; ++i) h.e[i] = swiglu_hidden(a.e[i], b.e[i]);
+        if (in) *(uint2*)(hid + (size_t)row * ldh + c) = h.u;
+#pragma unroll
+        for (int i = 0; i < 4; ++i) v[g][i] = in ? bf2f(h.e[i]) : 0.f;
+    }
+    float mean, rstd;
+    ln_row_stats<MAXG>(v, ng, Hd, lane, eps, mean, rstd);
+    __bf16* yr = y + (size_t)row * ldy;
+    float4 ga[MAXG], be[MAXG];
+#pragma unroll
+    for (int g = 0; g < MAXG; ++g) {
+        const int c = g < ng ? min((g * 64 + lane) * 4, clast) : 0;
+        ga[g] = *(const float4*)(gamma + c);
+        be[g] = *(const float4*)(beta + c);
+    }
+#pragma unroll
+    for (int g = 0; g < MAXG; ++g) {
+        const int c = (g * 64 + lane) * 4;
+        if (g < ng && c < Hd) {
+            const float o[4] = {ln_affine(v[g][0], mean, rstd, ga[g].x, be[g].x), ln_affine(v[g][1], mean, rstd, ga[g].y, be[g].y),
+                                ln_affine(v[g][2], mean, rstd, ga[g].z, be[g].z), ln_affine(v[g][3], mean, rstd, ga[g].w, be[g].w)};
+            store_bf16x4(yr + c, o);
         }
     }
     if (lane == 0 && mean_out) { mean_out[row] = mean; rstd_out[row] = rstd; }
@@ -347,34 +413,8 @@
 
 __global__ __launch_bounds__(256) void ln_param_reduce_kernel(const float* __restrict__ part, int nparts, int C, int NR, float* __restrict__ out0,
                                                               float* __restrict__ out1, float* __restrict__ out2, int accumulate) {
-    __shared__ float red[16][16];
-    const int cl = threadIdx.x & 15, grp = threadIdx.x >> 4;
-    const int Cp = (C + 3) & ~3;
-    const int c = blockIdx.x * 16 + cl;
-    const int r = c / Cp, cc = c - r * Cp;
-    float* const outs[3] = {out0, out1, out2};
-    const bool live = r < NR && cc < C && outs[r < 3 ? r : 0] != nullptr;
-    float s0 = 0.f, s1 = 0.f, s2 = 0.f, s3 = 0.f;
-    const size_t stride = (size_t)NR * Cp;
-    if (live) {
-        int p = grp;
-        for (; p + 48 < nparts; p += 64) {
-            s0 += part[(size_t)p * stride + c];
-            s1 += part[(size_t)(p + 16) * stride + c];
-            s2 += part[(size_t)(p + 32) * stride + c];
-            s3 += part[(size_t)(p + 48) * stride + c];
-        }
-        for (; p < nparts; p += 16) s0 += part[(size_t)p * stride + c];
-    }
-    red[grp][cl] = (s0 + s1) + (s2 + s3);
-    __syncthreads();
-    if (grp == 0 && live) {
-        float s = 0.f;
-#pragma unroll
-        for (int g = 0; g < 16; ++g) s += red[g][cl];
-        float* dst = outs[r] + cc;
-        *dst = accumulate ? *dst + s : s;
-    }
+    __shared__ float red[256];
+    ln_param_reduce_block(blockIdx.x, red, part, nparts, C, NR, out0, out1, out2, accumulate);
 }
 
 __global__ __launch_bounds__(256) void l2norm_fwd_kernel(const float* __restrict__ x, float* __restrict__ y,
@@ -452,6 +492,20 @@
     return layernorm_fwd_impl(x, x_dtype, ldx, gamma, beta, y, ldy, mean, rstd, M, C, eps, q8, ldq, q_scale, stream);
 }
 
+extern "C" int cs_swiglu_ln_fwd(const void* x12, long ldx, void* hid, long ldh, const float* gamma, const float* beta, void* y, long ldy,
+                                float* mean, float* rstd, int M, int Hd, float eps, hipStream_t stream) {
+    CS_CHECK_ARG(x12 && hid && gamma && beta && y && M > 0 && Hd >= 8 && Hd % 8 == 0 && Hd <= MAXC, "cs_swiglu_ln_fwd: Hd=%d must be a multiple of 8, at most %d", Hd, MAXC);
+    CS_CHECK_ARG(ldx % 8 == 0 && ldh % 8 == 0 && ldy % 8 == 0 && ldx >= 2 * (long)Hd && ldh >= Hd && ldy >= Hd, "cs_swiglu_ln_fwd: row strides must be multiples of 8 that hold a row");
+    CS_CHECK_ARG((((uintptr_t)x12 | (uintptr_t)hid | (uintptr_t)y | (uintptr_t)gamma | (uintptr_t)beta) % 16) == 0, "cs_swiglu_ln_fwd: buffers must be 16-byte aligned");
+    CS_CHECK_ARG((mean == nullptr) == (rstd == nullptr), "cs_swiglu_ln_fwd: mean/rstd must both be given or both null");
+    dim3 grid((M + ROWS_PER_WG - 1) / ROWS_PER_WG), block(256);
+#define SWLN(NG) hipLaunchKernelGGL((swiglu_ln_fwd_kernel<NG>), grid, block, 0, stream, (const __bf16*)x12, ldx, (__bf16*)hid, ldh, gamma, beta, (__bf16*)y, ldy, mean, rstd, M, Hd, eps)
+    if (Hd <= 1024) SWLN(4); else if (Hd <= 2048) SWLN(8); else SWLN(12);
+#undef SWLN
+    CS_LAUNCH_CHECK();
+    return 0;
+}
+
 extern "C" int cs_layernorm_fwd_f32(const float* x, long ldx, const float* gamma, const float* beta, float* y, long ldy, float* mean,
                                     float* rstd, int M, int C, float eps, hipStream_t stream) {
     CS_CHECK_ARG(x && y && gamma && beta && C <= MAXC && C % 4 == 0 && ldx % 4 == 0 && ldy % 4 == 0 && M > 0,
@@ -483,7 +537,7 @@
 static int layernorm_bwd_impl(const void* dy, long lddy, const void* x, int x_dtype, long ldx, const float* gamma, const float* mean,
                               const float* rstd, void* dx, int dx_mode, long lddx, float* dgamma, float* dbeta,
                               int accumulate_params, void* workspace, void* dx_copy, long ldcopy, float* copy_colsum, void* q8, long ldq,
-                              float* q_scale, int M, int C, hipStream_t stream) {
+                              float* q_scale, int M, int C, hipStream_t stream, CsReduceDesc* defer = nullptr) {
     const int Kp = (C + 127) / 128 * 128;
     CS_CHECK_ARG(q8 == nullptr || (dx_copy != nullptr && q_scale != nullptr && ldq >= Kp && ldq % 4 == 0 && ((uintptr_t)q8 % 4) == 0 && Kp <= 256 * 12),
                  "cs_layernorm_bwd_q8: needs dx_copy, the scale vector and 4-byte aligned e4m3 rows of >= %d bytes", Kp);
@@ -522,6 +576,12 @@
 #undef LNB4
 #undef LNB5
     CS_LAUNCH_CHECK();
+    if (defer != nullptr) {
+        *defer = CsReduceDesc{};
+        defer->kind = CS_REDUCE_LN_PARAM; defer->cols = C; defer->nr = NR; defer->accumulate = accumulate_params;
+        if (need_part) { defer->part = part; defer->nparts = nwg; defer->out0 = dgamma; defer->out1 = dbeta; defer->out2 = copy_colsum; }
+        return 0;
+    }
     if (need_part) {
         hipLaunchKernelGGL(ln_param_reduce_kernel, dim3((NR * ((C + 3) & ~3) + 15) / 16), dim3(256), 0, stream, part, nwg, C, NR, dgamma, dbeta,
                            copy_colsum, accumulate_params);
@@ -545,6 +605,15 @@
                               dx_copy, ldcopy, copy_colsum, q8, ldq, q_scale, M, C, stream);
 }
 
+extern "C" int cs_layernorm_bwd_partials(const void* dy, long lddy, const void* x, int x_dtype, long ldx, const float* gamma, const float* mean,
+                                         const float* rstd, void* dx, int dx_mode, long lddx, float* dgamma, float* dbeta,
+                                         int accumulate_params, void* workspace, void* dx_copy, long ldcopy, float* copy_colsum, void* q8,
+                                         long ldq, float* q_scale, int M, int C, CsReduceDesc* desc, hipStream_t stream) {
+    CS_CHECK_ARG(desc != nullptr, "cs_layernorm_bwd_partials: desc is required");
+    return layernorm_bwd_impl(dy, lddy, x, x_dtype, ldx, gamma, mean, rstd, dx, dx_mode, lddx, dgamma, dbeta, accumulate_params, workspace,
+                              dx_copy, ldcopy, copy_colsum, q8, ldq, q_scale, M, C, stream, desc);
+}
+
 extern "C" int cs_l2norm_fwd(const float* x, float* y, float* inv_norm, int M, int C, float eps, hipStream_t stream) {
     CS_CHECK_ARG(C % 4 == 0 && M > 0, "cs_l2norm_fwd: C must be a multiple of 4");
     hipLaunchKernelGGL(l2norm_fwd_kernel, dim3((M + ROWS_PER_WG - 1) / ROWS_PER_WG), dim3(256), 0, stream, x, y, inv_norm, M, C, eps);
diff --git a/clipself_amd/csrc/reduce.hip b/clipself_amd/csrc/reduce.hip
--- /dev/null
+++ b/clipself_amd/csrc/reduce.hip
@@ -0,0 +1,50 @@
+#include "reduce_common.h"
+
+namespace {
+
+constexpr int MAX_GROUP = 16;
+
+struct ReduceGroupArgs {
+    CsReduceDesc d[MAX_GROUP];
+    int first[MAX_GROUP + 1];
+    int n;
+};
+
+__global__ __launch_bounds__(256) void reduce_group_kernel(const ReduceGroupArgs a) {
+    __shared__ float red[256];
+    const int b = blockIdx.x;
+    int i = 0;
+    while (i + 1 < a.n && a.first[i + 1] <= b) ++i;
+    const CsReduceDesc& d = a.d[i];
+    const int blk = b - a.first[i];
+    if (d.kind == CS_REDUCE_LN_PARAM) ln_param_reduce_block(blk, red, d.part, d.nparts, d.cols, d.nr, d.out0, d.out1, d.out2, d.accumulate);
+    else if (d.kind == CS_REDUCE_COLSUM) colsum_reduce_block(blk, red, d.part, d.nparts, d.cols, d.out0, d.zero_begin, d.zero_end);
+    else splitk_reduce_block(blk, d.part, d.nparts, d.stride, d.out0, d.rows, d.cols, d.ldc);
+}
+
+}
+
+extern "C" int cs_reduce_group(const CsReduceDesc* descs, int n, hipStream_t stream) {
+    CS_CHECK_ARG(descs != nullptr && n >= 1 && n <= MAX_GROUP, "cs_reduce_group: 1 .. %d descriptors, got %d", MAX_GROUP, n);
+    ReduceGroupArgs a;
+    int total = 0;
+    for (int i = 0; i < n; ++i) {
+        const CsReduceDesc& d = descs[i];
+        const int blocks = cs_reduce_blocks(d);
+        CS_CHECK_ARG(blocks >= 0, "cs_reduce_group: descriptor %d has unknown kind %d", i, d.kind);
+        CS_CHECK_ARG(blocks == 0 || (d.part != nullptr && d.nparts >= 1 && d.cols >= 1), "cs_reduce_group: descriptor %d has outputs but no partials", i);
+        CS_CHECK_ARG(d.kind != CS_REDUCE_SPLITK || blocks == 0 || (d.rows >= 1 && d.cols % 4 == 0 && d.ldc % 4 == 0 && d.ldc >= d.cols),
+                     "cs_reduce_group: descriptor %d: split-K rows are whole float4s", i);
+        CS_CHECK_ARG(d.kind != CS_REDUCE_LN_PARAM || (d.nr >= 2 && d.nr <= 3), "cs_reduce_group: descriptor %d: 2 or 3 partial rows per workgroup", i);
+        a.d[i] = d;
+        a.first[i] = total;
+        total += blocks;
+    }
+    for (int i = n; i <= MAX_GROUP; ++i) a.first[i] = total;
+    for (int i = n; i < MAX_GROUP; ++i) a.d[i] = CsReduceDesc{};
+    a.n = n;
+    if (total == 0) return 0;
+    hipLaunchKernelGGL(reduce_group_kernel, dim3((unsigned)total), dim3(256), 0, stream, a);
+    CS_LAUNCH_CHECK();
+    return 0;
+}
diff --git a/clipself_amd/csrc/reduce_common.h b/clipself_amd/csrc/reduce_common.h
--- /dev/null
+++ b/clipself_amd/csrc/reduce_common.h
@@ -0,0 +1,102 @@
+#pragma once
+#include "cs_common.h"
+
+enum { CS_REDUCE_LN_PARAM = 0, CS_REDUCE_COLSUM = 1, CS_REDUCE_SPLITK = 2 };
+struct CsReduceDesc {
+    const float* part;
+    float* out0;
+    float* out1;
+    float* out2;
+    long stride;
+    int kind;
+    int nparts;
+    int rows;
+    int cols;
+    int ldc;
+    int nr;
+    int accumulate;
+    int zero_begin, zero_end;
+    int reserved;
+};
+static_assert(sizeof(CsReduceDesc) == 80, "descriptor layout is part of the C ABI");
+
+inline int cs_reduce_blocks(const CsReduceDesc& d) {
+    switch (d.kind) {
+    case CS_REDUCE_LN_PARAM: return (d.out0 || d.out1 || d.out2) ? (d.nr * ((d.cols + 3) & ~3) + 15) / 16 : 0;
+    case CS_REDUCE_COLSUM: return d.out0 ? (d.cols + 63) / 64 : 0;
+    case CS_REDUCE_SPLITK: return d.out0 ? (int)(((long)d.rows * (d.cols >> 2) + 255) / 256) : 0;
+    }
+    return -1;
+}
+
+__device__ __forceinline__ void ln_param_reduce_block(int blk, float* __restrict__ red, const float* __restrict__ part, int nparts, int C, int NR,
+                                                      float* __restrict__ out0, float* __restrict__ out1, float* __restrict__ out2,
+                                                      int accumulate) {
+    const int cl = threadIdx.x & 15, grp = threadIdx.x >> 4;
+    const int Cp = (C + 3) & ~3;
+    const int c = blk * 16 + cl;
+    const int r = c / Cp, cc = c - r * Cp;
+    float* const outs[3] = {out0, out1, out2};
+    const bool live = r < NR && cc < C && outs[r < 3 ? r : 0] != nullptr;
+    float s0 = 0.f, s1 = 0.f, s2 = 0.f, s3 = 0.f;
+    const size_t stride = (size_t)NR * Cp;
+    if (live) {
+        int p = grp;
+        for (; p + 48 < nparts; p += 64) {
+            s0 += part[(size_t)p * stride + c];
+            s1 += part[(size_t)(p + 16) * stride + c];
+            s2 += part[(size_t)(p + 32) * stride + c];
+            s3 += part[(size_t)(p + 48) * stride + c];
+        }
+        for (; p < nparts; p += 16) s0 += part[(size_t)p * stride + c];
+    }
+    red[grp * 16 + cl] = (s0 + s1) + (s2 + s3);
+    __syncthreads();
+    if (grp == 0 && live) {
+        float s = 0.f;
+#pragma unroll
+        for (int g = 0; g < 16; ++g) s += red[g * 16 + cl];
+        float* dst = outs[r] + cc;
+        *dst = accumulate ? *dst + s : s;
+    }
+}
+
+__device__ __forceinline__ void colsum_reduce_block(int blk, float* __restrict__ red, const float* __restrict__ part, int nblocks, int N,
+                                                    float* __restrict__ out, int zero_begin, int zero_end) {
+    const int tx = threadIdx.x & 63, r = threadIdx.x >> 6;
+    const int n = blk * 64 + tx;
+    float s = 0.f;
+    if (n < N) {
+        int b = r;
+        for (; b + 28 < nblocks; b += 32) {
+            float v[8];
+#pragma unroll
+            for (int u = 0; u < 8; ++u) v[u] = part[(size_t)(b + 4 * u) * N + n];
+#pragma unroll
+            for (int u = 0; u < 8; ++u) s += v[u];
+        }
+        for (; b < nblocks; b += 4) s += part[(size_t)b * N + n];
+    }
+    red[r * 64 + tx] = s;
+    __syncthreads();
+    if (r == 0 && n < N) {
+        if (n >= zero_begin && n < zero_end) out[n] = 0.f;
+        else out[n] += (red[tx] + red[64 + tx]) + (red[128 + tx] + red[192 + tx]);
+    }
+}
+
+__device__ __forceinline__ void splitk_reduce_block(int blk, const float* __restrict__ ws, int splits, long stride, float* __restrict__ dst,
+                                                    int M, int N, int ldc) {
+    const long i = (long)blk * 256 + threadIdx.x;
+    const int n4 = N >> 2;
+    if (i >= (long)M * n4) return;
+    const int row = (int)(i / n4), c = (int)(i - (long)row * n4) * 4;
+    float4 acc = *(const float4*)(ws + (size_t)row * N + c);
+    for (int s = 1; s < splits; ++s) {
+        const float4 t = *(const float4*)(ws + (size_t)s * stride + (size_t)row * N + c);
+        acc.x += t.x; acc.y += t.y; acc.z += t.z; acc.w += t.w;
+    }
+    float4* d = (float4*)(dst + (size_t)row * ldc + c);
+    const float4 o = *d;
+    *d = make_float4(o.x + acc.x, o.y + acc.y, o.z + acc.z, o.w + acc.w);
+}
diff --git a/clipself_amd/csrc/swiglu_common.h b/clipself_amd/csrc/swiglu_common.h
--- /dev/null
+++ b/clipself_amd/csrc/swiglu_common.h
@@ -0,0 +1,6 @@
+#pragma once
+#include "cs_common.h"
+
+__device__ __forceinline__ float silu_f(float x) { return x / (1.f + __expf(-x)); }
+
+__device__ __forceinline__ __bf16 swiglu_hidden(__bf16 x1, __bf16 x2) { return f2bf(silu_f(bf2f(x1)) * bf2f(x2)); }
diff --git a/clipself_amd/engine.py b/clipself_amd/engine.py
--- a/clipself_amd/engine.py
+++ b/clipself_amd/engine.py
@@ -57,6 +57,7 @@
         self.fp8_dgrad = False
         self.wt8 = {}
         self.fused_swiglu_colsum = os.environ.get("CLIPSELF_NO_FUSED_SWIGLU_COLSUM") != "1"
+        self.fused_swiglu_ln = bool(getattr(ops, "SWIGLU_LN_FWD", False))
 
     def _wants_folds(self):
         return self.fold_sub_ln
@@ -302,12 +303,19 @@
         if keep or self.fp8_forward:
             x12 = ops.empty((M, 2 * Hd), BF16)
             self._linear(i, "w12", ln2, w12, x12, b12, xq=q3)
-            ops.swiglu_fwd(x12, hid)
-        else:
+            fused_ln = self.fused_swiglu_ln and not padded and not self.fp8_forward and Hd <= 3072
+            if not fused_ln:
+                ops.swiglu_fwd(x12, hid)
+        else:
+            fused_ln = False
             ops.gemm_nt(ln2, w12, hid, bias=b12, epi=EPI_SWIGLU_BF16, group=Hd)
         fln = (ops.zeros if padded else ops.empty)((M, Hd), BF16)
         m4, r4 = st()
-        q4 = self._ln(hid[:, :Hl], self.p[b + "mlp.ffn_ln.weight"], self.p[b + "mlp.ffn_ln.bias"], fln[:, :Hl], m4, r4, eps)
+        if fused_ln:
+            q4 = None
+            ops.swiglu_ln_fwd(x12, hid, self.p[b + "mlp.ffn_ln.weight"], self.p[b + "mlp.ffn_ln.bias"], fln, m4, r4, eps)
+        else:
+            q4 = self._ln(hid[:, :Hl], self.p[b + "mlp.ffn_ln.weight"], self.p[b + "mlp.ffn_ln.bias"], fln[:, :Hl], m4, r4, eps)
         x2 = x1 if inplace else ops.empty((M, C), F32)
         self._linear(i, "w3", fln, self.storage_of(self.shadow, b + "mlp.w3.weight"), x2, self.p[b + "mlp.w3.bias"], extra=x1,
                      epi=EPI_RESID_F32, xq=q4)
@@ -421,6 +429,8 @@
         b = f"{self.prefix}blocks.{i}."
         M = B * N
         G = self.g
+        if self.deferred_reduce and gq is None and not self.fp8_dgrad and not padded and self.wgrad_tn:
+            return self._block_bwd_deferred(i, s, g, gb, B, N, cos, sin, ws, next_bias)
         self._wgrad(gb, s["fln"], self.storage_of(self.grad, b + "mlp.w3.weight"))
         d_fln = ops.empty((M, Hd), BF16)
         self._dgrad(i, "w3", gb, d_fln, q=gq)
@@ -469,6 +479,60 @@
                           G[b + "norm1.weight"], G[b + "norm1.bias"], True, ws[0], dx_copy=gb if next_bias is not None else None,
                           copy_colsum=next_bias, **(q8a if next_bias is not None else {}))
 
+    def _block_bwd_deferred(self, i, s, g, gb, B, N, cos, sin, ws, next_bias):
+        ops, cfg = self.ops, self.cfg
+        C, Hd, H = cfg.width, self.Hp, cfg.heads
+        b = f"{self.prefix}blocks.{i}."
+        M = B * N
+        G = self.g
+        descs = []
+        ln_ws = lambda slot, width: self._deferred_ws(slot, ops.layernorm_bwd_workspace(M, width))
+        self._wgrad_deferred(gb, s["fln"], self.storage_of(self.grad, b + "mlp.w3.weight"), "wg_w3", descs)
+        d_fln = ops.empty((M, Hd), BF16)
+        self._dgrad(i, "w3", gb, d_fln)
+        d_hid = ops.empty((M, Hd), BF16)
+        descs.append(ops.layernorm_bwd_partials(d_fln, s["hid"], self.p[b + "mlp.ffn_ln.weight"], *s["st4"], d_hid, DX_BF16,
+                                                G[b + "mlp.ffn_ln.weight"], G[b + "mlp.ffn_ln.bias"], True, ln_ws("ln_ffn", Hd)))
+        d_x12 = ops.empty((M, 2 * Hd), BF16)
+        ob = self.offsets[b + "mlp.w1.bias"][0]
+        cs12 = self._deferred_ws("cs_w12", ops.colsum_workspace(M, 2 * Hd))
+        if self.fused_swiglu_colsum:
+            descs.append(ops.swiglu_bwd_colsum_partials(d_hid, s["x12"], d_x12, self.grad[ob:ob + 2 * Hd], cs12))
+        else:
+            ops.swiglu_bwd(d_hid, s["x12"], d_x12)
+            descs.append(ops.colsum_bf16_partials(d_x12, self.grad[ob:ob + 2 * Hd], cs12))
+        ow = self.offsets[b + "mlp.w1.weight"][0]
+        self._wgrad_deferred(d_x12, s["ln2"], self.grad[ow:ow + 2 * Hd * C].view(2 * Hd, C), "wg_w12", descs)
+        d_ln2 = ops.empty((M, C), BF16)
+        self._dgrad(i, "w12", d_x12, d_ln2)
+        descs.append(ops.layernorm_bwd_partials(d_ln2, s["x1"], self.p[b + "norm2.weight"], *s["st3"], g, DX_F32_ACCUM,
+                                                G[b + "norm2.weight"], G[b + "norm2.bias"], True, ln_ws("ln_norm2", C), dx_copy=gb,
+                                                copy_colsum=G[b + "attn.proj.bias"]))
+        self._wgrad_deferred(gb, s["iln"], G[b + "attn.proj.weight"], "wg_proj", descs)
+        d_iln = ops.empty((M, C), BF16)
+        self._dgrad(i, "proj", gb, d_iln)
+        d_att = ops.empty((M, C), BF16)
+        descs.append(ops.layernorm_bwd_partials(d_iln, s["att"], self.p[b + "attn.inner_attn_ln.weight"], *s["st2"], d_att, DX_BF16,
+                                                G[b + "attn.inner_attn_ln.weight"], G[b + "attn.inner_attn_ln.bias"], True, ln_ws("ln_inner", C)))
+        oq = self.offsets[b + "attn.q_proj.weight"][0]
+        d_ln1 = ops.empty((M, C), BF16)
+        if s["with_attn"]:
+            d_qkv = ops.empty((M, 3 * C), BF16)
+            ops.attn_bwd(s["qkv"], s["att"], d_att, s["lse"], cos, sin, d_qkv, ws[0], B, N, H, cfg.head_width ** -0.5)
+            obq = self.offsets[b + "attn.q_bias"][0]
+            descs.append(ops.colsum_bf16_partials(d_qkv, self.grad[obq:obq + 3 * C], self._deferred_ws("cs_qkv", ops.colsum_workspace(M, 3 * C)),
+                                                  zero=(C, 2 * C)))
+            self._wgrad_deferred(d_qkv, s["ln1"], self.grad[oq:oq + 3 * C * C].view(3 * C, C), "wg_qkv", descs)
+            self._dgrad(i, "qkv", d_qkv, d_ln1)
+        else:
+            descs.append(ops.colsum_bf16_partials(d_att, G[b + "attn.v_bias"], self._deferred_ws("cs_qkv", ops.colsum_workspace(M, 3 * C))))
+            self._wgrad_deferred(d_att, s["ln1"], G[b + "attn.v_proj.weight"], "wg_qkv", descs)
+            self._dgrad(i, "qkv", d_att, d_ln1, cols=(2 * C, 3 * C))
+        descs.append(ops.layernorm_bwd_partials(d_ln1, s["x0"], self.p[b + "norm1.weight"], *s["st1"], g, DX_F32_ACCUM,
+                                                G[b + "norm1.weight"], G[b + "norm1.bias"], True, ln_ws("ln_norm1", C),
+                                                dx_copy=gb if next_bias is not None else None, copy_colsum=next_bias))
+        ops.reduce_group(descs)
+
     def _stem_bwd(self, g, keep, B, N, grid, ws):
         ops, cfg, P = self.ops, self.cfg, self.prefix
         C = cfg.width
diff --git a/clipself_amd/engine_base.py b/clipself_amd/engine_base.py
--- a/clipself_amd/engine_base.py
+++ b/clipself_amd/engine_base.py
@@ -88,6 +88,8 @@
         self.fold = {}
         self.rccl_window = (0, 0)
         self.wgrad_tn = True
+        self.deferred_reduce = bool(getattr(ops, "DEFERRED_REDUCE", False))
+        self._defer_ws = None
         if trainable:
             self.grad = ops.zeros((self.numel,), F32)
             self.exp_avg = ops.zeros((self.numel,), F32)
@@ -404,6 +406,20 @@
             self._wgrad_ws = ops.empty((need,), torch.uint8)
         ops.gemm_wgrad(dYt, Xt, dW, self._wgrad_ws)
 
+    def _deferred_ws(self, slot, nbytes):
+        if self._defer_ws is None:
+            self._defer_ws = {}
+        t = self._defer_ws.get(slot)
+        if t is None or t.numel() < nbytes:
+            t = self._defer_ws[slot] = self.ops.empty((max(int(nbytes), 4),), torch.uint8)
+        return t
+
+    def _wgrad_deferred(self, dY, X, dW, slot, descs):
+        need = self.ops.gemm_wgrad_tn_workspace(dY.shape[1], X.shape[1], dY.shape[0]) if self.wgrad_tn else 0
+        if not need:
+            return self._wgrad(dY, X, dW)
+        descs.append(self.ops.gemm_wgrad_tn_partials(dY, X, dW, self._deferred_ws(slot, need)))
+
     def _transposed(self, X):
         M, K = X.shape
         Xt = self.ops.empty((K, _round_up(M, 64)), BF16)
@@ -443,10 +459,12 @@
         else:
             ops.layernorm_bwd(d_lnf, c["xL"], self.p[fn + ".weight"], *c["stf"], g, DX_F32_ASSIGN, None, None, True, ws[0],
                               dx_copy=gb if first < L else None, copy_colsum=resid_bias(L - 1), **(q8a if first < L else {}))
+        self._defer_ws = {}
         for i in range(L - 1, first - 1, -1):
             self._block_bwd(i, c["saves"].pop(i), g, gb, B, N, c["cos"], c["sin"], ws, next_bias=resid_bias(i - 1) if i > 0 else None, gq=gq)
             if self.grad_ready_hook is not None:
                 self.grad_ready_hook(i)
+        self._defer_ws = None
         if c["stem"] is not None:
             self._stem_bwd(g, c["stem"], B, N, c["g"], ws[0])
             if self.grad_ready_hook is not None:
diff --git a/clipself_amd/hip.py b/clipself_amd/hip.py
--- a/clipself_amd/hip.py
+++ b/clipself_amd/hip.py
@@ -69,9 +69,26 @@
     "cs_adamw_step": (_i, [_vp, _vp, _vp, _vp, _vp, _vp, _l, _f, _f, _f, _f, _f, _i, _f, _vp]),
 }
 
+DEFERRED_SIGNATURES = {
+    "cs_reduce_group": (_i, [_vp, _i, _vp]),
+    "cs_layernorm_bwd_partials": (_i, [_vp, _l, _vp, _i, _l, _vp, _vp, _vp, _vp, _i, _l, _vp, _vp, _i, _vp, _vp, _l, _vp, _vp, _l, _vp, _i, _i, _vp, _vp]),
+    "cs_swiglu_bwd_colsum_partials": (_i, [_vp, _l, _vp, _l, _vp, _l, _vp, _vp, _i, _i, _vp, _vp]),
+    "cs_colsum_bf16_partials": (_i, [_vp, _l, _vp, _vp, _i, _i, _i, _i, _vp, _vp]),
+    "cs_gemm_wgrad_tn_partials": (_i, [_vp, _vp, _vp, _vp, _i, _i, _i, _i, _i, _i, _vp, _vp]),
+    "cs_swiglu_ln_fwd": (_i, [_vp, _l, _vp, _l, _vp, _vp, _vp, _l, _vp, _vp, _i, _i, _f, _vp]),
+}
+
 
 class AttnExtra(ctypes.Structure):
     _fields_ = [("q", _vp), ("o", _vp), ("dout", _vp), ("lse", _vp), ("allow", _vp), ("dq", _vp), ("Q", _i), ("ldq", _i), ("ldo", _i), ("lddq", _i)]
+
+
+class ReduceDesc(ctypes.Structure):
+    _fields_ = [("part", _vp), ("out0", _vp), ("out1", _vp), ("out2", _vp), ("stride", _l), ("kind", _i), ("nparts", _i), ("rows", _i),
+                ("cols", _i), ("ldc", _i), ("nr", _i), ("accumulate", _i), ("zero_begin", _i), ("zero_end", _i), ("reserved", _i)]
+
+
+REDUCE_GROUP_MAX = 16
 
 
 def library_path() -> Path:
@@ -97,7 +114,7 @@
                 f"{_LIB_PATH} is missing: build it with clipself_amd/csrc/build.sh (or __graft_entry__.build()). "
                 "There is no CPU fallback for the CLIPSelf hot path.")
         lib = ctypes.CDLL(str(_LIB_PATH))
-        for name, (res, args) in SIGNATURES.items():
+        for name, (res, args) in {**SIGNATURES, **DEFERRED_SIGNATURES}.items():
             fn = getattr(lib, name)
             fn.restype, fn.argtypes = res, args
         _lib = lib
@@ -125,6 +142,8 @@
     name = "hip"
     ATTN_EXTRA_QUERIES = True
     ATTN_CAUSAL = True
+    DEFERRED_REDUCE = True
+    SWIGLU_LN_FWD = True
 
     def __init__(self):
         self.lib = load_library()
@@ -300,6 +319,20 @@
         if rc == 1:
             raise RuntimeError("cs_gemm_wgrad_tn: shape outside the kernel's coverage (check gemm_wgrad_tn_workspace first)")
         self._ok(rc, "cs_gemm_wgrad_tn")
+
+    def gemm_wgrad_tn_partials(self, dY, X, dW, workspace):
+        self._chk(dY, X, dW, workspace)
+        T, N = dY.shape
+        K = X.shape[1]
+        assert X.shape[0] == T and dY.stride(1) == 1 and X.stride(1) == 1 and dW.stride(1) == 1 and dW.dtype == torch.float32
+        assert workspace.numel() * workspace.element_size() >= self.gemm_wgrad_tn_workspace(N, K, T) > 0
+        desc = ReduceDesc()
+        rc = self.lib.cs_gemm_wgrad_tn_partials(_p(dY), _p(X), _p(dW), _p(workspace), N, K, T, dY.stride(0), X.stride(0), dW.stride(0),
+                                                ctypes.byref(desc), self._stream())
+        if rc == 1:
+            raise RuntimeError("cs_gemm_wgrad_tn_partials: shape outside the kernel's coverage (check gemm_wgrad_tn_workspace first)")
+        self._ok(rc, "cs_gemm_wgrad_tn_partials")
+        return desc
 
     def ln_stats_finalize(self, part, npp, C, mean, rstd, eps=1e-6):
         self._chk(part, mean, rstd)
@@ -397,6 +430,40 @@
                                            _p(workspace), _p(dx_copy), dx_copy.stride(0) if dx_copy is not None else 0, _p(copy_colsum),
                                            M, C, self._stream()), "cs_layernorm_bwd")
 
+    def layernorm_bwd_partials(self, dy, x, gamma, mean, rstd, dx, dx_mode, dgamma=None, dbeta=None, accumulate=False, workspace=None,
+                               dx_copy=None, copy_colsum=None, q8=None, q_scale=None):
+        self._chk(dy, x, gamma, mean, rstd, dx, dgamma, dbeta, workspace, dx_copy, copy_colsum, q8, q_scale)
+        M, C = x.shape
+        self._ln_pad(C, gamma)
+        if dx_copy is not None:
+            assert dx_copy.dtype == torch.bfloat16 and dx_copy.shape == (M, C) and dx_copy.stride(1) == 1
+        if q8 is not None:
+            assert q8.element_size() == 1 and q8.stride(1) == 1 and q8.shape[1] >= (C + 127) // 128 * 128 and q_scale is not None
+        if dgamma is not None or copy_colsum is not None:
+            assert workspace is not None and workspace.numel() * workspace.element_size() >= self.layernorm_bwd_workspace(M, C)
+        desc = ReduceDesc()
+        self._ok(self.lib.cs_layernorm_bwd_partials(_p(dy), dy.stride(0), _p(x), _dt(x), x.stride(0), _p(gamma), _p(mean), _p(rstd),
+                                                    _p(dx), dx_mode, dx.stride(0), _p(dgamma), _p(dbeta), int(accumulate), _p(workspace),
+                                                    _p(dx_copy), dx_copy.stride(0) if dx_copy is not None else 0, _p(copy_colsum),
+                                                    _p(q8), q8.stride(0) if q8 is not None else 0, _p(q_scale), M, C, ctypes.byref(desc),
+                                                    self._stream()), "cs_layernorm_bwd_partials")
+        return desc
+
+    def reduce_group(self, descs):
+        descs = list(descs)
+        for i in range(0, len(descs), REDUCE_GROUP_MAX):
+            chunk = descs[i:i + REDUCE_GROUP_MAX]
+            arr = (ReduceDesc * len(chunk))(*chunk)
+            self._ok(self.lib.cs_reduce_group(arr, len(chunk), self._stream()), "cs_reduce_group")
+
+    def swiglu_ln_fwd(self, x12, hid, gamma, beta, y, mean=None, rstd=None, eps=1e-6):
+        self._chk(x12, hid, gamma, beta, y, mean, rstd)
+        M, Hd = hid.shape
+        assert x12.shape == (M, 2 * Hd) and y.shape == (M, Hd) and x12.stride(1) == 1 and hid.stride(1) == 1 and y.stride(1) == 1
+        assert x12.dtype == hid.dtype == y.dtype == torch.bfloat16 and gamma.numel() >= Hd and beta.numel() >= Hd
+        self._ok(self.lib.cs_swiglu_ln_fwd(_p(x12), x12.stride(0), _p(hid), hid.stride(0), _p(gamma), _p(beta), _p(y), y.stride(0), _p(mean),
+                                           _p(rstd), M, Hd, eps, self._stream()), "cs_swiglu_ln_fwd")
+
     def l2norm_fwd(self, x, y, inv_norm, eps=1e-12):
         self._chk(x, y, inv_norm)
         M, C = x.shape
@@ -487,6 +554,16 @@
         self._ok(self.lib.cs_swiglu_bwd_colsum(_p(dh), dh.stride(0), _p(x12), x12.stride(0), _p(dx12), dx12.stride(0), _p(colsum), _p(workspace),
                                                M, Hd, self._stream()), "cs_swiglu_bwd_colsum")
 
+    def swiglu_bwd_colsum_partials(self, dh, x12, dx12, colsum, workspace):
+        self._chk(dh, x12, dx12, colsum, workspace)
+        M, Hd = dh.shape
+        assert colsum.dtype == torch.float32 and colsum.numel() >= 2 * Hd and colsum.is_contiguous()
+        assert workspace.numel() * workspace.element_size() >= self.colsum_workspace(M, 2 * Hd)
+        desc = ReduceDesc()
+        self._ok(self.lib.cs_swiglu_bwd_colsum_partials(_p(dh), dh.stride(0), _p(x12), x12.stride(0), _p(dx12), dx12.stride(0), _p(colsum),
+                                                        _p(workspace), M, Hd, ctypes.byref(desc), self._stream()), "cs_swiglu_bwd_colsum_partials")
+        return desc
+
     def swiglu_bwd(self, dh, x12, dx12, q8=None, q_scale=None):
         if q8 is not None:
             return self.swiglu_bwd_q8(dh, x12, dx12, q8, q_scale)
@@ -549,6 +626,17 @@
             workspace = torch.empty(need, dtype=torch.uint8, device=x.device)
         self._ok(self.lib.cs_colsum_bf16(_p(x), x.stride(0), _p(out), _p(workspace), M, N, self._stream()), "cs_colsum_bf16")
 
+    def colsum_bf16_partials(self, x, out, workspace, zero=None):
+        self._chk(x, out, workspace)
+        M, N = x.shape
+        assert out.dtype == torch.float32 and out.numel() >= N and out.is_contiguous()
+        assert workspace.numel() * workspace.element_size() >= self.colsum_workspace(M, N)
+        zb, ze = zero if zero is not None else (0, 0)
+        desc = ReduceDesc()
+        self._ok(self.lib.cs_colsum_bf16_partials(_p(x), x.stride(0), _p(out), _p(workspace), M, N, int(zb), int(ze), ctypes.byref(desc),
+                                                  self._stream()), "cs_colsum_bf16_partials")
+        return desc
+
     def im2row(self, img, out, p):
         self._chk(img, out)
         B, _, S, _ = img.shape
diff --git a/include/clipself_hip_deferred.h b/include/clipself_hip_deferred.h
--- /dev/null
+++ b/include/clipself_hip_deferred.h
@@ -0,0 +1,46 @@
+#ifndef CLIPSELF_HIP_DEFERRED_H
+#define CLIPSELF_HIP_DEFERRED_H
+#include "clipself_hip.h"
+
+#ifdef __cplusplus
+extern "C" {
+#endif
+
+enum { CS_REDUCE_LN_PARAM = 0, CS_REDUCE_COLSUM = 1, CS_REDUCE_SPLITK = 2 };
+typedef struct cs_reduce_desc {
+    const float* part;
+    float* out0;
+    float* out1;
+    float* out2;
+    long stride;
+    int kind;
+    int nparts;
+    int rows;
+    int cols;
+    int ldc;
+    int nr;
+    int accumulate;
+    int zero_begin, zero_end;
+    int reserved;
+} cs_reduce_desc;
+
+int cs_reduce_group(const cs_reduce_desc* descs, int n, cs_stream_t stream);
+
+int cs_layernorm_bwd_partials(const void* dy, long lddy, const void* x, int x_dtype, long ldx, const float* gamma, const float* mean,
+                              const float* rstd, void* dx, int dx_mode, long lddx, float* dgamma, float* dbeta, int accumulate_params,
+                              void* workspace, void* dx_copy, long ldcopy, float* copy_colsum, void* q8, long ldq, float* q_scale, int M, int C,
+                              cs_reduce_desc* desc, cs_stream_t stream);
+int cs_swiglu_bwd_colsum_partials(const void* dh, long lddh, const void* x12, long ldx, void* dx12, long lddx, float* colsum, void* workspace,
+                                  int M, int Hd, cs_reduce_desc* desc, cs_stream_t stream);
+int cs_colsum_bf16_partials(const void* x, long ldx, float* out, void* workspace, int M, int N, int zero_begin, int zero_end,
+                            cs_reduce_desc* desc, cs_stream_t stream);
+int cs_gemm_wgrad_tn_partials(const void* dY, const void* X, float* dW, void* workspace, int N, int K, int tokens, int ldy, int ldx, int ldc,
+                              cs_reduce_desc* desc, cs_stream_t stream);
+
+int cs_swiglu_ln_fwd(const void* x12, long ldx, void* hid, long ldh, const float* gamma, const float* beta, void* y, long ldy, float* mean,
+                     float* rstd, int M, int Hd, float eps, cs_stream_t stream);
+
+#ifdef __cplusplus
+}
+#endif
+#endif
```

After: 731.2 images/sec, median of 2. About the same (+0.0%).
